# tmtlakmal/acme

Measured on AMD Instinct MI355X. Metric: learner transitions/sec (sample+step) at batch 512, 1/2/4/8 MI355X, higher is better.
Workload: dtype f32 (2xf16 split planes, 3 MFMA terms); 1 GPU; dqn_nature_cnn_prioritized_replay (BASELINE configs[1]); global_batch=512, batch_per_gpu=512, replay_slots=1000000, replay_slots_per_gpu=1000000, obs=uint8[84,84,4], num_actions=18, sampler=prioritized(alpha=0.6), IS beta=0.2, prefetch_size=4, parallelism=dp1

## Files before the change

acme_amd/csrc/conv.h:

```cpp
#pragma once

#include "gemm.h"

namespace acme {
namespace conv {

using gemm::f32x4;
using gemm::KCONTIG;
using gemm::RCONTIG;
using gemm::zero4;

template <int IH_, int IW_, int CI_, int OH_, int OW_, int CO_, int KH_, int KW_, int S_,
          int PT_, int PL_>
struct Geom {
  static constexpr int IH = IH_, IW = IW_, CI = CI_, OH = OH_, OW = OW_, CO = CO_;
  static constexpr int KH = KH_, KW = KW_, S = S_, PT = PT_, PL = PL_;
  static constexpr int K = KH * KW * CI;
  static constexpr int IPIX = IH * IW, OPIX = OH * OW;
  static_assert(CI % 4 == 0 && CO % 4 == 0, "channel counts must be multiples of 4");
};

struct InU8 {
  using T = uint8_t;
  __device__ static __forceinline__ float scale(uint32_t x) {
    const float xf = (float)x;
    const float c = 1.0f / 255.0f;
    const float q = xf * c;
    return __builtin_fmaf(__builtin_fmaf(-q, 255.0f, xf), c, q);
  }
  __device__ static __forceinline__ f32x4 load4(const uint8_t* p) {
    const uint32_t w = *reinterpret_cast<const uint32_t*>(p);
    return f32x4{scale(w & 0xff), scale((w >> 8) & 0xff), scale((w >> 16) & 0xff),
                 scale(w >> 24)};
  }
};
struct InF32 {
  using T = float;
  __device__ static __forceinline__ f32x4 load4(const float* p) {
    return *reinterpret_cast<const f32x4*>(p);
  }
};

template <class G, class In>
struct ConvFwd {
  static constexpr int A_MODE = KCONTIG, B_MODE = KCONTIG;
  int M, N, K, k_chunk;
  const typename In::T* x;
  const typename In::T* x2;
  int split_b;
  const float* w;
  const float* bias;
  float* y;
  struct ARow {
    const typename In::T* base;
    int ih0, iw0;
    bool ok;
  };
  struct BRow {
    int n;
  };
  __device__ ARow a_row(int m) const {
    ARow a;
    a.ok = m < M;
    const int mm = a.ok ? m : 0;
    const int b = mm / G::OPIX, rem = mm - b * G::OPIX;
    const int oh = rem / G::OW, ow = rem - oh * G::OW;
    a.base = b < split_b ? x + (size_t)b * G::IPIX * G::CI
                         : x2 + (size_t)(b - split_b) * G::IPIX * G::CI;
    a.ih0 = oh * G::S - G::PT;
    a.iw0 = ow * G::S - G::PL;
    return a;
  }
  __device__ f32x4 a_load(const ARow& a, int k) const {
    const int kh = k / (G::KW * G::CI), r = k - kh * (G::KW * G::CI);
    const int kw = r / G::CI, ci = r - kw * G::CI;
    const int ih = a.ih0 + kh, iw = a.iw0 + kw;
    if (!a.ok || (unsigned)ih >= (unsigned)G::IH || (unsigned)iw >= (unsigned)G::IW) return zero4();
    return In::load4(a.base + (ih * G::IW + iw) * G::CI + ci);
  }
  __device__ BRow b_row(int n) const { return BRow{n}; }
  __device__ f32x4 b_load(const BRow& b, int k) const {
    if (b.n >= N) return zero4();
    const float* p = w + (size_t)k * G::CO + b.n;
    return f32x4{p[0], p[G::CO], p[2 * G::CO], p[3 * G::CO]};
  }
  __device__ void store(int m, int n, float v, int) const {
    v += bias[n];
    y[(size_t)m * G::CO + n] = v > 0.f ? v : 0.f;
  }
};

template <class G, class In>
struct ConvWgrad {
  static constexpr int A_MODE = RCONTIG, B_MODE = RCONTIG;
  static constexpr bool kColSum = true;
  int M, N, K, k_chunk;
  const typename In::T* x;
  const float* dz;
  float* slab;
  struct ARow {
    int dh, dw, ci;
    bool ok;
  };
  struct BRow {
    int n;
  };
  __device__ ARow a_row(int i) const {
    ARow a;
    a.ok = i < M;
    const int ii = a.ok ? i : 0;
    const int kh = ii / (G::KW * G::CI), r = ii - kh * (G::KW * G::CI);
    const int kw = r / G::CI;
    a.ci = r - kw * G::CI;
    a.dh = kh - G::PT;
    a.dw = kw - G::PL;
    return a;
  }
  __device__ f32x4 a_load(const ARow& a, int m) const {
    if (!a.ok) return zero4();
    const int b = m / G::OPIX, rem = m - b * G::OPIX;
    const int oh = rem / G::OW, ow = rem - oh * G::OW;
    const int ih = oh * G::S + a.dh, iw = ow * G::S + a.dw;
    if ((unsigned)ih >= (unsigned)G::IH || (unsigned)iw >= (unsigned)G::IW) return zero4();
    return In::load4(x + ((size_t)b * G::IPIX + ih * G::IW + iw) * G::CI + a.ci);
  }
  __device__ BRow b_row(int n) const { return BRow{n}; }
  __device__ f32x4 b_load(const BRow& b, int m) const {
    if (b.n >= N) return zero4();
    return *reinterpret_cast<const f32x4*>(dz + (size_t)m * G::CO + b.n);
  }
  __device__ void store(int i, int n, float v, int split) const {
    slab[((size_t)split * (M + 1) + i) * N + n] = v;
  }
  __device__ void store_colsum(int n, float v, int split) const {
    slab[((size_t)split * (M + 1) + M) * N + n] = v;
  }
};

template <class G, int PH, int PW>
struct ConvDgradSub {
  static_assert(G::KH % G::S == 0 && G::KW % G::S == 0, "kernel must be a multiple of stride");
  static constexpr int A_MODE = KCONTIG, B_MODE = KCONTIG;
  static constexpr int S = G::S;
  static constexpr int RH = ((PH - G::PT) % S + S) % S;
  static constexpr int RW = ((PW - G::PL) % S + S) % S;
  static constexpr int NH = (G::IH - RH + S - 1) / S;
  static constexpr int NW = (G::IW - RW + S - 1) / S;
  static constexpr int JH = G::KH / S, JW = G::KW / S;
  static constexpr int KR = JH * JW * G::CO;
  int M, N, K, k_chunk;
  const float* dz;
  const float* w;
  const float* xprev;
  float* dx;
  struct ARow {
    const float* base;
    int oh0, ow0;
    bool ok;
  };
  struct BRow {
    int ci;
  };
  __device__ static void decode(int m, int& b, int& ih, int& iw) {
    b = m / (NH * NW);
    const int rem = m - b * (NH * NW);
    const int i = rem / NW, j = rem - i * NW;
    ih = RH + S * i;
    iw = RW + S * j;
  }
  __device__ ARow a_row(int m) const {
    ARow a;
    a.ok = m < M;
    int b, ih, iw;
    decode(a.ok ? m : 0, b, ih, iw);
    a.base = dz + (size_t)b * G::OPIX * G::CO;
    a.oh0 = (ih + G::PT - PH) / S;
    a.ow0 = (iw + G::PL - PW) / S;
    return a;
  }
  __device__ f32x4 a_load(const ARow& a, int k) const {
    const int jh = k / (JW * G::CO), r = k - jh * (JW * G::CO);
    const int jw = r / G::CO, co = r - jw * G::CO;
    const int oh = a.oh0 - jh, ow = a.ow0 - jw;
    if (!a.ok || (unsigned)oh >= (unsigned)G::OH || (unsigned)ow >= (unsigned)G::OW) return zero4();
    return *reinterpret_cast<const f32x4*>(a.base + (oh * G::OW + ow) * G::CO + co);
  }
  __device__ BRow b_row(int ci) const { return BRow{ci}; }
  __device__ f32x4 b_load(const BRow& b, int k) const {
    if (b.ci >= N) return zero4();
    const int jh = k / (JW * G::CO), r = k - jh * (JW * G::CO);
    const int jw = r / G::CO, co = r - jw * G::CO;
    const int kh = PH + S * jh, kw = PW + S * jw;
    return *reinterpret_cast<const f32x4*>(w + ((size_t)(kh * G::KW + kw) * G::CI + b.ci) * G::CO + co);
  }
  __device__ void store(int m, int ci, float v, int) const {
    int b, ih, iw;
    decode(m, b, ih, iw);
    const size_t idx = ((size_t)b * G::IPIX + ih * G::IW + iw) * G::CI + ci;
    dx[idx] = xprev[idx] > 0.f ? v : 0.f;
  }
};
template <class G>
struct ConvDgradSubZ {
  static_assert(G::KH % G::S == 0 && G::KW % G::S == 0, "kernel must be a multiple of stride");
  static constexpr int A_MODE = KCONTIG, B_MODE = KCONTIG;
  static constexpr bool kZClass = true;
  static constexpr int S = G::S;
  static constexpr int JH = G::KH / S, JW = G::KW / S;
  static constexpr int KR = JH * JW * G::CO;
  int M, N, K, k_chunk;
  int batch;
  const float* dz;
  const float* w;
  const float* xprev;
  float* dx;
  int ph = 0, pw = 0, rh = 0, rw = 0, nh = 1, nw = 1, mc = 0;
  __device__ ConvDgradSubZ for_z(int z) const {
    ConvDgradSubZ q = *this;
    q.ph = z / S;
    q.pw = z % S;
    q.rh = ((q.ph - G::PT) % S + S) % S;
    q.rw = ((q.pw - G::PL) % S + S) % S;
    q.nh = (G::IH - q.rh + S - 1) / S;
    q.nw = (G::IW - q.rw + S - 1) / S;
    q.mc = batch * q.nh * q.nw;
    return q;
  }
  static int max_rows(int batch) {
    int best = 0;
    for (int ph = 0; ph < S; ++ph)
      for (int pw = 0; pw < S; ++pw) {
        const int rh = ((ph - G::PT) % S + S) % S, rw = ((pw - G::PL) % S + S) % S;
        const int n = batch * ((G::IH - rh + S - 1) / S) * ((G::IW - rw + S - 1) / S);
        best = n > best ? n : best;
      }
    return best;
  }
  struct ARow {
    const float* base;
    int oh0, ow0;
    bool ok;
  };
  struct BRow {
    int ci;
  };
  __device__ void decode(int m, int& b, int& ih, int& iw) const {
    b = m / (nh * nw);
    const int rem = m - b * (nh * nw);
    const int i = rem / nw, j = rem - i * nw;
    ih = rh + S * i;
    iw = rw + S * j;
  }
  __device__ ARow a_row(int m) const {
    ARow a;
    a.ok = m < mc;
    int b, ih, iw;
    decode(a.ok ? m : 0, b, ih, iw);
    a.base = dz + (size_t)b * G::OPIX * G::CO;
    a.oh0 = (ih + G::PT - ph) / S;
    a.ow0 = (iw + G::PL - pw) / S;
    return a;
  }
  __device__ f32x4 a_load(const ARow& a, int k) const {
    const int jh = k / (JW * G::CO), r = k - jh * (JW * G::CO);
    const int jw = r / G::CO, co = r - jw * G::CO;
    const int oh = a.oh0 - jh, ow = a.ow0 - jw;
    if (!a.ok || (unsigned)oh >= (unsigned)G::OH || (unsigned)ow >= (unsigned)G::OW) return zero4();
    return *reinterpret_cast<const f32x4*>(a.base + (oh * G::OW + ow) * G::CO + co);
  }
  __device__ BRow b_row(int ci) const { return BRow{ci}; }
  __device__ f32x4 b_load(const BRow& b, int k) const {
    if (b.ci >= N) return zero4();
    const int jh = k / (JW * G::CO), r = k - jh * (JW * G::CO);
    const int jw = r / G::CO, co = r - jw * G::CO;
    const int kh = ph + S * jh, kw = pw + S * jw;
    return *reinterpret_cast<const f32x4*>(w + ((size_t)(kh * G::KW + kw) * G::CI + b.ci) * G::CO + co);
  }
  __device__ void store(int m, int ci, float v, int) const {
    if (m >= mc) return;
    int b, ih, iw;
    decode(m, b, ih, iw);
    const size_t idx = ((size_t)b * G::IPIX + ih * G::IW + iw) * G::CI + ci;
    dx[idx] = xprev[idx] > 0.f ? v : 0.f;
  }
};

template <class G>
struct ConvDgrad {
  static constexpr int A_MODE = KCONTIG, B_MODE = KCONTIG;
  int M, N, K, k_chunk;
  const float* dz;
  const float* w;
  const float* xprev;
  float* dx;
  struct ARow {
    const float* base;
    int th0, tw0;
    bool ok;
  };
  struct BRow {
    int ci;
  };
  __device__ ARow a_row(int m) const {
    ARow a;
    a.ok = m < M;
    const int mm = a.ok ? m : 0;
    const int b = mm / G::IPIX, rem = mm - b * G::IPIX;
    const int ih = rem / G::IW, iw = rem - ih * G::IW;
    a.base = dz + (size_t)b * G::OPIX * G::CO;
    a.th0 = ih + G::PT;
    a.tw0 = iw + G::PL;
    return a;
  }
  __device__ f32x4 a_load(const ARow& a, int k) const {
    const int kh = k / (G::KW * G::CO), r = k - kh * (G::KW * G::CO);
    const int kw = r / G::CO, co = r - kw * G::CO;
    const int th = a.th0 - kh, tw = a.tw0 - kw;
    if (!a.ok || th < 0 || tw < 0) return zero4();
    if (G::S > 1 && ((th % G::S) != 0 || (tw % G::S) != 0)) return zero4();
    const int oh = th / G::S, ow = tw / G::S;
    if (oh >= G::OH || ow >= G::OW) return zero4();
    return *reinterpret_cast<const f32x4*>(a.base + (oh * G::OW + ow) * G::CO + co);
  }
  __device__ BRow b_row(int ci) const { return BRow{ci}; }
  __device__ f32x4 b_load(const BRow& b, int k) const {
    if (b.ci >= N) return zero4();
    const int kh = k / (G::KW * G::CO), r = k - kh * (G::KW * G::CO);
    const int kw = r / G::CO, co = r - kw * G::CO;
    return *reinterpret_cast<const f32x4*>(w + ((size_t)(kh * G::KW + kw) * G::CI + b.ci) * G::CO + co);
  }
  __device__ void store(int m, int ci, float v, int) const {
    const size_t idx = (size_t)m * G::CI + ci;
    dx[idx] = xprev[idx] > 0.f ? v : 0.f;
  }
};

template <bool VEC>
__device__ __forceinline__ f32x4 load_row4(const float* p, int k, int lim) {
  if (VEC) return *reinterpret_cast<const f32x4*>(p + k);
  f32x4 r;
#pragma unroll
  for (int j = 0; j < 4; ++j) r[j] = (k + j < lim) ? p[k + j] : 0.f;
  return r;
}

enum Act { ACT_NONE = 0, ACT_RELU = 1, ACT_ELU = 2, ACT_TANH = 3 };

__device__ __forceinline__ float act_fwd(int act, float v) {
  if (act == ACT_RELU) return v > 0.f ? v : 0.f;
  if (act == ACT_ELU) return v < 0.f ? expm1f(v) : v;
  if (act == ACT_TANH) return tanhf(v);
  return v;
}
__device__ __forceinline__ float act_bwd(int act, float y, float g) {
  if (act == ACT_RELU) return y > 0.f ? g : 0.f;
  if (act == ACT_ELU) return y < 0.f ? g * (y + 1.f) : g;
  if (act == ACT_TANH) return g * (1.f - y * y);
  return g;
}

template <bool VEC, class In = InF32>
struct DenseFwd {
  static constexpr int A_MODE = KCONTIG, B_MODE = KCONTIG;
  int M, N, K, k_chunk;
  const typename In::T* x;
  const typename In::T* x2;
  int split_b;
  int ldx;
  const float* w;
  const float* bias;
  float* y;
  int act;
  float* slab = nullptr;
  struct ARow {
    const typename In::T* p;
  };
  struct BRow {
    int n;
  };
  __device__ ARow a_row(int m) const {
    if (m >= M) return ARow{nullptr};
    return ARow{m < split_b ? x + (size_t)m * ldx : x2 + (size_t)(m - split_b) * ldx};
  }
  __device__ f32x4 a_load(const ARow& a, int k) const {
    if (!a.p) return zero4();
    if constexpr (sizeof(typename In::T) == 1) {
      if (VEC) return In::load4(a.p + k);
      f32x4 r;
      for (int j = 0; j < 4; ++j) r[j] = (k + j < K) ? In::scale(a.p[k + j]) : 0.f;
      return r;
    } else {
      return load_row4<VEC>(reinterpret_cast<const float*>(a.p), k, K);
    }
  }
  __device__ BRow b_row(int n) const { return BRow{n}; }
  __device__ f32x4 b_load(const BRow& b, int k) const {
    if (b.n >= N || k >= K) return zero4();
    const float* p = w + (size_t)k * N + b.n;
    return f32x4{p[0], k + 1 < K ? p[N] : 0.f, k + 2 < K ? p[2 * N] : 0.f,
                 k + 3 < K ? p[3 * N] : 0.f};
  }
  __device__ void store(int m, int n, float v, int split) const {
    if (slab) {
      slab[((size_t)split * M + m) * N + n] = v;
      return;
    }
    v += bias[n];
    y[(size_t)m * N + n] = act_fwd(act, v);
  }
  static constexpr bool kPreStore = true;
  __device__ float pre(int, int n) const { return bias[n]; }
  __device__ float finish(float v, float b) const { return slab ? v : act_fwd(act, v + b); }
  __device__ void put(int m, int n, float v, int split) const {
    if (slab) slab[((size_t)split * M + m) * N + n] = v;
    else y[(size_t)m * N + n] = v;
  }
  static constexpr bool kStrided = sizeof(typename In::T) == 4;
  static constexpr bool kAVec = VEC, kBVec = false;
  __device__ gemm::StridedOp a_op() const {
    return {reinterpret_cast<const float*>(x), (uint32_t)(4u * M * ldx), 4u * ldx, 4u};
  }
  __device__ gemm::StridedOp b_op() const { return {w, (uint32_t)(4u * K * N), 4u, 4u * N}; }
};

template <bool VEC, class In = InF32>
struct DenseWgrad {
  static constexpr int A_MODE = KCONTIG, B_MODE = KCONTIG;
  static constexpr bool kColSum = true;
  int M, N, K, k_chunk;
  const typename In::T* x;
  int ldx;
  const float* dz;
  float* out;
  float* bias_out;
  struct ARow {
    int i;
  };
  struct BRow {
    int n;
  };
  __device__ ARow a_row(int i) const { return ARow{i}; }
  __device__ f32x4 a_load(const ARow& a, int m) const {
    if (a.i >= M || m >= K) return zero4();
    f32x4 r;
#pragma unroll
    for (int j = 0; j < 4; ++j) {
      if (m + j >= K) {
        r[j] = 0.f;
      } else if constexpr (sizeof(typename In::T) == 1) {
        r[j] = In::scale(reinterpret_cast<const uint8_t*>(x)[(size_t)(m + j) * ldx + a.i]);
      } else {
        r[j] = reinterpret_cast<const float*>(x)[(size_t)(m + j) * ldx + a.i];
      }
    }
    return r;
  }
  __device__ BRow b_row(int n) const { return BRow{n}; }
  __device__ f32x4 b_load(const BRow& b, int m) const {
    if (b.n >= N || m >= K) return zero4();
    const float* p = dz + (size_t)m * N + b.n;
    return f32x4{p[0], m + 1 < K ? p[N] : 0.f, m + 2 < K ? p[2 * N] : 0.f,
                 m + 3 < K ? p[3 * N] : 0.f};
  }
  __device__ void store(int i, int n, float v, int) const { out[(size_t)i * N + n] = v; }
  __device__ void store_colsum(int n, float v, int) const {
    if (bias_out) bias_out[n] = v;
  }
  static constexpr bool kStrided = sizeof(typename In::T) == 4;
  static constexpr bool kAVec = false, kBVec = false;
  __device__ gemm::StridedOp a_op() const {
    return {reinterpret_cast<const float*>(x), (uint32_t)(4u * K * ldx), 4u, 4u * ldx};
  }
  __device__ gemm::StridedOp b_op() const { return {dz, (uint32_t)(4u * K * N), 4u, 4u * N}; }
};

template <bool VEC>
struct DenseDgrad {
  static constexpr int A_MODE = KCONTIG, B_MODE = KCONTIG;
  int M, N, K, k_chunk;
  const float* dz;
  const float* w;
  const float* xprev;
  int ldx;
  float* dx;
  int act = ACT_RELU;
  struct ARow {
    const float* p;
  };
  struct BRow {
    const float* p;
  };
  __device__ ARow a_row(int m) const { return ARow{m < M ? dz + (size_t)m * K : nullptr}; }
  __device__ f32x4 a_load(const ARow& a, int k) const {
    if (!a.p) return zero4();
    return load_row4<VEC>(a.p, k, K);
  }
  __device__ BRow b_row(int n) const { return BRow{n < N ? w + (size_t)n * K : nullptr}; }
  __device__ f32x4 b_load(const BRow& b, int k) const {
    if (!b.p) return zero4();
    return load_row4<VEC>(b.p, k, K);
  }
  __device__ void store(int m, int n, float v, int) const {
    const size_t idx = (size_t)m * ldx + n;
    if (xprev) v = act_bwd(act, xprev[idx], v);
    dx[idx] = v;
  }
  static constexpr bool kPreStore = true;
  __device__ float pre(int m, int n) const {
    return (xprev ? xprev : static_cast<const float*>(dx))[(size_t)m * ldx + n];
  }
  __device__ float finish(float v, float xp) const { return xprev ? act_bwd(act, xp, v) : v; }
  __device__ void put(int m, int n, float v, int) const { dx[(size_t)m * ldx + n] = v; }
  static constexpr bool kStrided = true;
  static constexpr bool kAVec = VEC, kBVec = VEC;
  __device__ gemm::StridedOp a_op() const { return {dz, (uint32_t)(4u * M * K), 4u * K, 4u}; }
  __device__ gemm::StridedOp b_op() const { return {w, (uint32_t)(4u * N * K), 4u * K, 4u}; }
};

struct DuelHeadFwd {
  static constexpr int A_MODE = KCONTIG, B_MODE = RCONTIG;
  int M, N, K, k_chunk;
  int H, A;
  const float* h;
  const float* wv;
  const float* wa;
  float* slab;
  struct ARow {
    const float* p;
  };
  struct BRow {
    int n;
  };
  __device__ ARow a_row(int m) const { return ARow{m < M ? h + (size_t)m * K : nullptr}; }
  __device__ f32x4 a_load(const ARow& a, int k) const {
    if (!a.p) return zero4();
    return *reinterpret_cast<const f32x4*>(a.p + k);
  }
  __device__ BRow b_row(int n) const { return BRow{n}; }
  __device__ float wt(int n, int k) const {
    if (n < A) return k >= H ? wa[(size_t)(k - H) * A + n] : 0.f;
    if (n == A) return k < H ? wv[k] : 0.f;
    return 0.f;
  }
  __device__ f32x4 b_load(const BRow& b, int k) const {
    return f32x4{wt(b.n, k), wt(b.n + 1, k), wt(b.n + 2, k), wt(b.n + 3, k)};
  }
  __device__ void store(int m, int n, float v, int split) const {
    slab[((size_t)split * M + m) * N + n] = v;
  }
};

struct DuelHeadWgrad {
  static constexpr int A_MODE = RCONTIG, B_MODE = RCONTIG;
  static constexpr bool kColSum = true;
  int M, N, K, k_chunk;
  int A;
  const float* h;
  const float* g;
  const int32_t* act;
  float* slab;
  struct ARow {
    int i;
  };
  struct BRow {
    int n;
  };
  __device__ ARow a_row(int i) const { return ARow{i}; }
  __device__ f32x4 a_load(const ARow& a, int b) const {
    if (a.i >= M) return zero4();
    return *reinterpret_cast<const f32x4*>(h + (size_t)b * M + a.i);
  }
  __device__ BRow b_row(int n) const { return BRow{n}; }
  __device__ f32x4 b_load(const BRow& r, int b) const {
    const float gb = g[b];
    const int ab = act[b];
    const float inv_a = 1.f / (float)A;
    f32x4 out;
#pragma unroll
    for (int j = 0; j < 4; ++j) {
      const int n = r.n + j;
      out[j] = n < A ? gb * ((n == ab ? 1.f : 0.f) - inv_a) : (n == A ? gb : 0.f);
    }
    return out;
  }
  __device__ void store(int i, int n, float v, int split) const {
    slab[((size_t)split * (M + 1) + i) * N + n] = v;
  }
  __device__ void store_colsum(int n, float v, int split) const {
    slab[((size_t)split * (M + 1) + M) * N + n] = v;
  }
};

}
}
```

acme_amd/csrc/dqn.hip:

```cpp
#include <hip/hip_runtime.h>

#include <algorithm>
#include <cmath>
#include <cstring>
#include <string>
#include <vector>

#include "common.h"
#include "conv.h"
#include "rescale.h"
#include "conv_p3.h"
#include "gemm.h"
#include "gemm_p3.h"
#include "gemm_x6.h"
#include "kernels.h"
#include "launch.h"
#include "learner_common.h"
#include "plane_guard.h"
#include "profiler.h"
#include "rccl_dyn.h"
#include "torso.h"

using namespace acme;
using namespace acme::conv;
using acme::gemm::launch_gemm;

namespace {

using torso::G1;
constexpr int kFlat = torso::kFlat;
constexpr int kHidden = 512;
constexpr int kObsBytes = 84 * 84 * 4;

struct Layer {
  int in = 0, out = 0;
  int w = -1, b = -1;
  bool relu = true;
};

}

struct acme_dqn : PlaneGuard {
  acme_dqn_config cfg;
  std::vector<Tensor> tensors;
  int64_t flat = 0, logical = 0;
  float *params = nullptr, *target = nullptr, *grads = nullptr, *m = nullptr, *v = nullptr;
  int64_t num_steps = 0;
  int t_c1w = -1, t_c1b, t_c2w, t_c2b, t_c3w, t_c3b, t_fcw, t_fcb, t_vw, t_vb, t_aw, t_ab;
  std::vector<Layer> layers;
  std::vector<void*> allocs;
  float *x1 = nullptr, *x2 = nullptr, *x3 = nullptr, *hid = nullptr;
  float *t1 = nullptr, *t2 = nullptr, *t3 = nullptr, *thid = nullptr;
  std::vector<float*> mlp_act, mlp_tact, mlp_dz;
  float *q_on = nullptr, *q_tg = nullptr;
  float *dzh = nullptr, *dz3 = nullptr, *dz2 = nullptr, *dz1 = nullptr;
  float* slab = nullptr;
  int64_t slab_floats = 0;
  bool stamps_on = false;
  uint64_t* stamps = nullptr;
  float* g = nullptr;
  int32_t* a_cache = nullptr;
  float* loss_tmp = nullptr;
  float* td_tmp = nullptr;
  double* prio_tmp = nullptr;
  bool p3_capable = false;
  bool planes_stale = true;
  bool last_p3 = false;
  uint16_t *wpl = nullptr, *tpl = nullptr;
  bool calibrating = false;
  int64_t fwd_batch = 0;
  uint16_t* frames = nullptr;
  torso::Frames cur_frames{nullptr};
  hipStream_t side = nullptr;
  hipEvent_t ev[4] = {nullptr, nullptr, nullptr, nullptr};
  float* slab2 = nullptr;
  bool fused_step = false;
  acme_replay* upd_replay = nullptr;
  const uint64_t* upd_keys = nullptr;
  hipEvent_t upd_after = nullptr;
  const double* upd_prio = nullptr;
  int upd_n = 0;
  bool slabs_pending = false;
  torso::WgradSlab wslabs[3];
  float* side_slab = nullptr;
  float* tslab = nullptr;
  bool target_dirty = true;
  torso::Plane x1p{}, x2p{}, x3p{}, t1p{}, t2p{}, t3p{}, dzhp{}, dz3p{}, dz2p{}, dz1p{};
  LossArgs pending_la{};
  bool loss_pending = false;
  bool head_deferred = false;
  int head_splits = 0;
  int64_t loss_nparts = 0;
  hipEvent_t ev_dense = nullptr;
  hipEvent_t dense_ev = nullptr;
  bool dense_on_side = false;
  void* dp_comm = nullptr;
  int dp_world = 0;
  hipStream_t dp_stream = nullptr;
  hipEvent_t dp_ev[4] = {nullptr, nullptr, nullptr, nullptr};
  double* dp_gmin = nullptr;
  double* loss_part = nullptr;
  bool single_stream = false;
  bool single_role = false;
  bool frames_u8 = true;
  int64_t seq = 0;
  uint32_t* host_verdicts = nullptr;
  uint32_t verdict_seq = 0;
  bool sticky = false;
  bool dp_gate = false;
  int64_t dp_gate_index = -1;
  bool step_rescaled = false;
};

namespace {

enum {
  kScX1, kScX2, kScX3, kScT1, kScT2, kScT3, kScDzh, kScDz3, kScDz2, kScDz1,
  kScTransient,
  kScParams = kScTransient, kScTarget,
  kScCount
};
constexpr int64_t kParamAmaxPeriod = 8;
constexpr int kVerdictRing = 64;

int add_tensor(acme_dqn* l, const std::string& name, std::initializer_list<int64_t> shape) {
  const int t = acme::add_tensor<acme_dqn>(l, name, shape);
  l->logical += l->tensors[t].numel;
  return t;
}

inline torso::Plane WP(const acme_dqn* l, uint16_t* base, int t) {
  return torso::Plane{base + l->tensors[t].offset, l->flat,
                      l->scales + (base == l->tpl ? kScTarget : kScParams)};
}
int convert_frames(acme_dqn* l, const void* obs_a, const void* obs_b, int split, int rows,
                   hipStream_t st) {
  ACME_PROF("frames_f16", st, 0.0, 3.0 * (double)rows * kObsBytes);
  return launch_frames_f16(static_cast<const uint8_t*>(obs_a), static_cast<const uint8_t*>(obs_b),
                           split, rows, kObsBytes, l->frames, st);
}
bool use_p3(const acme_dqn* l) { return l->p3_capable && gemm::use_x6(); }
Gate step_gate(const acme_dqn* l) {
  Gate q;
  q.g = l->guard;
  q.par = (int)(l->seq & 1);
  if (l->dp_gate) q.dp = l->grads + l->dp_gate_index;
  return q;
}
hipStream_t side_stream(const acme_dqn* l) { return prof::enabled() ? nullptr : l->side; }

constexpr int kFcFwdSplits = 8;
constexpr int kHeadFwdSplits = 16;
constexpr int kHeadBwdSplits = 8;

int64_t slab_floats_needed(int B, int A) {
  return std::max<int64_t>({torso::wgrad_slab_floats(), (int64_t)kFcFwdSplits * 2 * B * 2 * kHidden,
                            (int64_t)kHeadFwdSplits * 2 * B * (A + 1),
                            (int64_t)kHeadBwdSplits * (2 * kHidden + 1) * (A + 1)});
}

int slab_reduce(const float* slab, int splits, int64_t count, float* out0, int64_t split_at,
                float* out1, const float* bias, int ncols, int relu, const char* name,
                hipStream_t st) {
  ACME_PROF(name, st, 0.0, 4.0 * (double)(splits + 1) * (double)count);
  return launch_slab_reduce(slab, splits, count, out0, split_at, out1, bias, ncols, relu, st);
}

int adam_range(acme_dqn* l, int64_t off, int64_t n, const Gate& gate, const AdamTail& tail,
               hipStream_t st) {
  const bool jax = l->cfg.semantics == ACME_SEMANTICS_JAX;
  const bool p3 = l->p3_capable;
  return launch_adam(l->params + off, l->grads + off, l->m + off, l->v + off, n,
                     l->cfg.learning_rate, l->cfg.adam_beta1, l->cfg.adam_beta2,
                     l->cfg.adam_epsilon, 0, p3 ? l->wpl + off : nullptr, l->flat, st, jax ? 1 : 0,
                     &l->guard->applied, p3 ? l->scales + kScParams : nullptr, gate, !p3, tail);
}

torso::Weights torso_weights(const acme_dqn* l, const float* prm) {
  return torso::Weights{P(l, prm, l->t_c1w), P(l, prm, l->t_c1b), P(l, prm, l->t_c2w),
                        P(l, prm, l->t_c2b), P(l, prm, l->t_c3w), P(l, prm, l->t_c3b)};
}

int head_forward(acme_dqn* l, const float* prm, int rows, const float* hid, float* q,
                 hipStream_t st) {
  const int A = l->cfg.num_actions;
  DuelHeadFwd p;
  p.M = rows; p.N = A + 1; p.K = 2 * kHidden; p.k_chunk = chunk_for(p.K, kHeadFwdSplits);
  p.H = kHidden; p.A = A; p.h = hid; p.wv = P(l, prm, l->t_vw); p.wa = P(l, prm, l->t_aw);
  p.slab = l->slab;
  ACME_GEMM("head_fwd", 64, 32, 2, 1, 16, 1, p, kHeadFwdSplits);
  ACME_PROF("head_fwd_finish", st, 0.0, 0.0);
  return launch_duel_head_finish(l->slab, kHeadFwdSplits, rows, A, P(l, prm, l->t_vb),
                                 P(l, prm, l->t_ab), q, st);
}

int nature_forward(acme_dqn* l, const float* prm, const void* obs_a, const void* obs_b,
                   int split, int rows, float* x1, float* x2, float* x3, float* hid,
                   float* q, hipStream_t st) {
  const bool u8 = l->cfg.obs_dtype == ACME_OBS_U8_SCALED;
  int rc0 = torso::forward(torso_weights(l, prm), u8, obs_a, obs_b, split, rows,
                           torso::Acts{x1, x2, x3}, st);
  if (rc0 != ACME_OK) return rc0;
  {
    DenseFwd<true> p;
    const int splits = kFcFwdSplits;
    p.M = rows; p.N = 2 * kHidden; p.K = kFlat; p.k_chunk = chunk_for(kFlat, splits);
    p.x = x3; p.x2 = x3; p.split_b = rows; p.ldx = kFlat;
    p.w = P(l, prm, l->t_fcw); p.bias = P(l, prm, l->t_fcb); p.y = hid; p.act = ACT_RELU;
    p.slab = l->slab;
    ACME_GEMM("fc_fwd", 128, 128, 2, 2, 32, 1, p, splits);
    const int64_t cnt = (int64_t)rows * 2 * kHidden;
    int rc = slab_reduce(l->slab, splits, cnt, hid, cnt, nullptr, P(l, prm, l->t_fcb),
                         2 * kHidden, 1, "fc_fwd_reduce", st);
    if (rc != ACME_OK) return rc;
  }
  return head_forward(l, prm, rows, hid, q, st);
}

int nature_forward_p3(acme_dqn* l, const float* prm, uint16_t* wpl, const torso::Frames& frames,
                      int rows, const torso::Plane& x1, const torso::Plane& x2,
                      const torso::Plane& x3, float* hid, float* q, hipStream_t st,
                      float* slab = nullptr, int keep_x1 = -1, bool defer_head = false) {
  if (!slab) slab = l->slab;
  torso::PWeights w{WP(l, wpl, l->t_c1w), WP(l, wpl, l->t_c2w), WP(l, wpl, l->t_c3w),
                    P(l, prm, l->t_c1b), P(l, prm, l->t_c2b), P(l, prm, l->t_c3b)};
  int rc = torso::forward_p3(w, frames, rows, torso::PActs{x1, x2, x3}, st, keep_x1);
  if (rc != ACME_OK) return rc;
  {
    P3DenseFwd p;
    const bool tall = rows > 512;
    const bool ttall = rows == 512 && !defer_head;
    const int splits = kFcFwdSplits;
    p.M = rows; p.N = 2 * kHidden; p.K = kFlat; p.k_chunk = chunk_for(kFlat, splits);
    p.a_src = SRC(x3, (int64_t)rows * kFlat); p.ldx = kFlat;
    p.b_src = SRC(WP(l, wpl, l->t_fcw), (int64_t)kFlat * 2 * kHidden); p.slab = slab;
    if (tall) p.stamps = l->stamps;
    if (ttall && l->single_role) ACME_P3_GEMM("fc_fwd_target", 256, 128, 2, 2, 32, p, splits);
    else if (ttall) ACME_P3WS_GEMM("fc_fwd_target", 256, 128, 2, 2, 32, p, splits);
    else if (tall && l->single_role) ACME_P3_GEMM("fc_fwd", 256, 128, 2, 2, 32, p, splits);
    else if (tall) ACME_P3WS_GEMM("fc_fwd", 256, 128, 2, 2, 32, p, splits);
    else if (l->single_role) ACME_P3_GEMM("fc_fwd", 128, 128, 2, 2, 32, p, splits);
    else ACME_P3WS_GEMM("fc_fwd", 128, 128, 2, 2, 32, p, splits);
    if (defer_head &&
        dqn_head_loss_dz_fusable(kHidden, l->cfg.num_actions, splits, P(l, prm, l->t_vw),
                                 P(l, prm, l->t_aw), P(l, prm, l->t_fcb))) {
      l->head_deferred = true;
      l->head_splits = splits;
      return ACME_OK;
    }
    ACME_PROF("fc_head_fwd", st, 0.0, 4.0 * (double)rows * 2 * kHidden * (splits + 1));
    return launch_fc_head_forward(slab, splits, rows, kHidden, P(l, prm, l->t_fcb),
                                  P(l, prm, l->t_vw), P(l, prm, l->t_vb), P(l, prm, l->t_aw),
                                  P(l, prm, l->t_ab), l->cfg.num_actions, hid, q, st);
  }
}

template <class In>
int mlp_layer(acme_dqn* l, const float* prm, const Layer& L, const void* a, const void* b,
              int split, int rows, float* y, hipStream_t st) {
  const bool vec = L.in % 4 == 0 && L.out % 4 == 0;
  if (vec) {
    DenseFwd<true, In> p;
    p.M = rows; p.N = L.out; p.K = L.in; p.k_chunk = L.in;
    p.x = static_cast<const typename In::T*>(a); p.x2 = static_cast<const typename In::T*>(b);
    p.split_b = split; p.ldx = L.in; p.w = P(l, prm, L.w); p.bias = P(l, prm, L.b); p.y = y;
    p.act = L.relu ? ACT_RELU : ACT_NONE;
    ACME_GEMM("mlp_fwd", 64, 64, 2, 2, 16, 1, p, 1);
  } else {
    DenseFwd<false, In> p;
    p.M = rows; p.N = L.out; p.K = L.in; p.k_chunk = L.in;
    p.x = static_cast<const typename In::T*>(a); p.x2 = static_cast<const typename In::T*>(b);
    p.split_b = split; p.ldx = L.in; p.w = P(l, prm, L.w); p.bias = P(l, prm, L.b); p.y = y;
    p.act = L.relu ? ACT_RELU : ACT_NONE;
    ACME_GEMM("mlp_fwd", 64, 64, 2, 2, 16, 1, p, 1);
  }
  return ACME_OK;
}

int mlp_forward(acme_dqn* l, const float* prm, const void* obs_a, const void* obs_b, int split,
                int rows, std::vector<float*>& act, float* q, hipStream_t st) {
  const int nl = (int)l->layers.size();
  for (int i = 0; i < nl; ++i) {
    const Layer& L = l->layers[i];
    float* y = i == nl - 1 ? q : act[i];
    int rc;
    if (i == 0) {
      rc = l->cfg.obs_dtype == ACME_OBS_U8_SCALED
               ? mlp_layer<InU8>(l, prm, L, obs_a, obs_b, split, rows, y, st)
               : mlp_layer<InF32>(l, prm, L, obs_a, obs_b, split, rows, y, st);
    } else {
      rc = mlp_layer<InF32>(l, prm, L, act[i - 1], act[i - 1], rows, rows, y, st);
    }
    if (rc != ACME_OK) return rc;
  }
  return ACME_OK;
}

RescaleJob step_rescale_job(acme_dqn* l, bool defer_r) {
  RescaleJob j;
  j.s = l->scales;
  j.nt = j.n = kScTransient;
  j.overflow = l->overflow;
  j.skip_lo = kScT1;
  j.skip_hi = kScT3 + 1;
  j.defer_r = defer_r ? 1 : 0;
  j.rg.g = l->guard;
  j.rg.mode = kRgStep;
  j.rg.gate = step_gate(l);
  j.rg.host_skipped = l->host_skipped;
  j.rg.host_verdicts = l->host_verdicts;
  j.rg.seq = l->verdict_seq++;
  j.rg.sticky = l->sticky ? 1 : 0;
  return j;
}

int priority_update_tail(void* ctx, hipStream_t st) {
  acme_dqn* l = static_cast<acme_dqn*>(ctx);
  acme_replay* r = l->upd_replay;
  if (!r || !l->upd_prio) return ACME_OK;
  l->upd_replay = nullptr;
  if (l->upd_after) ACME_HIP_TRY(hipStreamWaitEvent(st, l->upd_after, 0));
  const RescaleJob job = step_rescale_job(l, true);
  const int rc =
      replay_update_priorities_gated(r, l->upd_keys, l->upd_prio, l->upd_n, step_gate(l), st, &job);
  if (rc == ACME_OK) l->step_rescaled = true;
  return rc;
}

int nature_backward(acme_dqn* l, const void* o_tm1, int B, hipStream_t st_main,
                    bool join_dense) {
  hipStream_t st = st_main;
  const float* prm = l->params;
  float* gr = l->grads;
  const int A = l->cfg.num_actions;
  const bool p3 = use_p3(l);
  int rc;
  bool loss_sum = false;
  const LossArgs la = l->pending_la;
  if (p3 && l->loss_pending && l->head_deferred) {
    l->loss_pending = l->head_deferred = false;
    loss_sum = true;
    l->loss_nparts = B;
    ACME_PROF("head_loss_dz", st, 0.0, 4.0 * (double)2 * B * 2 * kHidden * (l->head_splits + 1));
    rc = launch_dqn_head_loss_dz(la, l->slab, l->head_splits, kHidden, P(l, prm, l->t_fcb),
                                 P(l, prm, l->t_vw), P(l, prm, l->t_vb), P(l, prm, l->t_aw),
                                 P(l, prm, l->t_ab), l->hid, l->dzhp.p, l->dzhp.stride,
                                 l->dzhp.sc, st);
    if (rc != ACME_OK) return rc;
  } else if (p3 && l->loss_pending) {
    l->loss_pending = false;
    loss_sum = la.loss_part != nullptr;
    l->loss_nparts = dqn_loss_head_dz_blocks(B, kHidden);
    ACME_PROF("loss_head_dz", st, 0.0, 0.0);
    rc = launch_dqn_loss_head_dz(la, l->hid, kHidden, P(l, prm, l->t_vw),
                                 P(l, prm, l->t_aw), l->dzhp.p, l->dzhp.stride, l->dzhp.sc, st);
    if (rc != ACME_OK) return rc;
  } else {
    ACME_PROF("head_dz", st, 0.0, 0.0);
    rc = p3 ? launch_head_dz_planes(l->hid, l->g, l->a_cache, B, kHidden, A, P(l, prm, l->t_vw),
                                    P(l, prm, l->t_aw), l->dzhp.p, l->dzhp.stride, l->dzhp.sc, st)
            : launch_duel_head_dz(l->hid, l->g, l->a_cache, B, kHidden, A, P(l, prm, l->t_vw),
                                  P(l, prm, l->t_aw), l->dzh, st);
    if (rc != ACME_OK) return rc;
  }
  const bool fork = p3 && side_stream(l);
  float* hslab = fork ? l->side_slab : l->slab;
  if (fork) {
    ACME_HIP_TRY(hipEventRecord(l->ev[2], st_main));
    ACME_HIP_TRY(hipStreamWaitEvent(l->side, l->ev[2], 0));
    st = l->side;
  }
  if (p3 && l->upd_replay && !l->calibrating) {
    l->upd_prio = la.prio;
    l->upd_n = B;
  }
  const bool sum_in_scatter = loss_sum;
  {
    DuelHeadWgrad p;
    p.M = 2 * kHidden; p.N = A + 1; p.K = B; p.k_chunk = chunk_for(B, kHeadBwdSplits);
    p.A = A; p.h = l->hid; p.g = l->g; p.act = l->a_cache; p.slab = hslab;
    ACME_GEMM("head_wgrad", 64, 32, 2, 1, 16, 1, p, kHeadBwdSplits);
    ACME_PROF("head_wgrad_scatter", st, 0.0, 0.0);
    rc = launch_duel_head_grad_scatter(
        hslab, kHeadBwdSplits, kHidden, A, Pm(l, gr, l->t_vw), Pm(l, gr, l->t_vb),
        Pm(l, gr, l->t_aw), Pm(l, gr, l->t_ab), st, sum_in_scatter ? la.loss_part : nullptr,
        l->loss_nparts, la.mean_over, la.loss);
    if (rc != ACME_OK) return rc;
  }
  if (p3) {
    {
      P3DenseWgrad p;
      p.M = kFlat; p.N = 2 * kHidden; p.K = B; p.k_chunk = B;
      p.a_src = SRC(l->x3p, (int64_t)B * kFlat); p.ldx = kFlat;
      p.b_src = SRC(l->dzhp, (int64_t)B * 2 * kHidden); p.out = Pm(l, gr, l->t_fcw);
      p.bias_out = Pm(l, gr, l->t_fcb);
      ACME_P3_GEMM("fc_wgrad", 128, 128, 2, 2, 16, p, 1);
    }
    if (fork) {
      ACME_HIP_TRY(hipEventRecord(l->ev[3], l->side));
      st = st_main;
    }
    {
      P3DenseDgrad p;
      p.M = B; p.N = kFlat; p.K = 2 * kHidden; p.k_chunk = p.K;
      p.a_src = SRC(l->dzhp, (int64_t)B * 2 * kHidden);
      p.b_src = SRC(WP(l, l->wpl, l->t_fcw), (int64_t)kFlat * 2 * kHidden); p.xprev = CP(l->x3p);
      p.ldx = kFlat; p.dx = PP(l->dz3p);
      if (l->single_role) ACME_P3G_GEMM("fc_dgrad", 128, 128, 2, 2, 32, 3, p, 1);
      else ACME_P3WS_GEMM("fc_dgrad", 128, 128, 2, 2, 32, p, 1);
    }
    if (fork && join_dense) ACME_HIP_TRY(hipStreamWaitEvent(st_main, l->ev[3], 0));
    l->dense_on_side = fork;
    return ACME_OK;
  }
  {
    DenseWgrad<true> p;
    p.M = kFlat; p.N = 2 * kHidden; p.K = B; p.k_chunk = B;
    p.x = l->x3; p.ldx = kFlat; p.dz = l->dzh; p.out = Pm(l, gr, l->t_fcw);
    p.bias_out = Pm(l, gr, l->t_fcb);
    ACME_GEMM("fc_wgrad", 128, 128, 2, 2, 16, 1, p, 1);
  }
  {
    DenseDgrad<true> p;
    p.M = B; p.N = kFlat; p.K = 2 * kHidden; p.k_chunk = p.K;
    p.dz = l->dzh; p.w = P(l, prm, l->t_fcw); p.xprev = l->x3; p.ldx = kFlat; p.dx = l->dz3;
    ACME_GEMM("fc_dgrad", 64, 128, 2, 2, 16, 1, p, 1);
  }
  return ACME_OK;
}

template <class In>
int mlp_wgrad(acme_dqn* l, const Layer& L, const void* x, const float* dz, int B, float* dw,
              float* db, hipStream_t st) {
  if (L.in % 4 == 0 && L.out % 4 == 0) {
    DenseWgrad<true, In> p;
    p.M = L.in; p.N = L.out; p.K = B; p.k_chunk = B;
    p.x = static_cast<const typename In::T*>(x); p.ldx = L.in; p.dz = dz; p.out = dw;
    p.bias_out = db;
    ACME_GEMM("mlp_wgrad", 64, 64, 2, 2, 16, 1, p, 1);
  } else {
    DenseWgrad<false, In> p;
    p.M = L.in; p.N = L.out; p.K = B; p.k_chunk = B;
    p.x = static_cast<const typename In::T*>(x); p.ldx = L.in; p.dz = dz; p.out = dw;
    p.bias_out = db;
    ACME_GEMM("mlp_wgrad", 64, 64, 2, 2, 16, 1, p, 1);
  }
  return ACME_OK;
}

int mlp_backward(acme_dqn* l, const void* o_tm1, int B, hipStream_t st) {
  const int nl = (int)l->layers.size();
  const float* prm = l->params;
  float* gr = l->grads;
  int rc = launch_onehot_dq(l->g, l->a_cache, B, l->cfg.num_actions, l->mlp_dz[nl - 1], st);
  if (rc != ACME_OK) return rc;
  for (int i = nl - 1; i >= 0; --i) {
    const Layer& L = l->layers[i];
    const float* dz = l->mlp_dz[i];
    if (i == 0) {
      rc = l->cfg.obs_dtype == ACME_OBS_U8_SCALED
               ? mlp_wgrad<InU8>(l, L, o_tm1, dz, B, Pm(l, gr, L.w), Pm(l, gr, L.b), st)
               : mlp_wgrad<InF32>(l, L, o_tm1, dz, B, Pm(l, gr, L.w), Pm(l, gr, L.b), st);
    } else {
      rc = mlp_wgrad<InF32>(l, L, l->mlp_act[i - 1], dz, B, Pm(l, gr, L.w), Pm(l, gr, L.b), st);
    }
    if (rc != ACME_OK) return rc;
    if (i > 0) {
      if (L.in % 4 == 0 && L.out % 4 == 0) {
        DenseDgrad<true> p;
        p.M = B; p.N = L.in; p.K = L.out; p.k_chunk = L.out;
        p.dz = dz; p.w = P(l, prm, L.w); p.xprev = l->mlp_act[i - 1]; p.ldx = L.in;
        p.dx = l->mlp_dz[i - 1];
        ACME_GEMM("mlp_dgrad", 64, 64, 2, 2, 16, 1, p, 1);
      } else {
        DenseDgrad<false> p;
        p.M = B; p.N = L.in; p.K = L.out; p.k_chunk = L.out;
        p.dz = dz; p.w = P(l, prm, L.w); p.xprev = l->mlp_act[i - 1]; p.ldx = L.in;
        p.dx = l->mlp_dz[i - 1];
        ACME_GEMM("mlp_dgrad", 64, 64, 2, 2, 16, 1, p, 1);
      }
    }
  }
  return ACME_OK;
}

int sync_planes(acme_dqn* l, hipStream_t st) {
  if (!l->p3_capable || !l->planes_stale) return ACME_OK;
  int rc = launch_split_planes(l->params, l->flat, l->wpl, l->flat, l->scales + kScParams, st,
                               l->overflow, 1);
  if (rc == ACME_OK)
    rc = launch_split_planes(l->target, l->flat, l->tpl, l->flat, l->scales + kScTarget, st,
                             l->overflow, 1);
  if (rc == ACME_OK) l->planes_stale = false;
  return rc;
}

int reset_scales(acme_dqn* l) {
  return scales_init(l, kScCount, [l](int i) {
    return i >= kScT1 && i <= kScT3 ? &l->guard->tt
           : i >= kScTransient     ? &l->guard->prm
                                   : &l->guard->on;
  });
}

}

extern "C" {

int acme_dqn_create(const acme_dqn_config* cfg, acme_dqn** out) {
  ACME_CHECK_ARG(cfg && out, "null argument");
  ACME_CHECK_ARG(cfg->num_actions >= 1 && cfg->num_actions <= 63, "num_actions must be in [1, 63]");
  ACME_CHECK_ARG(cfg->max_batch >= 1 && cfg->max_batch <= 65536, "max_batch must be in [1, 65536]");
  ACME_CHECK_ARG(cfg->network == ACME_NET_NATURE_DQN || cfg->network == ACME_NET_MLP,
                 "unknown network kind %d", cfg->network);
  ACME_CHECK_ARG(cfg->obs_dtype == ACME_OBS_U8_SCALED || cfg->obs_dtype == ACME_OBS_F32,
                 "unknown observation dtype %d", cfg->obs_dtype);
  ACME_CHECK_ARG(cfg->huber_loss_parameter >= 0.f, "quadratic_linear_boundary must be >= 0.");
  ACME_CHECK_ARG(cfg->target_update_period >= 1, "target_update_period must be >= 1");
  ACME_CHECK_ARG(cfg->semantics == ACME_SEMANTICS_TF || cfg->semantics == ACME_SEMANTICS_JAX,
                 "unknown learner semantics %d", cfg->semantics);
  acme_dqn* l = new acme_dqn();
  l->cfg = *cfg;
  l->single_stream = tune_variant("SIDE") == 1;
  l->single_role = tune_variant("WSN") == 1;
  l->stamps_on = tune_variant("STAMPS") == 1;
  const int A = cfg->num_actions;
  const int B = cfg->max_batch;
  int rc = ACME_OK;
  auto fail = [&](int code) {
    acme_dqn_destroy(l);
    return code;
  };
  if ((rc = guard_create(l)) != ACME_OK) return fail(rc);
  if (hipHostMalloc(reinterpret_cast<void**>(&l->host_verdicts), kVerdictRing * sizeof(uint32_t),
                    hipHostMallocCoherent | hipHostMallocMapped) != hipSuccess)
    return fail((set_error("step guard allocation failed"), ACME_ERR_HIP));
  for (int i = 0; i < kVerdictRing; ++i) l->host_verdicts[i] = 0xFFFFFFFFu;
  if (cfg->network == ACME_NET_NATURE_DQN) {
    l->t_c1w = add_tensor(l, "atari_torso/conv2_d/w", {8, 8, 4, 32});
    l->t_c1b = add_tensor(l, "atari_torso/conv2_d/b", {32});
    l->t_c2w = add_tensor(l, "atari_torso/conv2_d_1/w", {4, 4, 32, 64});
    l->t_c2b = add_tensor(l, "atari_torso/conv2_d_1/b", {64});
    l->t_c3w = add_tensor(l, "atari_torso/conv2_d_2/w", {3, 3, 64, 64});
    l->t_c3b = add_tensor(l, "atari_torso/conv2_d_2/b", {64});
    l->t_fcw = add_tensor(l, "duelling_q_network/hidden/w", {kFlat, 2 * kHidden});
    l->t_fcb = add_tensor(l, "duelling_q_network/hidden/b", {2 * kHidden});
    l->t_vw = add_tensor(l, "duelling_q_network/mlp/linear_1/w", {kHidden, 1});
    l->t_vb = add_tensor(l, "duelling_q_network/mlp/linear_1/b", {1});
    l->t_aw = add_tensor(l, "duelling_q_network/mlp_1/linear_1/w", {kHidden, A});
    l->t_ab = add_tensor(l, "duelling_q_network/mlp_1/linear_1/b", {A});
    const int R2 = 2 * B;
    if ((rc = dev_alloc(l, &l->x1, (int64_t)R2 * G1::OPIX * G1::CO)) ||
        (rc = dev_alloc(l, &l->x2, (int64_t)R2 * kFlat)) ||
        (rc = dev_alloc(l, &l->x3, (int64_t)R2 * kFlat)) ||
        (rc = dev_alloc(l, &l->hid, (int64_t)R2 * 2 * kHidden)) ||
        (rc = dev_alloc(l, &l->t1, (int64_t)B * G1::OPIX * G1::CO)) ||
        (rc = dev_alloc(l, &l->t2, (int64_t)B * kFlat)) ||
        (rc = dev_alloc(l, &l->t3, (int64_t)B * kFlat)) ||
        (rc = dev_alloc(l, &l->thid, (int64_t)B * 2 * kHidden)) ||
        (rc = dev_alloc(l, &l->dzh, (int64_t)B * 2 * kHidden)) ||
        (rc = dev_alloc(l, &l->dz3, (int64_t)B * kFlat)) ||
        (rc = dev_alloc(l, &l->dz2, (int64_t)B * kFlat)) ||
        (rc = dev_alloc(l, &l->dz1, (int64_t)B * G1::OPIX * G1::CO)))
      return fail(rc);
    l->slab_floats = slab_floats_needed(B, A);
    if (cfg->obs_dtype == ACME_OBS_U8_SCALED && (int64_t)R2 * kObsBytes * 2 < (int64_t)INT32_MAX) {
      l->p3_capable = true;
      const int64_t fl = l->flat;
      if ((rc = reset_scales(l)) ||
          (rc = dev_alloc(l, &l->wpl, gemm::kPlanes * fl)) ||
          (rc = dev_alloc(l, &l->tpl, gemm::kPlanes * fl)) ||
          (rc = dev_alloc(l, &l->frames, (int64_t)R2 * kObsBytes)) ||
          (rc = plane_alloc(l, &l->x1p, (int64_t)R2 * torso::kX1, kScX1)) ||
          (rc = plane_alloc(l, &l->x2p, (int64_t)R2 * kFlat, kScX2)) ||
          (rc = plane_alloc(l, &l->x3p, (int64_t)R2 * kFlat, kScX3)) ||
          (rc = plane_alloc(l, &l->t1p, (int64_t)B * torso::kX1, kScT1)) ||
          (rc = plane_alloc(l, &l->t2p, (int64_t)B * kFlat, kScT2)) ||
          (rc = plane_alloc(l, &l->t3p, (int64_t)B * kFlat, kScT3)) ||
          (rc = plane_alloc(l, &l->dzhp, (int64_t)B * 2 * kHidden, kScDzh)) ||
          (rc = dev_alloc(l, &l->loss_part,
                          std::max<int64_t>(B, dqn_loss_head_dz_blocks(B, kHidden)))) ||
          (rc = plane_alloc(l, &l->dz3p, (int64_t)B * kFlat, kScDz3)) ||
          (rc = plane_alloc(l, &l->dz2p, (int64_t)B * kFlat, kScDz2)) ||
          (rc = plane_alloc(l, &l->dz1p, (int64_t)B * torso::kX1, kScDz1)))
        return fail(rc);
      l->slab_floats = std::max(l->slab_floats, torso::wgrad_slab_floats_p3());
      if (!l->single_stream) {
        hipError_t e = hipStreamCreateWithFlags(&l->side, hipStreamNonBlocking);
        for (auto& ev : l->ev)
          if (e == hipSuccess) e = make_order_event(&ev);
        if (e != hipSuccess)
          return fail((set_error("side stream: %s", hipGetErrorString(e)), ACME_ERR_HIP));
      }
      if ((rc = dev_alloc(l, &l->side_slab, l->slab_floats)) ||
          (rc = dev_alloc(l, &l->tslab, l->slab_floats)) ||
          (rc = dev_alloc(l, &l->slab2, torso::wgrad_slab_floats_p3())))
        return fail(rc);
    }
  } else {
    ACME_CHECK_ARG(cfg->obs_dim >= 1, "obs_dim must be >= 1");
    ACME_CHECK_ARG(cfg->num_hidden >= 0 && cfg->num_hidden <= ACME_MAX_MLP_LAYERS,
                   "num_hidden must be in [0, %d]", ACME_MAX_MLP_LAYERS);
    int in = cfg->obs_dim;
    char name[64];
    for (int i = 0; i <= cfg->num_hidden; ++i) {
      Layer L;
      L.in = in;
      L.out = i < cfg->num_hidden ? cfg->hidden[i] : A;
      L.relu = i < cfg->num_hidden;
      if (L.out < 1) return fail((set_error("hidden sizes must be >= 1"), ACME_ERR_INVALID));
      snprintf(name, sizeof(name), "mlp/linear_%d/w", i);
      L.w = add_tensor(l, name, {L.in, L.out});
      snprintf(name, sizeof(name), "mlp/linear_%d/b", i);
      L.b = add_tensor(l, name, {L.out});
      l->layers.push_back(L);
      in = L.out;
    }
    for (size_t i = 0; i < l->layers.size(); ++i) {
      float *a = nullptr, *ta = nullptr, *dz = nullptr;
      const int w = l->layers[i].out;
      if ((rc = dev_alloc(l, &a, (int64_t)2 * B * w)) || (rc = dev_alloc(l, &ta, (int64_t)B * w)) ||
          (rc = dev_alloc(l, &dz, (int64_t)B * w)))
        return fail(rc);
      l->mlp_act.push_back(a);
      l->mlp_tact.push_back(ta);
      l->mlp_dz.push_back(dz);
    }
    l->slab_floats = 1;
  }
  if (make_order_event(&l->ev_dense) != hipSuccess)
    return fail((set_error("event creation failed"), ACME_ERR_HIP));
  if ((rc = dev_alloc(l, &l->q_on, (int64_t)2 * B * A)) ||
      (rc = dev_alloc(l, &l->q_tg, (int64_t)B * A)) ||
      (rc = dev_alloc(l, &l->slab, l->slab_floats)) ||
      (rc = dev_alloc(l, &l->g, (int64_t)B)) || (rc = dev_alloc(l, &l->a_cache, (int64_t)B)) ||
      (rc = dev_alloc(l, &l->loss_tmp, 4)) || (rc = dev_alloc(l, &l->td_tmp, (int64_t)B)) ||
      (rc = dev_alloc(l, &l->prio_tmp, (int64_t)B)) ||
      (l->stamps_on && (rc = dev_alloc(l, &l->stamps, (int64_t)5 * 4096 * 8))))
    return fail(rc);
  if (l->stamps_on) {
    for (int i = 0; i < 3; ++i) torso::g_stamps_conv[i] = l->stamps + (int64_t)(i + 1) * 4096 * 8;
    g_update_stamps = l->stamps + (int64_t)4 * 4096 * 8;
  }
  if (hipDeviceSynchronize() != hipSuccess)
    return fail((set_error("learner init failed"), ACME_ERR_HIP));
  *out = l;
  return ACME_OK;
}

int acme_dqn_destroy(acme_dqn* l) {
  if (!l) return ACME_OK;
  (void)hipDeviceSynchronize();
  if (l->stamps_on) {
    for (auto& p : torso::g_stamps_conv) p = nullptr;
    g_update_stamps = nullptr;
  }
  for (void* p : l->allocs) (void)hipFree(p);
  for (auto& e : l->ev)
    if (e) (void)hipEventDestroy(e);
  if (l->side) (void)hipStreamDestroy(l->side);
  if (l->ev_dense) (void)hipEventDestroy(l->ev_dense);
  for (auto& e : l->dp_ev)
    if (e) (void)hipEventDestroy(e);
  if (l->dp_stream) (void)hipStreamDestroy(l->dp_stream);
  guard_destroy(l);
  if (l->host_verdicts) (void)hipHostFree(l->host_verdicts);
  delete l;
  return ACME_OK;
}

int64_t acme_dqn_num_params(const acme_dqn* l) { return l ? l->logical : 0; }
int64_t acme_dqn_flat_size(const acme_dqn* l) { return l ? l->flat : 0; }
int32_t acme_dqn_num_tensors(const acme_dqn* l) { return l ? (int32_t)l->tensors.size() : 0; }

int acme_dqn_tensor_info(const acme_dqn* l, int32_t i, int64_t* offset, int64_t* numel,
                         int32_t* ndim, int64_t* shape4, const char** name) {
  return tensor_info(l, i, offset, numel, ndim, shape4, name);
}

int acme_dqn_bind(acme_dqn* l, float* params, float* target, float* grads, float* adam_m,
                  float* adam_v) {
  ACME_CHECK_ARG(l && params && target && grads && adam_m && adam_v, "null buffer");
  for (const float* p : {params, target, grads, adam_m, adam_v})
    ACME_CHECK_ARG(reinterpret_cast<uintptr_t>(p) % 16 == 0, "buffers must be 16-byte aligned");
  l->params = params;
  l->target = target;
  l->grads = grads;
  l->m = adam_m;
  l->v = adam_v;
  l->planes_stale = true;
  l->scales_ok = false;
  return ACME_OK;
}

int acme_dqn_params_changed(acme_dqn* l) {
  ACME_CHECK_ARG(l, "null learner");
  l->planes_stale = true;
  l->scales_ok = false;
  l->target_dirty = true;
  return ACME_OK;
}

int acme_dqn_scale_state(const acme_dqn* l, float* out, int32_t capacity, int32_t* count) {
  return scale_state(l, out, capacity, count);
}

int acme_dqn_set_scale_state(acme_dqn* l, const float* in, int32_t count) {
  const int rc = set_scale_state(l, in, count);
  if (rc == ACME_OK) l->target_dirty = true;
  return rc;
}

int acme_dqn_plane_overflow(acme_dqn* l, int32_t* overflow, int32_t reset) {
  return plane_overflow(l, overflow, reset);
}

int64_t acme_dqn_skipped_steps(const acme_dqn* l) { return skipped_steps(l); }

int acme_dqn_guard_state(acme_dqn* l, int64_t* out4) {
  ACME_CHECK_ARG(l && out4 && l->guard, "null argument");
  StepGuard g;
  if (int rc = read_guard(l, &g)) return rc;
  out4[0] = g.applied;
  out4[1] = g.skipped;
  out4[2] = g.last;
  out4[3] = g.qv;
  return ACME_OK;
}

int acme_dqn_verdict_timeouts(acme_dqn* l, int64_t* out) {
  ACME_CHECK_ARG(l && out, "null argument");
  *out = 0;
  if (!l->guard) return ACME_OK;
  StepGuard g;
  if (int rc = read_guard(l, &g)) return rc;
  *out = g.vtimeout;
  return ACME_OK;
}

int acme_dqn_set_reissue(acme_dqn* l, int32_t enable) {
  ACME_CHECK_ARG(l, "null learner");
  l->sticky = enable != 0 && l->p3_capable;
  return ACME_OK;
}

int64_t acme_dqn_verdicts_issued(const acme_dqn* l) { return l ? (int64_t)l->verdict_seq : 0; }

int acme_dqn_step_verdict(const acme_dqn* l, int64_t seq, int32_t* state) {
  ACME_CHECK_ARG(l && state && seq >= 0, "bad argument");
  *state = -1;
  if (!l->host_verdicts || seq >= (int64_t)l->verdict_seq) return ACME_OK;
  ACME_CHECK_ARG(seq + kVerdictRing >= (int64_t)l->verdict_seq,
                 "verdict %lld is older than the ring's %d", (long long)seq, kVerdictRing);
  const uint32_t v =
      __atomic_load_n(l->host_verdicts + (seq & (kVerdictRing - 1)), __ATOMIC_ACQUIRE);
  if ((v >> 1) == ((uint32_t)seq & 0x7fffffffu)) *state = (int32_t)(v & 1u);
  return ACME_OK;
}

int acme_dqn_set_applied_steps(acme_dqn* l, int64_t n) {
  ACME_CHECK_ARG(l && l->guard && n >= 0, "bad argument");
  return set_applied(l, n);
}

int acme_dqn_skip_word(const acme_dqn* l, const uint32_t** out) {
  ACME_CHECK_ARG(l && out, "null argument");
  *out = l->p3_capable ? &l->guard->last : nullptr;
  return ACME_OK;
}

int acme_dqn_set_data_parallel_gate(acme_dqn* l, int32_t enable) {
  ACME_CHECK_ARG(l, "null learner");
  if (enable && l->cfg.network == ACME_NET_NATURE_DQN && l->p3_capable) {
    const Tensor& t = l->tensors[l->t_c1b];
    ACME_CHECK_ARG(align64(t.offset + t.numel) > t.offset + t.numel, "no padding word for the gate");
    l->dp_gate_index = t.offset + t.numel;
    l->dp_gate = true;
  } else {
    l->dp_gate = false;
  }
  return ACME_OK;
}

int64_t acme_dqn_num_steps(const acme_dqn* l) { return l ? l->num_steps : 0; }
int acme_dqn_set_num_steps(acme_dqn* l, int64_t n) {
  ACME_CHECK_ARG(l && n >= 0, "bad argument");
  l->num_steps = n;
  return ACME_OK;
}

int acme_dqn_debug_buffer(const acme_dqn* l, const char* name, const float** out,
                          int64_t* count) {
  ACME_CHECK_ARG(l && name && out && count, "null argument");
  const int64_t B = l->cfg.max_batch;
  struct {
    const char* n;
    const float* p;
    int64_t c;
  } tab[] = {{"gemm_stamps", reinterpret_cast<const float*>(l->stamps), 2 * 5 * 4096 * 8},
             {"x1", l->x1, 2 * B * 441 * 32}, {"x2", l->x2, 2 * B * kFlat},
             {"x3", l->x3, 2 * B * kFlat},    {"hid", l->hid, 2 * B * 2 * kHidden},
             {"dzh", l->dzh, B * 2 * kHidden}, {"dz3", l->dz3, B * kFlat},
             {"dz2", l->dz2, B * kFlat},       {"dz1", l->dz1, B * 441 * 32},
             {"q_on", l->q_on, 2 * B * l->cfg.num_actions},
             {"q_tg", l->q_tg, B * l->cfg.num_actions}, {"g", l->g, B}};
  for (auto& e : tab)
    if (e.p && std::strcmp(e.n, name) == 0) {
      if (l->last_p3) {
        struct {
          const char* n;
          torso::Plane pl;
        } ptab[] = {{"x1", l->x1p},   {"x2", l->x2p},   {"x3", l->x3p},  {"dzh", l->dzhp},
                    {"dz3", l->dz3p}, {"dz2", l->dz2p}, {"dz1", l->dz1p}};
        for (auto& q : ptab)
          if (std::strcmp(q.n, name) == 0) {
            int rc = launch_join_planes(q.pl.p, q.pl.stride, e.c, const_cast<float*>(e.p),
                                        q.pl.sc, 0);
            if (rc != ACME_OK) return rc;
            ACME_HIP_TRY(hipDeviceSynchronize());
          }
      }
      *out = e.p;
      *count = e.c;
      return ACME_OK;
    }
  for (size_t i = 0; i < l->mlp_act.size(); ++i) {
    char nm[16];
    snprintf(nm, sizeof(nm), "act%zu", i);
    if (std::strcmp(nm, name) == 0) {
      *out = l->mlp_act[i];
      *count = 2 * B * l->layers[i].out;
      return ACME_OK;
    }
  }
  set_error("unknown debug buffer '%s'", name);
  return ACME_ERR_INVALID;
}

int acme_dqn_q_values(acme_dqn* l, const void* obs, int64_t batch, int32_t use_target,
                      float* q_out, void* stream) {
  ACME_CHECK_ARG(l && obs && q_out && l->params, "null argument or unbound learner");
  ACME_CHECK_ARG(batch >= 1 && batch <= l->cfg.max_batch, "batch must be in [1, max_batch]");
  hipStream_t st = as_stream(stream);
  const float* prm = use_target ? l->target : l->params;
  const int B = (int)batch;
  if (l->cfg.network == ACME_NET_NATURE_DQN && use_p3(l)) {
    l->target_dirty = true;
    int rc = sync_planes(l, st);
    if (rc == ACME_OK) rc = convert_frames(l, obs, obs, B, B, st);
    for (int pass = l->scales_ok ? 1 : 0; pass < 2 && rc == ACME_OK; ++pass) {
      rc = nature_forward_p3(l, prm, use_target ? l->tpl : l->wpl, torso::Frames{l->frames}, B,
                             l->t1p, l->t2p, l->t3p, l->thid, q_out, st);
      RescaleGuard rg;
      rg.g = l->guard;
      rg.mode = kRgQValues;
      if (rc == ACME_OK)
        rc = launch_plane_rescale(l->scales + kScT1, 3, 3, -1, -1, l->overflow, st, -1, -1, rg);
    }
    return rc;
  }
  if (l->cfg.network == ACME_NET_NATURE_DQN)
    return nature_forward(l, prm, obs, obs, B, B, l->t1, l->t2, l->t3, l->thid, q_out, st);
  return mlp_forward(l, prm, obs, obs, B, B, l->mlp_tact, q_out, st);
}

static int forward_backward_stage(acme_dqn* l, const acme_transition_batch* batch,
                                  const acme_dqn_outputs* out, int32_t stage, void* stream,
                                  bool join_dense);

int acme_dqn_forward_backward_stage(acme_dqn* l, const acme_transition_batch* batch,
                                    const acme_dqn_outputs* out, int32_t stage, void* stream) {
  return forward_backward_stage(l, batch, out, stage, stream, true);
}

static int loss_and_dense_backward(acme_dqn* l, const acme_transition_batch* batch,
                                   const acme_dqn_outputs* out, hipStream_t st, bool join_dense);

constexpr int kCalibrationPasses = 4;
static int calibrate_scales(acme_dqn* l, const acme_transition_batch* batch, hipStream_t st) {
  acme_transition_batch cb = *batch;
  cb.global_min_probability = nullptr;
  l->calibrating = true;
  int rc = ACME_OK;
  for (int pass = 0; pass < kCalibrationPasses && rc == ACME_OK; ++pass) {
    rc = forward_backward_stage(l, &cb, nullptr, 2, st, false);
    if (rc == ACME_OK) rc = forward_backward_stage(l, &cb, nullptr, 3, st, false);
    if (rc == ACME_OK) rc = forward_backward_stage(l, &cb, nullptr, 1, st, false);
    if (rc == ACME_OK)
      rc = launch_plane_rescale(l->scales, kScTransient, kScTransient, -1, -1, l->overflow, st);
  }
  l->calibrating = false;
  if (rc != ACME_OK) return rc;
  return calibration_done(l, st);
}

static int forward_backward_stage(acme_dqn* l, const acme_transition_batch* batch,
                                  const acme_dqn_outputs* out, int32_t stage, void* stream,
                                  bool join_dense) {
  ACME_CHECK_ARG(l && batch && l->params, "null argument or unbound learner");
  ACME_CHECK_ARG(stage >= 0 && stage <= 4, "stage must be 0, 1, 2, 3 or 4");
  ACME_CHECK_ARG(batch->o_tm1 && batch->a_tm1 && batch->r_t && batch->d_t && batch->o_t &&
                     batch->probabilities,
                 "transition batch has null fields");
  ACME_CHECK_ARG(batch->batch >= 1 && batch->batch <= l->cfg.max_batch,
                 "batch %lld outside [1, max_batch=%d]", (long long)batch->batch, l->cfg.max_batch);
  hipStream_t st = as_stream(stream);
  const int B = (int)batch->batch;
  const bool nature = l->cfg.network == ACME_NET_NATURE_DQN;
  if (stage == 1) {
    if (!nature) return ACME_OK;
    if (use_p3(l)) {
      torso::Grads g{Pm(l, l->grads, l->t_c1w), Pm(l, l->grads, l->t_c1b),
                     Pm(l, l->grads, l->t_c2w), Pm(l, l->grads, l->t_c2b),
                     Pm(l, l->grads, l->t_c3w), Pm(l, l->grads, l->t_c3b)};
      torso::PWeights w{WP(l, l->wpl, l->t_c1w), WP(l, l->wpl, l->t_c2w),
                        WP(l, l->wpl, l->t_c3w), P(l, l->params, l->t_c1b),
                        P(l, l->params, l->t_c2b), P(l, l->params, l->t_c3b)};
      torso::Side sd;
      sd.single_role = l->single_role;
      sd.conv1_single = true;
      if (side_stream(l)) {
        sd.side = l->side;
        sd.slab = l->side_slab;
        for (int i = 0; i < 3; ++i) sd.e[i] = l->ev[i];
      }
      l->slabs_pending = false;
      if (l->upd_replay && l->upd_prio && !l->calibrating) {
        sd.tail = priority_update_tail;
        sd.tail_ctx = l;
      }
      if (l->fused_step && !l->calibrating && l->slab2) {
        sd.slab = l->side_slab;
        sd.slab2 = l->slab2;
        sd.defer = l->wslabs;
        l->slabs_pending = true;
      }
      int rc = torso::backward_p3(w, g, l->cur_frames, B,
                                  torso::PActs{l->x1p, l->x2p, l->x3p}, l->dz3p, l->dz2p, l->dz1p,
                                  l->slab, st, sd);
      if (rc == ACME_OK && l->dp_gate && !l->calibrating) {
        Gate local = step_gate(l);
        local.dp = nullptr;
        rc = launch_gate_publish(local, l->grads + l->dp_gate_index, st, l->scales,
                                 kScTransient, kScT1, kScT3 + 1);
      }
      return rc;
    }
    torso::Grads g{Pm(l, l->grads, l->t_c1w), Pm(l, l->grads, l->t_c1b), Pm(l, l->grads, l->t_c2w),
                   Pm(l, l->grads, l->t_c2b), Pm(l, l->grads, l->t_c3w), Pm(l, l->grads, l->t_c3b)};
    return torso::backward(torso_weights(l, l->params), g,
                           l->cfg.obs_dtype == ACME_OBS_U8_SCALED, batch->o_tm1, B,
                           torso::Acts{l->x1, l->x2, l->x3}, l->dz3, l->dz2, l->dz1, l->slab, st);
  }
  const int A = l->cfg.num_actions;
  int rc;
  if (stage == 3 || stage == 4) {
    ACME_CHECK_ARG(l->fwd_batch == (int64_t)B, "stage %d needs the stage-2 forward of this batch",
                   stage);
    l->fwd_batch = 0;
    return loss_and_dense_backward(l, batch, out, st, join_dense && stage == 3);
  }
  l->last_p3 = nature && use_p3(l);
  if (l->last_p3) {
    const bool u8 = !batch->obs_f16 && l->frames_u8 &&
                    ((reinterpret_cast<uintptr_t>(batch->o_tm1) |
                      reinterpret_cast<uintptr_t>(batch->o_t)) & 15) == 0;
    const bool quiet =
        !l->planes_stale && l->scales_ok && (batch->obs_f16 || u8) && !l->calibrating;
    if ((rc = sync_planes(l, st)) != ACME_OK) return rc;
    if (!l->scales_ok && !l->calibrating && (rc = calibrate_scales(l, batch, st)) != ACME_OK)
      return rc;
    l->last_p3 = true;
    hipStream_t tst = st;
    hipStream_t side = side_stream(l);
    if (!batch->obs_f16 && !u8 &&
        (rc = convert_frames(l, batch->o_tm1, batch->o_t, B, 2 * B, st)) != ACME_OK)
      return rc;
    const torso::Frames fwd_frames =
        u8 ? torso::Frames{batch->o_tm1, true, batch->o_t, B}
           : torso::Frames{batch->obs_f16 ? static_cast<const void*>(batch->obs_f16)
                                          : static_cast<const void*>(l->frames)};
    l->cur_frames = fwd_frames;
    if (side) {
      if (quiet && batch->inputs_event && !l->target_dirty) {
        ACME_HIP_TRY(hipStreamWaitEvent(side, static_cast<hipEvent_t>(batch->inputs_event), 0));
      } else {
        ACME_HIP_TRY(hipEventRecord(l->ev[0], st));
        ACME_HIP_TRY(hipStreamWaitEvent(side, l->ev[0], 0));
      }
      l->target_dirty = l->calibrating;
      tst = side;
    } else {
      l->target_dirty = true;
    }
    const bool online_first = side != nullptr;
    l->head_deferred = false;
    if (online_first &&
        (rc = nature_forward_p3(l, l->params, l->wpl, fwd_frames, 2 * B, l->x1p, l->x2p, l->x3p,
                                l->hid, l->q_on, st, nullptr, B, true)) != ACME_OK)
      return rc;
    if ((rc = nature_forward_p3(l, l->target, l->tpl, fwd_frames.rows_from(B), B,
                                l->t1p, l->t2p, l->t3p, l->thid, l->q_tg, tst,
                                side ? l->tslab : l->slab, 0)) != ACME_OK)
      return rc;
    {
      RescaleGuard rg;
      rg.g = l->guard;
      rg.mode = kRgTarget;
      rg.gate = step_gate(l);
      if ((rc = launch_plane_rescale(l->scales + kScT1, 3, 3, -1, -1, l->overflow, tst, -1, -1,
                                     rg)))
        return rc;
    }
    if (side) ACME_HIP_TRY(hipEventRecord(l->ev[1], side));
    if (!online_first &&
        (rc = nature_forward_p3(l, l->params, l->wpl, fwd_frames, 2 * B, l->x1p, l->x2p, l->x3p,
                                l->hid, l->q_on, st, nullptr, B, true)) != ACME_OK)
      return rc;
    if (side) ACME_HIP_TRY(hipStreamWaitEvent(st, l->ev[1], 0));
  } else if (nature) {
    if ((rc = nature_forward(l, l->params, batch->o_tm1, batch->o_t, B, 2 * B, l->x1, l->x2, l->x3,
                             l->hid, l->q_on, st)) != ACME_OK)
      return rc;
    if ((rc = nature_forward(l, l->target, batch->o_t, batch->o_t, B, B, l->t1, l->t2, l->t3,
                             l->thid, l->q_tg, st)) != ACME_OK)
      return rc;
  } else {
    if ((rc = mlp_forward(l, l->params, batch->o_tm1, batch->o_t, B, 2 * B, l->mlp_act, l->q_on,
                          st)) != ACME_OK)
      return rc;
    if ((rc = mlp_forward(l, l->target, batch->o_t, batch->o_t, B, B, l->mlp_tact, l->q_tg, st)) !=
        ACME_OK)
      return rc;
  }
  if (stage == 2) {
    l->fwd_batch = B;
    return ACME_OK;
  }
  return loss_and_dense_backward(l, batch, out, st, join_dense);
}

static int loss_and_dense_backward(acme_dqn* l, const acme_transition_batch* batch,
                                   const acme_dqn_outputs* out, hipStream_t st, bool join_dense) {
  const int B = (int)batch->batch, A = l->cfg.num_actions;
  const bool nature = l->cfg.network == ACME_NET_NATURE_DQN;
  int rc;
  float* loss = out && out->loss ? out->loss : l->loss_tmp;
  float* td = out && out->td_error ? out->td_error : l->td_tmp;
  double* prio = out && out->priorities ? out->priorities : l->prio_tmp;
  LossArgs la;
  la.q_on = l->q_on;
  la.q_tg = l->q_tg;
  la.a = batch->a_tm1;
  la.r = batch->r_t;
  la.d = batch->d_t;
  la.probs = batch->probabilities;
  la.global_min_prob = batch->global_min_probability;
  la.B = B;
  la.A = A;
  la.mean_over = batch->mean_over > 0 ? (int)batch->mean_over : B;
  la.discount = l->cfg.discount;
  la.beta = l->cfg.importance_sampling_exponent;
  la.delta = l->cfg.huber_loss_parameter;
  la.max_abs_reward = l->cfg.max_abs_reward;
  la.jax = l->cfg.semantics == ACME_SEMANTICS_JAX;
  la.loss = loss;
  la.td = td;
  la.prio = prio;
  la.g = l->g;
  la.a_cache = l->a_cache;
  if (l->last_p3) {
    la.loss_part = l->loss_part;
    l->pending_la = la;
    l->loss_pending = true;
  } else {
    ACME_PROF("loss", st, 0.0, 0.0);
    if ((rc = launch_dqn_loss(la, st)) != ACME_OK) return rc;
  }
  l->dense_on_side = false;
  rc = nature ? nature_backward(l, batch->o_tm1, B, st, join_dense)
              : mlp_backward(l, batch->o_tm1, B, st);
  if (rc != ACME_OK) return rc;
  if (out && out->q_tm1)
    ACME_HIP_TRY(hipMemcpyAsync(out->q_tm1, l->q_on, (size_t)B * A * sizeof(float),
                                hipMemcpyDeviceToDevice, st));
  if (l->dense_on_side) {
    l->dense_ev = l->ev[3];
  } else {
    ACME_HIP_TRY(hipEventRecord(l->ev_dense, st));
    l->dense_ev = l->ev_dense;
  }
  return ACME_OK;
}

int acme_dqn_forward_backward(acme_dqn* l, const acme_transition_batch* batch,
                              const acme_dqn_outputs* out, void* stream) {
  int rc = forward_backward_stage(l, batch, out, 0, stream, false);
  if (rc != ACME_OK) return rc;
  return forward_backward_stage(l, batch, out, 1, stream, false);
}

int acme_dqn_grad_split(const acme_dqn* l, int64_t* split) {
  ACME_CHECK_ARG(l && split, "null argument");
  *split = l->cfg.network == ACME_NET_NATURE_DQN ? l->tensors[l->t_fcw].offset : 0;
  return ACME_OK;
}

static int apply_impl(acme_dqn* l, bool copy, hipStream_t st) {
  int rc = ACME_OK;
  Gate gate;
  AdamTail tail;
  if (l->p3_capable) {
    if (!l->step_rescaled) {
      ACME_PROF("plane_rescale", st, 0.0, 0.0);
      if ((rc = launch_rescale_job(step_rescale_job(l, false), st)) != ACME_OK) return rc;
    } else {
      tail.commit = l->scales;
      tail.ncommit = kScTransient;
      tail.skip_lo = kScT1;
      tail.skip_hi = kScT3 + 1;
    }
    l->step_rescaled = false;
    gate.g = l->guard;
    gate.use_last = 1;
    tail.clear = l->guard;
    tail.params = l->scales + kScParams;
    if (copy) tail.target = l->scales + kScTarget;
  }
  const double adam_bytes = 28.0 * (double)l->logical + (l->p3_capable ? 4.0 * (double)l->flat : 0.0);
  if (l->slabs_pending) {
    l->slabs_pending = false;
    double slab_bytes = 0.0;
    for (int k = 0; k < 3; ++k) {
      const double count4 = (double)((l->wslabs[k].wcount + l->wslabs[k].bcount) / 4);
      slab_bytes += 16.0 * count4 * (double)(l->wslabs[k].splits + 1);
    }
    ACME_PROF("adam", st, 0.0, adam_bytes + slab_bytes);
    const int ten[3][2] = {{l->t_c1w, l->t_c1b}, {l->t_c2w, l->t_c2b}, {l->t_c3w, l->t_c3b}};
    AdamSlabs a;
    for (int k = 0; k < 3; ++k) {
      const torso::WgradSlab& w = l->wslabs[k];
      const int64_t count4 = (w.wcount + w.bcount) / 4;
      for (int j = 0; j < 2; ++j) {
        const Tensor& t = l->tensors[ten[k][j]];
        a.seg[a.nseg++] = AdamSlabs::Seg{t.offset / 4, t.numel / 4, w.slab, w.splits, count4,
                                         j ? w.wcount / 4 : 0};
      }
    }
    a.dense_off4 = l->tensors[l->t_fcw].offset / 4;
    a.dense_n4 = (l->flat - l->tensors[l->t_fcw].offset) / 4;
    rc = launch_adam_slabs(l->params, l->grads, l->m, l->v, a, l->cfg.learning_rate,
                           l->cfg.adam_beta1, l->cfg.adam_beta2, l->cfg.adam_epsilon,
                           &l->guard->applied, l->wpl, l->flat, l->scales + kScParams,
                           l->cfg.semantics == ACME_SEMANTICS_JAX ? 1 : 0, gate, tail, st);
    if (rc != ACME_OK) return rc;
  } else {
    ACME_PROF("adam", st, 0.0, adam_bytes);
    if ((rc = adam_range(l, 0, l->flat, gate, tail, st)) != ACME_OK) return rc;
  }
  if (copy) {
    l->target_dirty = true;
    ACME_PROF("target_copy", st, 0.0, 8.0 * (double)l->logical);
    if (l->p3_capable) {
      if ((rc = launch_copy_gated(l->target, l->params, l->flat * sizeof(float), l->tpl, l->wpl,
                                  gemm::kPlanes * l->flat * sizeof(uint16_t), gate, st)))
        return rc;
    } else {
      ACME_HIP_TRY(hipMemcpyAsync(l->target, l->params, l->flat * sizeof(float),
                                  hipMemcpyDeviceToDevice, st));
    }
  }
  if (l->p3_capable && l->num_steps % kParamAmaxPeriod == 0) {
    {
      ACME_PROF("param_amax", st, 0.0, 4.0 * (double)l->flat);
      if ((rc = launch_param_amax(l->params, l->flat, l->scales + kScParams, st)) != ACME_OK)
        return rc;
    }
    ACME_PROF("param_rescale", st, 0.0, 0.0);
    rc = launch_plane_rescale(l->scales + kScParams, 0, 1, -1, -1, l->overflow, st);
  }
  return rc;
}

static bool copies_target(const acme_dqn* l) {
  const int64_t at = l->cfg.semantics == ACME_SEMANTICS_JAX ? l->num_steps + 1 : l->num_steps;
  return at % l->cfg.target_update_period == 0;
}

int acme_dqn_apply(acme_dqn* l, void* stream) {
  ACME_CHECK_ARG(l && l->params, "unbound learner");
  int rc = apply_impl(l, copies_target(l), as_stream(stream));
  if (rc != ACME_OK) return rc;
  l->num_steps += 1;
  l->seq += 1;
  return ACME_OK;
}

static int step_impl(acme_dqn* l, const acme_transition_batch* batch, const acme_dqn_outputs* out,
                     bool copy, hipStream_t st) {
  int rc = forward_backward_stage(l, batch, out, 0, st, false);
  l->fused_step = true;
  if (rc == ACME_OK) rc = forward_backward_stage(l, batch, out, 1, st, false);
  l->fused_step = false;
  if (rc == ACME_OK) rc = apply_impl(l, copy, st);
  return rc;
}

int acme_dqn_dense_grads_ready(acme_dqn* l, void* stream) {
  ACME_CHECK_ARG(l && l->dense_ev, "no stage 3 / 4 has run");
  ACME_HIP_TRY(hipStreamWaitEvent(as_stream(stream), l->dense_ev, 0));
  return ACME_OK;
}

int acme_dqn_dp_init(acme_dqn* l, void* nccl_comm, int32_t world_size) {
  ACME_CHECK_ARG(l && nccl_comm && world_size >= 1, "bad data-parallel arguments");
  if (!acme::rccl::api()) return ACME_ERR_HIP;
  if (!l->dp_stream) {
    ACME_HIP_TRY(hipStreamCreateWithFlags(&l->dp_stream, hipStreamNonBlocking));
    for (auto& e : l->dp_ev) ACME_HIP_TRY(make_order_event(&e));
    int rc = dev_alloc(l, &l->dp_gmin, 1);
    if (rc != ACME_OK) return rc;
  }
  l->dp_comm = nccl_comm;
  l->dp_world = world_size;
  return acme_dqn_set_data_parallel_gate(l, 1);
}

int acme_dqn_dp_step(acme_dqn* l, const acme_transition_batch* batch, const acme_dqn_outputs* out,
                     void* stream) {
  ACME_CHECK_ARG(l && batch && l->params, "null argument or unbound learner");
  ACME_CHECK_ARG(l->dp_comm, "acme_dqn_dp_init must be called first");
  const acme::rccl::Api* r = acme::rccl::api();
  if (!r) return ACME_ERR_HIP;
  hipStream_t st = as_stream(stream), cs = l->dp_stream;
  ncclComm_t comm = static_cast<ncclComm_t>(l->dp_comm);
  auto nccl = [&](ncclResult_t e, const char* what) {
    if (e == ncclSuccess) return ACME_OK;
    set_error("%s: %s", what, r->GetErrorString(e));
    return ACME_ERR_HIP;
  };
  int rc = acme_min_f64(batch->probabilities, batch->batch, l->dp_gmin, st);
  if (rc != ACME_OK) return rc;
  ACME_HIP_TRY(hipEventRecord(l->dp_ev[0], st));
  ACME_HIP_TRY(hipStreamWaitEvent(cs, l->dp_ev[0], 0));
  if ((rc = nccl(r->AllReduce(l->dp_gmin, l->dp_gmin, 1, ncclFloat64, ncclMin, comm, cs),
                 "all-reduce (min probability)")))
    return rc;
  ACME_HIP_TRY(hipEventRecord(l->dp_ev[1], cs));
  acme_transition_batch b = *batch;
  b.global_min_probability = l->dp_gmin;
  if ((rc = forward_backward_stage(l, &b, out, 2, st, false))) return rc;
  ACME_HIP_TRY(hipStreamWaitEvent(st, l->dp_ev[1], 0));
  if ((rc = forward_backward_stage(l, &b, out, 4, st, false))) return rc;
  int64_t split = 0;
  if ((rc = acme_dqn_grad_split(l, &split))) return rc;
  ACME_HIP_TRY(hipStreamWaitEvent(cs, l->dense_ev, 0));
  const ncclRedOp_t avg = static_cast<ncclRedOp_t>(ncclAvg);
  if ((rc = nccl(r->AllReduce(l->grads + split, l->grads + split, (size_t)(l->flat - split),
                              ncclFloat32, avg, comm, cs),
                 "all-reduce (dense gradients)")))
    return rc;
  if ((rc = forward_backward_stage(l, &b, out, 1, st, false))) return rc;
  if (split > 0) {
    ACME_HIP_TRY(hipEventRecord(l->dp_ev[2], st));
    ACME_HIP_TRY(hipStreamWaitEvent(cs, l->dp_ev[2], 0));
    if ((rc = nccl(r->AllReduce(l->grads, l->grads, (size_t)split, ncclFloat32, avg, comm, cs),
                   "all-reduce (torso gradients)")))
      return rc;
  }
  ACME_HIP_TRY(hipEventRecord(l->dp_ev[3], cs));
  ACME_HIP_TRY(hipStreamWaitEvent(st, l->dp_ev[3], 0));
  if ((rc = apply_impl(l, copies_target(l), st))) return rc;
  l->num_steps += 1;
  l->seq += 1;
  return ACME_OK;
}

int acme_dqn_step_update(acme_dqn* l, const acme_transition_batch* batch,
                         const acme_dqn_outputs* out, acme_replay* replay, const uint64_t* keys,
                         void* after_event, void* stream) {
  ACME_CHECK_ARG(l && batch && l->params, "null argument or unbound learner");
  ACME_CHECK_ARG(replay && keys, "null replay or keys");
  const bool inside = use_p3(l) && l->cfg.network == ACME_NET_NATURE_DQN && !l->calibrating;
  l->upd_replay = inside ? replay : nullptr;
  l->upd_keys = keys;
  l->upd_prio = nullptr;
  l->upd_after = static_cast<hipEvent_t>(after_event);
  int rc = step_impl(l, batch, out, copies_target(l), as_stream(stream));
  const bool pending = l->upd_replay != nullptr || !inside;
  l->upd_replay = nullptr;
  if (rc != ACME_OK) return rc;
  l->num_steps += 1;
  l->seq += 1;
  if (pending) {
    const double* prio = out && out->priorities ? out->priorities : l->prio_tmp;
    if (after_event)
      ACME_HIP_TRY(hipStreamWaitEvent(as_stream(stream), static_cast<hipEvent_t>(after_event), 0));
    Gate q;
    if (l->p3_capable) {
      q.g = l->guard;
      q.use_last = 1;
    }
    return replay_update_priorities_gated(replay, keys, prio, batch->batch, q,
                                          as_stream(stream));
  }
  return ACME_OK;
}

int acme_dqn_step(acme_dqn* l, const acme_transition_batch* batch, const acme_dqn_outputs* out,
                  void* stream) {
  ACME_CHECK_ARG(l && batch && l->params, "null argument or unbound learner");
  const int rc = step_impl(l, batch, out, copies_target(l), as_stream(stream));
  if (rc != ACME_OK) return rc;
  l->num_steps += 1;
  l->seq += 1;
  return ACME_OK;
}

}
```

acme_amd/csrc/gemm_p3c12.h:

```cpp
#pragma once

#include "conv_p3.h"
#include "gemm_p3i.h"

namespace acme {
namespace gemm {

template <class G1, class G2, bool U8 = false>
struct P3C1ToLds {
  using Base = conv::P3ConvFwd<G1, 1, U8>;
  using I2 = ImgGeom<G2, false>;
  static constexpr int A_MODE = Base::A_MODE, B_MODE = Base::B_MODE;
  static constexpr int A_PLANES = 1, B_PLANES = kPlanes;
  static constexpr bool kStore8 = true;
  static constexpr bool kAmax = true;
  int M, N, K, k_chunk;
  Base base;
  uint8_t* x1;
  int plane;
  int m0;
  bool hbm;
  __device__ PScale* amax_sc() const { return base.y.sc; }
  __device__ float store8(int m, int n, const conv::V8& acc, int) const {
    conv::V8 v;
    base.act8(n, acc, v);
    uint32_t h[4], l[4];
    const float mx = conv::split8(v, base.y.w(), h, l);
    const int pp = m - m0, oh = pp / G1::OW, ow = pp - oh * G1::OW;
    const int q = I2::pix(0, oh, ow);
    const int a = q * (2 * I2::C) + 16 * ((n / 8) ^ I2::swz(q));
    *reinterpret_cast<u32x4*>(x1 + a) = u32x4{h[0], h[1], h[2], h[3]};
    *reinterpret_cast<u32x4*>(x1 + plane + a) = u32x4{l[0], l[1], l[2], l[3]};
    if (hbm) {
      const int64_t e = (int64_t)m * G1::CO + n;
      *reinterpret_cast<uint4*>(base.y.p + e) = uint4{h[0], h[1], h[2], h[3]};
      *reinterpret_cast<uint4*>(base.y.p + base.y.stride + e) = uint4{l[0], l[1], l[2], l[3]};
    }
    return mx;
  }
};

template <class G1, class G2, bool U8 = false>
struct P3C12Cfg {
  using I1 = ImgGeomPairs<G1>;
  using I2 = ImgGeom<G2, false>;
  using P1 = conv::P3ConvFwd<G1, 1, U8>;
  using P2 = conv::P3ConvFwd<G2, kPlanes>;
  static constexpr int NP = kPlanes;
  using P1L = P3C1ToLds<G1, G2, U8>;
  static constexpr int NT = 512, BK = 32, KS = 2;
  using C1 = P3Core<512, 32, 8, 1, BK, P1L>;
  using C2 = P3Core<128, 64, 4, 2, BK, P2>;
  using PB1 = PlanP3<32, NT, RCONTIG, NP, BK>;
  using PB2 = PlanP3<64, NT, RCONTIG, NP, BK>;
  static constexpr int FRAME = I1::IMG + 16;
  static constexpr int RING1 = FRAME;
  static constexpr int X1 = RING1 + 2 * PB1::BYTES;
  static constexpr int PLANE2 = I2::IMG + 16;
  static constexpr int LDS = X1 + NP * PLANE2;
  static_assert(2 * PB2::BYTES <= I1::IMG && C1::EPI_BYTES <= I1::IMG && C2::EPI_BYTES <= I1::IMG,
                "conv2's ring and the epilogue staging reuse the frame image region");
  static_assert(G1::OPIX <= 512 && I2::OPIX <= 128 && P2::A_PLANES == NP, "geometry");
};

template <class G1, class G2, bool U8>
__global__ void __launch_bounds__(512) gemm_p3c12_kernel(const conv::P3ConvFwd<G1, 1, U8> p1,
                                                         const conv::P3ConvFwd<G2, kPlanes> p2,
                                                         int frames, int hbm_frames) {
  using Cfg = P3C12Cfg<G1, G2, U8>;
  using I1 = typename Cfg::I1;
  using I2 = typename Cfg::I2;
  using PB1 = typename Cfg::PB1;
  using PB2 = typename Cfg::PB2;
  using P1 = typename Cfg::P1;
  using P2 = typename Cfg::P2;
  constexpr int NT = Cfg::NT, BK = Cfg::BK, KS = Cfg::KS, NP = Cfg::NP;
  extern __shared__ __attribute__((aligned(16))) uint8_t smem[];
  const int tid = threadIdx.x, lane = tid & 63, wave = tid >> 6;
  const int f = blockIdx.x;
  uint8_t* x1 = smem + Cfg::X1;
  using S0 = std::integral_constant<int, 0>;
  using S1 = std::integral_constant<int, 1>;

  const bool own1 = PB1::owns(tid), own2 = PB2::owns(tid);
  const typename P1::BRow br1 = p1.b_row(own1 ? PB1::row_of(tid) : 0);
  const typename P2::BRow br2 = p2.b_row(own2 ? PB2::row_of(tid) : 0);
  __amdgpu_buffer_rsrc_t sb1[NP], sb2[NP];
#pragma unroll
  for (int pl = 0; pl < NP; ++pl) {
    sb1[pl] = plane_rsrc(p1.b_src, pl);
    sb2[pl] = plane_rsrc(p2.b_src, pl);
  }
  u32x4 r1[2][NP], r2[2][NP];
  auto fetch1 = [&](auto S, int k0) {
    constexpr int set = decltype(S)::value;
    const uint32_t off = own1 && k0 < p1.K ? p1.b_off(br1, k0, PB1::kk_of(tid)) : kOOB;
#pragma unroll
    for (int pl = 0; pl < NP; ++pl)
      r1[set][pl] = __builtin_bit_cast(u32x4, __builtin_amdgcn_raw_buffer_load_b128(sb1[pl], off, 0, 0));
  };
  auto fetch2 = [&](auto S, int k0) {
    constexpr int set = decltype(S)::value;
    const uint32_t off = own2 && k0 < p2.K ? p2.b_off(br2, k0, PB2::kk_of(tid)) : kOOB;
#pragma unroll
    for (int pl = 0; pl < NP; ++pl)
      r2[set][pl] = __builtin_bit_cast(u32x4, __builtin_amdgcn_raw_buffer_load_b128(sb2[pl], off, 0, 0));
  };
  auto stash1 = [&](auto S, int buf) {
    constexpr int set = decltype(S)::value;
    if (!own1) return;
    uint8_t* s = smem + Cfg::RING1 + buf * PB1::BYTES;
#pragma unroll
    for (int pl = 0; pl < NP; ++pl) *reinterpret_cast<u32x4*>(s + pl * PB1::PLANE + PB1::offset(tid)) = r1[set][pl];
  };
  auto stash2 = [&](auto S, int buf) {
    constexpr int set = decltype(S)::value;
    if (!own2) return;
    uint8_t* s = smem + buf * PB2::BYTES;
#pragma unroll
    for (int pl = 0; pl < NP; ++pl) *reinterpret_cast<u32x4*>(s + pl * PB2::PLANE + PB2::offset(tid)) = r2[set][pl];
  };
  fetch1(S0{}, 0);
  fetch1(S1{}, BK);
  fetch2(S0{}, 0);
  fetch2(S1{}, BK);

  if constexpr (AU8<P1>::value) {
    constexpr int U8U = I1::UNITS / 2;
    constexpr int PER = (U8U + NT - 1) / NT;
    const __amdgpu_buffer_rsrc_t sa = plane_rsrc(p1.a_src, 0);
    u32x4 v[PER];
#pragma unroll
    for (int j = 0; j < PER; ++j) {
      const int u = tid + j * NT;
      const uint32_t off = u < U8U ? (uint32_t)(((int64_t)f * U8U + u) * 16) : kOOB;
      v[j] = __builtin_bit_cast(u32x4, __builtin_amdgcn_raw_buffer_load_b128(sa, off, 0, 0));
    }
#pragma unroll
    for (int j = 0; j < PER; ++j) {
      const int u = tid + j * NT;
      if (u < U8U) {
        *reinterpret_cast<u32x4*>(smem + I1::fill(0, 2 * u)) = f16x8_of_bytes(v[j][0], v[j][1]);
        *reinterpret_cast<u32x4*>(smem + I1::fill(0, 2 * u + 1)) = f16x8_of_bytes(v[j][2], v[j][3]);
      }
    }
    if (tid == 0) *reinterpret_cast<u32x4*>(smem + Cfg::FRAME - 16) = zero_u4();
    if (tid < NP) *reinterpret_cast<u32x4*>(x1 + tid * Cfg::PLANE2 + Cfg::PLANE2 - 16) = zero_u4();
  } else {
    constexpr int PER = (I1::UNITS + NT - 1) / NT;
    const __amdgpu_buffer_rsrc_t sa = plane_rsrc(p1.a_src, 0);
    u32x4 v[PER];
#pragma unroll
    for (int j = 0; j < PER; ++j) {
      const int u = tid + j * NT;
      const uint32_t off = u < I1::UNITS ? (uint32_t)(((int64_t)f * I1::UNITS + u) * 16) : kOOB;
      v[j] = __builtin_bit_cast(u32x4, __builtin_amdgcn_raw_buffer_load_b128(sa, off, 0, 0));
    }
#pragma unroll
    for (int j = 0; j < PER; ++j) {
      const int u = tid + j * NT;
      if (u < I1::UNITS) *reinterpret_cast<u32x4*>(smem + I1::fill(0, u)) = v[j];
    }
    if (tid == 0) *reinterpret_cast<u32x4*>(smem + Cfg::FRAME - 16) = zero_u4();
    if (tid < NP) *reinterpret_cast<u32x4*>(x1 + tid * Cfg::PLANE2 + Cfg::PLANE2 - 16) = zero_u4();
  }
  stash1(S0{}, 0);
  __syncthreads();

  {
    typename I1::Lane ln[2];
#pragma unroll
    for (int i = 0; i < 2; ++i) {
      const int lr = wave * 64 + i * 32 + (lane & 31);
      ln[i] = I1::lane(0, lr, lr < G1::OPIX);
    }
    typename Cfg::C1::Acc acc;
    acc.zero();
    auto compute = [&](int k0, int buf) {
      const uint8_t* sb = smem + Cfg::RING1 + buf * PB1::BYTES;
      typename I1::Stage sg[2];
#pragma unroll
      for (int i = 0; i < 2; ++i) sg[i] = I1::stage(ln[i], k0);
#pragma unroll
      for (int s = 0; s < KS; ++s) {
        f16x8 fb[NP];
#pragma unroll
        for (int pl = 0; pl < NP; ++pl) fb[pl] = PB1::frag(sb, pl, 0, s, lane);
#pragma unroll
        for (int i = 0; i < 2; ++i) {
          const int u = I1::unit(sg[i], ln[i], k0, s, lane >> 5);
          const f16x8 fa[1] = {*reinterpret_cast<const f16x8*>(smem + (u >= 0 ? u : Cfg::FRAME - 16))};
          acc.terms(i, 0, fa, fb);
        }
      }
    };
    auto iter = [&](auto S, int kt) {
      constexpr int set = decltype(S)::value;
      using Other = std::integral_constant<int, set ^ 1>;
      stash1(Other{}, set ^ 1);
      fetch1(S, (kt + 2) * BK);
      compute(kt * BK, set);
      __syncthreads();
    };
    const int nk = p1.K / BK;
    for (int kt = 0; kt < nk; kt += 2) {
      iter(S0{}, kt);
      iter(S1{}, kt + 1);
    }
    typename Cfg::P1L q;
    q.M = (f + 1) * G1::OPIX < p1.M ? (f + 1) * G1::OPIX : p1.M;
    q.N = p1.N; q.K = p1.K; q.k_chunk = p1.k_chunk;
    q.base = p1; q.x1 = x1; q.plane = Cfg::PLANE2; q.m0 = f * G1::OPIX; q.hbm = f < hbm_frames;
    Cfg::C1::epilogue(q, smem, q.m0, 0, wave, wave, 0, lane, 0, acc, false);
  }

  stash2(S0{}, 0);
  __syncthreads();
  {
    const int wm = wave >> 1, wn = wave & 1;
    const int lr = wm * 32 + (lane & 31);
    const typename I2::Lane ln = I2::lane(0, lr, lr < I2::OPIX);
    typename Cfg::C2::Acc acc;
    acc.zero();
    auto compute = [&](int k0, int buf) {
      const uint8_t* sb = smem + buf * PB2::BYTES;
      const typename I2::Stage sg = I2::stage(ln, k0);
#pragma unroll
      for (int s = 0; s < KS; ++s) {
        f16x8 fb[NP];
#pragma unroll
        for (int pl = 0; pl < NP; ++pl) fb[pl] = PB2::frag(sb, pl, wn * 32, s, lane);
        const int u = I2::unit(sg, ln, k0, s, lane >> 5);
        const uint8_t* a = x1 + (u >= 0 ? u : Cfg::PLANE2 - 16);
        f16x8 fa[NP];
#pragma unroll
        for (int pl = 0; pl < NP; ++pl) fa[pl] = *reinterpret_cast<const f16x8*>(a + pl * Cfg::PLANE2);
        acc.terms(0, 0, fa, fb);
      }
    };
    auto iter = [&](auto S, int kt) {
      constexpr int set = decltype(S)::value;
      using Other = std::integral_constant<int, set ^ 1>;
      stash2(Other{}, set ^ 1);
      fetch2(S, (kt + 2) * BK);
      compute(kt * BK, set);
      __syncthreads();
    };
    const int nk = p2.K / BK;
    for (int kt = 0; kt < nk; kt += 2) {
      iter(S0{}, kt);
      iter(S1{}, kt + 1);
    }
    P2 q = p2;
    q.M = (f + 1) * I2::OPIX < p2.M ? (f + 1) * I2::OPIX : p2.M;
    Cfg::C2::epilogue(q, smem, f * I2::OPIX, 0, wave, wm, wn, lane, 0, acc, false);
  }
}

template <class G1, class G2, bool U8>
inline hipError_t launch_gemm_p3c12(const conv::P3ConvFwd<G1, 1, U8>& p1,
                                    const conv::P3ConvFwd<G2, kPlanes>& p2, int frames, int hbm_frames,
                                    hipStream_t st) {
  using Cfg = P3C12Cfg<G1, G2, U8>;
  static_assert(Cfg::LDS <= 160 * 1024, "LDS");
  static hipError_t attr = p3_set_lds(&gemm_p3c12_kernel<G1, G2, U8>, Cfg::LDS);
  if (attr != hipSuccess) return attr;
  if (frames < 1 || p1.M != frames * G1::OPIX || p2.M != frames * G2::OPIX || p1.N > 32 ||
      p2.N > 64 || (p1.K / Cfg::BK) % 2 != 0 || (p2.K / Cfg::BK) % 2 != 0)
    return hipErrorInvalidValue;
  hipLaunchKernelGGL((gemm_p3c12_kernel<G1, G2, U8>), dim3(frames), dim3(Cfg::NT), Cfg::LDS, st, p1, p2,
                     frames, hbm_frames);
  return hipGetLastError();
}

}
}
```

acme_amd/csrc/gemm_p3i.h:

```cpp
#pragma once

#include "gemm_p3.h"

namespace acme {
namespace gemm {

template <class G, bool DGRAD>
struct ImgGeom {
  static constexpr int H = DGRAD ? G::OH : G::IH, W = DGRAD ? G::OW : G::IW;
  static constexpr int C = DGRAD ? G::CO : G::CI;
  static constexpr int OH = DGRAD ? G::IH : G::OH, OW = DGRAD ? G::IW : G::OW;
  static constexpr int S = DGRAD ? 1 : G::S;
  static constexpr int KW = G::KW;
  static constexpr int OPIX = OH * OW, IPIX = H * W;
  static constexpr int CPX = C / 8;
  static constexpr int HALF = (W + 1) / 2;
  static constexpr int SWZ = CPX == 8 ? 1 : 2;
  static constexpr int UNITS = IPIX * CPX, IMG = IPIX * 2 * C;
  static_assert(!DGRAD || G::S == 1, "strided input gradients are not image-resident");
  static_assert(C == 32 || C == 64, "a 32-k stage must stay within one tap");
  static_assert(S == 1 || S == 2, "stride 1 or 2");
  __device__ static __forceinline__ int dh(int kh) { return DGRAD ? G::PT - kh : kh - G::PT; }
  __device__ static __forceinline__ int dw(int kw) { return DGRAD ? G::PL - kw : kw - G::PL; }
  __device__ static __forceinline__ int pix(int fr, int ih, int iw) {
    return (fr * H + ih) * W + (S == 1 ? iw : (iw & 1) * HALF + (iw >> 1));
  }
  __device__ static __forceinline__ int swz(int q) { return (q >> SWZ) & (CPX - 1); }
  __device__ static __forceinline__ int fill(int f, int u) {
    const int px = u / CPX, c = u - px * CPX;
    const int ih = px / W, iw = px - ih * W;
    const int q = pix(f, ih, iw);
    return q * (2 * C) + 16 * (c ^ swz(q));
  }
  struct Lane {
    int f, ih, iw;
    bool ok;
  };
  __device__ static __forceinline__ Lane lane(int f, int pp, bool ok) {
    const int oh = pp / OW, ow = pp - oh * OW;
    return Lane{f, oh * S, ow * S, ok};
  }
  struct Stage {
    int base, x;
  };
  __device__ static __forceinline__ Stage stage(const Lane& l, int k0) {
    const int tap = k0 / C;
    const int kh = tap / KW, kw = tap - kh * KW;
    const int ih = l.ih + dh(kh), iw = l.iw + dw(kw);
    const bool in = l.ok && (unsigned)ih < (unsigned)H && (unsigned)iw < (unsigned)W;
    const int q = pix(l.f, ih, iw);
    return Stage{in ? q * (2 * C) : -1, swz(q)};
  }
  __device__ static __forceinline__ int unit(const Stage& st, const Lane&, int k0, int s, int h) {
    const int c = ((k0 % C) >> 3) + 2 * s + h;
    return st.base >= 0 ? st.base + 16 * (c ^ st.x) : -1;
  }
};

template <class G>
struct ImgGeomPairs {
  static constexpr int UNIT = 16;
  static constexpr int H = G::IH, W = G::IW;
  static constexpr int OW = G::OW, OPIX = G::OPIX;
  static constexpr int PAIRS = W / 2, HALF = (PAIRS + 1) / 2;
  static constexpr int UNITS = H * PAIRS, IMG = UNITS * UNIT;
  static_assert(G::CI == 4 && G::KW * G::CI == 32, "4 channels, one kernel row per stage");
  static_assert(W % 2 == 0 && G::S % 2 == 0 && G::PL % 2 == 0, "pairs never straddle the border");
  __device__ static __forceinline__ int col(int pw) { return (pw & 1) * HALF + (pw >> 1); }
  __device__ static __forceinline__ int fill(int f, int u) {
    const int ih = u / PAIRS, pw = u - ih * PAIRS;
    return ((f * H + ih) * PAIRS + col(pw)) * UNIT;
  }
  struct Lane {
    int f, ih, iw;
    bool ok;
  };
  __device__ static __forceinline__ Lane lane(int f, int pp, bool ok) {
    const int oh = pp / OW, ow = pp - oh * OW;
    return Lane{f, oh * G::S - G::PT, ow * G::S - G::PL, ok};
  }
  struct Stage {
    int base;
  };
  __device__ static __forceinline__ Stage stage(const Lane& l, int k0) {
    const int ih = l.ih + k0 / 32;
    const bool in = l.ok && (unsigned)ih < (unsigned)H;
    return Stage{in ? (l.f * H + ih) * PAIRS * UNIT : -1};
  }
  __device__ static __forceinline__ int unit(const Stage& st, const Lane& l, int, int s, int h) {
    const int iw = l.iw + 4 * s + 2 * h;
    return st.base >= 0 && (unsigned)iw < (unsigned)W ? st.base + col(iw >> 1) * UNIT : -1;
  }
};


template <class GI, int FPB, int BN, int WM, int WN, int MT, class P>
struct P3ICfg {
  static constexpr int BK = 32, KS = 2;
  static constexpr int NW = WM * WN, NT = 64 * NW;
  static constexpr int TN = BN / WN, NTL = TN / 32;
  static constexpr int BM = WM * 32 * MT;
  static_assert(BM >= FPB * GI::OPIX, "the block's waves must cover its frames' rows");
  static_assert(TN % 32 == 0, "wave panel of whole 32-column MFMA tiles");
  using Core = P3Core<BM, BN, WM, WN, BK, P>;
  using PB = typename Core::PB;
  static constexpr int NPA = P::A_PLANES;
  static constexpr int PLANE = FPB * GI::IMG + 16;
  static constexpr int IMG = NPA * PLANE;
  static constexpr int STAGE_B = PB::BYTES;
  static constexpr int MAIN = IMG + 2 * STAGE_B;
  static constexpr int LDS = MAIN > Core::EPI_BYTES ? MAIN : Core::EPI_BYTES;
};

template <class GI, int FPB, int BN, int WM, int WN, int MT, class P>
__global__ void __launch_bounds__(64 * WM * WN) gemm_p3i_kernel(const P p_in, int frames) {
  using Cfg = P3ICfg<GI, FPB, BN, WM, WN, MT, P>;
  using C = typename Cfg::Core;
  using PB = typename Cfg::PB;
  constexpr int NT = Cfg::NT, NTL = Cfg::NTL, TN = Cfg::TN, BK = Cfg::BK, KS = Cfg::KS;
  constexpr int PLANE = Cfg::PLANE, NPA = Cfg::NPA;
  constexpr int NPB = kPlanes;
  static_assert(P::A_MODE == KCONTIG && (NPA == 1 || NPA == kPlanes) && P::B_PLANES == NPB,
                "k-contiguous A (one or two planes), two-plane B");
  extern __shared__ __attribute__((aligned(16))) uint8_t smem[];

  const int tid = threadIdx.x;
  const int lane = tid & 63, wave = tid >> 6;
  const int wm = wave / WN, wn = wave % WN;
  uint64_t st_rt0 = 0, st_t0 = 0, st_t1 = 0, st_t2 = 0;
  bool stamp = false;
  if constexpr (HasStamps<P>::value) {
    stamp = p_in.stamps != nullptr && tid == 0;
    if (stamp) {
      st_rt0 = __builtin_amdgcn_s_memrealtime();
      st_t0 = __builtin_amdgcn_s_memtime();
    }
  }
  const int f0 = blockIdx.x * FPB;
  const int nf = frames - f0 < FPB ? frames - f0 : FPB;
  const int rows = nf * GI::OPIX;
  const int m0 = f0 * GI::OPIX;
  P p = p_in;
  p.M = m0 + rows < p_in.M ? m0 + rows : p_in.M;
  const int nk = p.K / BK;

  typename P::BRow brow[PB::PER_THREAD];
#pragma unroll
  for (int i = 0; i < PB::PER_THREAD; ++i)
    brow[i] = p.b_row(PB::owns(tid + i * NT) ? PB::row_of(tid + i * NT) : 0);
  __amdgpu_buffer_rsrc_t srcB[NPB];
#pragma unroll
  for (int pl = 0; pl < NPB; ++pl) srcB[pl] = plane_rsrc(p.b_src, pl);
  constexpr int RS = 2;
  u32x4 rb[RS][PB::PER_THREAD][NPB];
  auto fetch_b = [&](auto S, int k0) {
    constexpr int set = decltype(S)::value;
#pragma unroll
    for (int i = 0; i < PB::PER_THREAD; ++i) {
      const int u = tid + i * NT;
      const int kk = PB::kk_of(u);
      const uint32_t off = (PB::owns(u) && k0 + kk < p.K) ? p.b_off(brow[i], k0, kk) : kOOB;
#pragma unroll
      for (int pl = 0; pl < NPB; ++pl)
        rb[set][i][pl] =
            __builtin_bit_cast(u32x4, __builtin_amdgcn_raw_buffer_load_b128(srcB[pl], off, 0, 0));
    }
  };
  auto stash_b = [&](auto S, int buf) {
    constexpr int set = decltype(S)::value;
    uint8_t* sb = smem + Cfg::IMG + buf * Cfg::STAGE_B;
#pragma unroll
    for (int i = 0; i < PB::PER_THREAD; ++i) {
      const int u = tid + i * NT;
      if (!PB::owns(u)) continue;
      const int off = PB::offset(u);
#pragma unroll
      for (int pl = 0; pl < NPB; ++pl)
        *reinterpret_cast<u32x4*>(sb + pl * PB::PLANE + off) = rb[set][i][pl];
    }
  };

  using S0 = std::integral_constant<int, 0>;
  using S1 = std::integral_constant<int, 1>;
  fetch_b(S0{}, 0);
  fetch_b(S1{}, BK);

  constexpr int UB = 16;
  using UT = u32x4;
  if constexpr (AU8<P>::value) {
    static_assert(FPB == 1 && NPA == 1 && GI::UNITS % 2 == 0, "uint8 frames: one per block");
    constexpr int U8U = GI::UNITS / 2;
    constexpr int PER = (U8U + NT - 1) / NT;
    const bool second = f0 >= p.a_split;
    const __amdgpu_buffer_rsrc_t sa = plane_rsrc(second ? p.a_src2 : p.a_src, 0);
    const int fl = second ? f0 - p.a_split : f0;
    u32x4 v[PER];
#pragma unroll
    for (int j = 0; j < PER; ++j) {
      const int u = tid + j * NT;
      const uint32_t off = u < U8U ? (uint32_t)(((int64_t)fl * U8U + u) * 16) : kOOB;
      v[j] = __builtin_bit_cast(u32x4, __builtin_amdgcn_raw_buffer_load_b128(sa, off, 0, 0));
    }
#pragma unroll
    for (int j = 0; j < PER; ++j) {
      const int u = tid + j * NT;
      if (U8U % NT == 0 || u < U8U) {
        *reinterpret_cast<u32x4*>(smem + GI::fill(0, 2 * u)) = f16x8_of_bytes(v[j][0], v[j][1]);
        *reinterpret_cast<u32x4*>(smem + GI::fill(0, 2 * u + 1)) = f16x8_of_bytes(v[j][2], v[j][3]);
      }
    }
    if (tid == 0) *reinterpret_cast<u32x4*>(smem + PLANE - 16) = zero_u4();
  } else {
    constexpr int UNITS = FPB * GI::UNITS;
    constexpr int PER = (UNITS + NT - 1) / NT;
    __amdgpu_buffer_rsrc_t srcA[NPA];
#pragma unroll
    for (int pl = 0; pl < NPA; ++pl) srcA[pl] = plane_rsrc(p.a_src, pl);
    UT v[PER][NPA];
#pragma unroll
    for (int j = 0; j < PER; ++j) {
      const int u = tid + j * NT;
      const int f = u / GI::UNITS;
      const bool ok = u < UNITS && f < nf;
      const uint32_t off = ok ? (uint32_t)(((int64_t)f0 * GI::UNITS + u) * UB) : kOOB;
#pragma unroll
      for (int pl = 0; pl < NPA; ++pl) {
        v[j][pl] = __builtin_bit_cast(UT, __builtin_amdgcn_raw_buffer_load_b128(srcA[pl], off, 0, 0));
      }
    }
#pragma unroll
    for (int j = 0; j < PER; ++j) {
      const int u = tid + j * NT;
      if (UNITS % NT == 0 || u < UNITS) {
        const int f = u / GI::UNITS;
        const int a = GI::fill(f, u - f * GI::UNITS);
#pragma unroll
        for (int pl = 0; pl < NPA; ++pl) *reinterpret_cast<UT*>(smem + pl * PLANE + a) = v[j][pl];
      }
    }
    if (tid < NPA) *reinterpret_cast<u32x4*>(smem + tid * PLANE + PLANE - 16) = zero_u4();
  }
  stash_b(S0{}, 0);

  typename GI::Lane ln[MT];
#pragma unroll
  for (int i = 0; i < MT; ++i) {
    const int lr = wm * 32 * MT + i * 32 + (lane & 31);
    const int f = lr / GI::OPIX;
    ln[i] = GI::lane(f, lr - f * GI::OPIX, lr < rows);
  }
  __syncthreads();
  if constexpr (HasStamps<P>::value)
    if (stamp) st_t1 = __builtin_amdgcn_s_memtime();

  typename C::Acc acc;
  acc.zero();
  typename EpiPre<P>::type pre{};
  if constexpr (EpiPre<P>::has) pre = p.pre(wn * TN + C::epi_col(lane));

  auto compute = [&](int k0, int buf) {
    const uint8_t* sb = smem + Cfg::IMG + buf * Cfg::STAGE_B;
    typename GI::Stage sg[MT];
#pragma unroll
    for (int i = 0; i < MT; ++i) sg[i] = GI::stage(ln[i], k0);
    f16x8 fb[KS][NTL][NPB], fa[KS][MT][NPA];
#pragma unroll
    for (int s = 0; s < KS; ++s) {
#pragma unroll
      for (int j = 0; j < NTL; ++j)
#pragma unroll
        for (int pl = 0; pl < NPB; ++pl) fb[s][j][pl] = PB::frag(sb, pl, wn * TN + j * 32, s, lane);
#pragma unroll
      for (int i = 0; i < MT; ++i) {
        const int u = GI::unit(sg[i], ln[i], k0, s, lane >> 5);
        const int a = u >= 0 ? u : PLANE - 16;
#pragma unroll
        for (int pl = 0; pl < NPA; ++pl)
          fa[s][i][pl] = *reinterpret_cast<const f16x8*>(smem + pl * PLANE + a);
      }
    }
    __builtin_amdgcn_sched_barrier(0);
#pragma unroll
    for (int s = 0; s < KS; ++s)
#pragma unroll
      for (int i = 0; i < MT; ++i)
#pragma unroll
        for (int j = 0; j < NTL; ++j) acc.terms(i, j, fa[s][i], fb[s][j]);
  };

  auto iter = [&](auto S, int kt) {
    constexpr int set = decltype(S)::value;
    using Next = std::integral_constant<int, (set + 1) % RS>;
    stash_b(Next{}, (kt + 1) & 1);
    fetch_b(S, (kt + RS) * BK);
    __builtin_amdgcn_sched_barrier(0);
    compute(kt * BK, kt & 1);
    __syncthreads();
  };
  int kt = 0;
  for (; kt + 1 < nk; kt += 2) {
    iter(S0{}, kt);
    iter(S1{}, kt + 1);
  }
  if (kt < nk) iter(S0{}, kt);

  if constexpr (HasStamps<P>::value)
    if (stamp) st_t2 = __builtin_amdgcn_s_memtime();
  C::epilogue(p, smem, m0, 0, wave, wm, wn, lane, 0, acc, false, &pre);
  if constexpr (HasStamps<P>::value) {
    if (stamp) {
      uint64_t* o = p_in.stamps + 8 * (int64_t)blockIdx.x;
      o[0] = st_rt0;
      o[1] = __builtin_amdgcn_s_memrealtime();
      o[2] = st_t0;
      o[3] = st_t1;
      o[4] = st_t2;
      o[5] = __builtin_amdgcn_s_memtime();
    }
  }
}

template <class GI, int FPB, int BN, int WM, int WN, int MT, class P>
inline hipError_t launch_gemm_p3i(const P& p, int frames, hipStream_t st) {
  using Cfg = P3ICfg<GI, FPB, BN, WM, WN, MT, P>;
  static_assert(Cfg::LDS <= 160 * 1024, "image + two B stages must fit the 160-KiB LDS");
  static hipError_t attr = p3_set_lds(&gemm_p3i_kernel<GI, FPB, BN, WM, WN, MT, P>, Cfg::LDS);
  if (attr != hipSuccess) return attr;
  if (p.N > BN || p.M != frames * GI::OPIX || p.K % Cfg::BK != 0) return hipErrorInvalidValue;
  const int blocks = (frames + FPB - 1) / FPB;
  hipLaunchKernelGGL((gemm_p3i_kernel<GI, FPB, BN, WM, WN, MT, P>), dim3(blocks), dim3(Cfg::NT),
                     Cfg::LDS, st, p, frames);
  return hipGetLastError();
}

}
}
```

acme_amd/csrc/gemm_p3s.h:

```cpp
#pragma once

#include "conv_p3.h"
#include "gemm_p3.h"

namespace acme {
namespace gemm {

template <class G, int FPB = 1>
struct P3SCfg {
  using P = conv::P3ConvDgradSubZ<G>;
  static constexpr int S = G::S, CLASSES = G::S * G::S;
  static constexpr int MT = 2, NW = 2 * CLASSES * FPB, NT = 64 * NW, BK = 32, KS = 2;
  static constexpr int BN = 32;
  static constexpr int H = G::OH, W = G::OW, C = G::CO;
  static constexpr int CPX = C / 8;
  static constexpr int FRAME = H * W * 2 * C;
  static constexpr int PLANE = FPB * FRAME + 16;
  static constexpr int NP = kPlanes;
  static constexpr int IMG = NP * PLANE;
  using PB = PlanP3<BN, 64 * 2 * CLASSES, KCONTIG, NP, BK>;
  static constexpr int STAGE_B = CLASSES * PB::BYTES;
  static constexpr int MAIN = IMG + 2 * STAGE_B;
  static constexpr int EPI = NW * 32 * (BN + 4) * 4;
  static constexpr int LDS = MAIN > EPI ? MAIN : EPI;
  using Core = P3Core<2 * 32 * MT, BN, 2, 1, BK, P>;
  static_assert(G::CI == BN && C == 64 && CPX == 8, "conv2 geometry (CI 32, CO 64)");
  static constexpr int BT = PB::UNITS * CLASSES;
  static_assert(BT == 64 * 2 * CLASSES, "one B unit per loader thread per plane");
  static_assert(P::KR % BK == 0 && (P::KR / BK) % 2 == 0, "whole, even stage count");
  __device__ static __forceinline__ int swz(int q) { return (q >> 1) & (CPX - 1); }
};

template <class G, int FPB>
__global__ void __launch_bounds__(64 * 2 * G::S * G::S * FPB) gemm_p3s_kernel(
    const conv::P3ConvDgradSubZ<G> p_in, int frames) {
  using Cfg = P3SCfg<G, FPB>;
  using PB = typename Cfg::PB;
  using C = typename Cfg::Core;
  using P = conv::P3ConvDgradSubZ<G>;
  constexpr int NT = Cfg::NT, BK = Cfg::BK, KS = Cfg::KS, MT = Cfg::MT, PLANE = Cfg::PLANE;
  constexpr int W = Cfg::W, H = Cfg::H, CPX = Cfg::CPX, NP = Cfg::NP;
  extern __shared__ __attribute__((aligned(16))) uint8_t smem[];

  const int tid = threadIdx.x, lane = tid & 63, wave = tid >> 6;
  const int fi = wave / (2 * Cfg::CLASSES);
  const int f = blockIdx.x * FPB + fi;
  const int z = (wave >> 1) % Cfg::CLASSES, half = wave & 1;
  const uint8_t* img = smem + fi * Cfg::FRAME;
  P pz = p_in.for_z(z);
  const int nhw = pz.nh * pz.nw;
  const int m0 = f * nhw;
  pz.M = m0 + nhw < pz.M ? m0 + nhw : pz.M;
  const int nk = P::KR / BK;

  const bool bload = tid < Cfg::BT;
  const int bz = bload ? tid / PB::UNITS : 0, bu = tid - bz * PB::UNITS;
  const P pb = p_in.for_z(bz);
  const typename P::BRow brow = pb.b_row(PB::row_of(bu));
  __amdgpu_buffer_rsrc_t srcB[NP];
#pragma unroll
  for (int pl = 0; pl < NP; ++pl) srcB[pl] = plane_rsrc(p_in.b_src, pl);
  u32x4 rb[2][NP];
  auto fetch_b = [&](auto S_, int k0) {
    constexpr int set = decltype(S_)::value;
    const uint32_t off = bload && k0 < P::KR ? pb.b_off(brow, k0, PB::kk_of(bu)) : kOOB;
#pragma unroll
    for (int pl = 0; pl < NP; ++pl)
      rb[set][pl] =
          __builtin_bit_cast(u32x4, __builtin_amdgcn_raw_buffer_load_b128(srcB[pl], off, 0, 0));
  };
  auto stash_b = [&](auto S_, int buf) {
    constexpr int set = decltype(S_)::value;
    uint8_t* sb = smem + Cfg::IMG + buf * Cfg::STAGE_B + bz * PB::BYTES;
    if (!bload) return;
#pragma unroll
    for (int pl = 0; pl < NP; ++pl)
      *reinterpret_cast<u32x4*>(sb + pl * PB::PLANE + PB::offset(bu)) = rb[set][pl];
  };
  using S0 = std::integral_constant<int, 0>;
  using S1 = std::integral_constant<int, 1>;
  fetch_b(S0{}, 0);
  fetch_b(S1{}, BK);

  {
    constexpr int UNITS = FPB * H * W * CPX;
    constexpr int PER = (UNITS + NT - 1) / NT;
    __amdgpu_buffer_rsrc_t srcA[NP];
#pragma unroll
    for (int pl = 0; pl < NP; ++pl) srcA[pl] = plane_rsrc(p_in.a_src, pl);
    u32x4 v[PER][NP];
#pragma unroll
    for (int j = 0; j < PER; ++j) {
      const int u = tid + j * NT;
      const bool ok = u < UNITS && blockIdx.x * FPB + u / (H * W * CPX) < frames;
      const uint32_t off = ok ? (uint32_t)(((int64_t)blockIdx.x * UNITS + u) * 16) : kOOB;
#pragma unroll
      for (int pl = 0; pl < NP; ++pl)
        v[j][pl] =
            __builtin_bit_cast(u32x4, __builtin_amdgcn_raw_buffer_load_b128(srcA[pl], off, 0, 0));
    }
#pragma unroll
    for (int j = 0; j < PER; ++j) {
      const int u = tid + j * NT;
      if (u < UNITS) {
        const int fu = u / (H * W * CPX), uu = u - fu * (H * W * CPX);
        const int q = uu / CPX, c = uu - q * CPX;
        const int a = fu * Cfg::FRAME + q * (2 * Cfg::C) + 16 * (c ^ Cfg::swz(q));
#pragma unroll
        for (int pl = 0; pl < NP; ++pl) *reinterpret_cast<u32x4*>(smem + pl * PLANE + a) = v[j][pl];
      }
    }
    if (tid < NP) *reinterpret_cast<u32x4*>(smem + tid * PLANE + PLANE - 16) = zero_u4();
  }
  stash_b(S0{}, 0);

  int oh0[MT], ow0[MT];
  bool rok[MT];
#pragma unroll
  for (int i = 0; i < MT; ++i) {
    const int lr = half * 32 * MT + i * 32 + (lane & 31);
    rok[i] = lr < nhw && f < frames;
    const int ii = rok[i] ? lr / pz.nw : 0, jj = rok[i] ? lr - ii * pz.nw : 0;
    oh0[i] = (pz.rh + Cfg::S * ii + G::PT - pz.ph) / Cfg::S;
    ow0[i] = (pz.rw + Cfg::S * jj + G::PL - pz.pw) / Cfg::S;
  }
  __syncthreads();

  typename C::Acc acc;
  acc.zero();

  auto compute = [&](int k0, int buf) {
    const uint8_t* sb = smem + Cfg::IMG + buf * Cfg::STAGE_B + z * PB::BYTES;
    constexpr int T = P::JW * Cfg::C;
    const int jh = k0 / T, jw = (k0 - jh * T) / Cfg::C;
    const int cb = (k0 % Cfg::C) >> 3;
    int qb[MT], qs[MT];
#pragma unroll
    for (int i = 0; i < MT; ++i) {
      const int oh = oh0[i] - jh, ow = ow0[i] - jw;
      const bool in = rok[i] && (unsigned)oh < (unsigned)H && (unsigned)ow < (unsigned)W;
      const int q = oh * W + ow;
      qb[i] = in ? q * (2 * Cfg::C) : -1;
      qs[i] = Cfg::swz(q);
    }
#pragma unroll
    for (int s = 0; s < KS; ++s) {
      f16x8 fb[NP];
#pragma unroll
      for (int pl = 0; pl < NP; ++pl) fb[pl] = PB::frag(sb, pl, 0, s, lane);
      const int c = cb + 2 * s + (lane >> 5);
#pragma unroll
      for (int i = 0; i < MT; ++i) {
        const uint8_t* a = qb[i] >= 0 ? img + qb[i] + 16 * (c ^ qs[i]) : smem + PLANE - 16;
        f16x8 fa[NP];
#pragma unroll
        for (int pl = 0; pl < NP; ++pl)
          fa[pl] = *reinterpret_cast<const f16x8*>(a + pl * PLANE);
        acc.terms(i, 0, fa, fb);
      }
    }
  };
  auto iter = [&](auto S_, int kt) {
    constexpr int set = decltype(S_)::value;
    using Other = std::integral_constant<int, set ^ 1>;
    stash_b(Other{}, set ^ 1);
    fetch_b(S_, (kt + 2) * BK);
    compute(kt * BK, set);
    __syncthreads();
  };
  for (int kt = 0; kt < nk; kt += 2) {
    iter(S0{}, kt);
    iter(S1{}, kt + 1);
  }

  C::epilogue(pz, smem, m0, 0, wave, half, 0, lane, 0, acc, false);
}

template <class G, int FPB = 1>
inline hipError_t launch_gemm_p3s(const conv::P3ConvDgradSubZ<G>& p, int frames, hipStream_t st) {
  using Cfg = P3SCfg<G, FPB>;
  static_assert(Cfg::LDS <= 160 * 1024, "dZ images + two four-class B stages must fit the LDS");
  static hipError_t attr = p3_set_lds(&gemm_p3s_kernel<G, FPB>, Cfg::LDS);
  if (attr != hipSuccess) return attr;
  if (p.N > Cfg::BN || p.batch != frames || frames < 1) return hipErrorInvalidValue;
  hipLaunchKernelGGL((gemm_p3s_kernel<G, FPB>), dim3((frames + FPB - 1) / FPB), dim3(Cfg::NT),
                     Cfg::LDS, st, p, frames);
  return hipGetLastError();
}

}
}
```

acme_amd/csrc/torso.h:

```cpp
#pragma once

#include <hip/hip_runtime.h>

#include <cstdint>

#include "conv.h"

namespace acme {
namespace gemm {
struct PScale;
}
namespace torso {

using G1 = conv::Geom<84, 84, 4, 21, 21, 32, 8, 8, 4, 2, 2>;
using G2 = conv::Geom<21, 21, 32, 11, 11, 64, 4, 4, 2, 1, 1>;
using G3 = conv::Geom<11, 11, 64, 11, 11, 64, 3, 3, 1, 1, 1>;
constexpr int kFlat = 11 * 11 * 64;
constexpr int kObsBytes = 84 * 84 * 4;
constexpr int kX1 = G1::OPIX * G1::CO;

struct Weights {
  const float *w1, *b1, *w2, *b2, *w3, *b3;
};
struct Grads {
  float *w1, *b1, *w2, *b2, *w3, *b3;
};
struct Acts {
  float *x1, *x2, *x3;
};

int64_t wgrad_slab_floats();

int forward(const Weights& w, bool u8, const void* obs_a, const void* obs_b, int split, int rows,
            const Acts& a, hipStream_t st);

int backward(const Weights& w, const Grads& g, bool u8, const void* obs, int rows, const Acts& a,
             const float* dz3, float* dz2, float* dz1, float* slab, hipStream_t st);

struct Plane {
  uint16_t* p;
  int64_t stride;
  gemm::PScale* sc;
};
struct PWeights {
  Plane w1, w2, w3;
  const float *b1, *b2, *b3;
};
extern uint64_t* g_stamps_conv[3];

struct PActs {
  Plane x1, x2, x3;
};
int64_t wgrad_slab_floats_p3();
struct Frames {
  const void* p;
  bool u8 = false;
  const void* p2 = nullptr;
  int split = 1 << 30;
  Frames rows_from(int r) const {
    if (!u8) return Frames{static_cast<const uint8_t*>(p) + (size_t)r * kObsBytes * 2};
    if (r >= split)
      return Frames{static_cast<const uint8_t*>(p2) + (size_t)(r - split) * kObsBytes, true};
    return Frames{static_cast<const uint8_t*>(p) + (size_t)r * kObsBytes, true, p2, split - r};
  }
};
int forward_p3(const PWeights& w, const Frames& frames, int rows, const PActs& a,
               hipStream_t st, int keep_x1 = -1);
struct WgradSlab {
  const float* slab = nullptr;
  int splits = 0;
  int64_t wcount = 0, bcount = 0;
};
struct Side {
  hipStream_t side = nullptr;
  float* slab = nullptr;
  hipEvent_t e[3] = {nullptr, nullptr, nullptr};
  float* slab2 = nullptr;
  WgradSlab* defer = nullptr;
  int (*tail)(void* ctx, hipStream_t st) = nullptr;
  void* tail_ctx = nullptr;
  bool single_role = false;
  bool conv1_single = false;
};
int backward_p3(const PWeights& w, const Grads& g, const Frames& frames, int rows,
                const PActs& a, const Plane& dz3, const Plane& dz2, const Plane& dz1, float* slab,
                hipStream_t st, const Side& side = Side());

}
}
```

acme_amd/csrc/torso.hip:

```cpp
#include "torso.h"

#include <algorithm>

#include "common.h"
#include "conv_p3.h"
#include "gemm.h"
#include "gemm_p3.h"
#include "gemm_p3i.h"
#include "gemm_p3s.h"
#include "gemm_p3c12.h"
#include "gemm_x6.h"
#include "kernels.h"
#include "launch.h"
#include "plane_guard.h"
#include "profiler.h"

namespace acme {
namespace torso {

using namespace acme::conv;
using acme::gemm::launch_gemm;

namespace {

constexpr int kConv1WgradSplits = 256, kConv2WgradSplits = 64, kConv3WgradSplits = 64;

template <class G, class In, int BM, int BN, int WM, int WN>
int conv_wgrad(const typename In::T* x, const float* dz, int rows, int splits, float* slab,
               float* dw, float* db, const char* name, const char* rname, hipStream_t st) {
  ConvWgrad<G, In> p;
  p.M = G::K; p.N = G::CO; p.K = rows * G::OPIX; p.k_chunk = chunk_for(p.K, splits);
  p.x = x; p.dz = dz; p.slab = slab;
  ACME_GEMM(name, BM, BN, WM, WN, 16, 1, p, splits);
  const int64_t count = (int64_t)(p.M + 1) * p.N;
  ACME_PROF(rname, st, 0.0, 4.0 * (double)(splits + 1) * (double)count);
  return launch_slab_reduce(slab, splits, count, dw, (int64_t)p.M * p.N, db, nullptr, 0, 0, st);
}

}

int64_t wgrad_slab_floats() {
  return std::max<int64_t>({(int64_t)kConv1WgradSplits * (G1::K + 1) * G1::CO,
                            (int64_t)kConv2WgradSplits * (G2::K + 1) * G2::CO,
                            (int64_t)kConv3WgradSplits * (G3::K + 1) * G3::CO});
}

int forward(const Weights& w, bool u8, const void* obs_a, const void* obs_b, int split, int rows,
            const Acts& a, hipStream_t st) {
  if (u8) {
    ConvFwd<G1, InU8> p;
    p.M = rows * G1::OPIX; p.N = G1::CO; p.K = G1::K; p.k_chunk = G1::K;
    p.x = static_cast<const uint8_t*>(obs_a); p.x2 = static_cast<const uint8_t*>(obs_b);
    p.split_b = split; p.w = w.w1; p.bias = w.b1; p.y = a.x1;
    ACME_GEMM("conv1_fwd", 128, 32, 4, 1, 16, 1, p, 1);
  } else {
    ConvFwd<G1, InF32> p;
    p.M = rows * G1::OPIX; p.N = G1::CO; p.K = G1::K; p.k_chunk = G1::K;
    p.x = static_cast<const float*>(obs_a); p.x2 = static_cast<const float*>(obs_b);
    p.split_b = split; p.w = w.w1; p.bias = w.b1; p.y = a.x1;
    ACME_GEMM("conv1_fwd", 128, 32, 4, 1, 16, 1, p, 1);
  }
  {
    ConvFwd<G2, InF32> p;
    p.M = rows * G2::OPIX; p.N = G2::CO; p.K = G2::K; p.k_chunk = G2::K;
    p.x = a.x1; p.x2 = a.x1; p.split_b = rows; p.w = w.w2; p.bias = w.b2; p.y = a.x2;
    ACME_GEMM("conv2_fwd", 128, 64, 2, 2, 16, 1, p, 1);
  }
  {
    ConvFwd<G3, InF32> p;
    p.M = rows * G3::OPIX; p.N = G3::CO; p.K = G3::K; p.k_chunk = G3::K;
    p.x = a.x2; p.x2 = a.x2; p.split_b = rows; p.w = w.w3; p.bias = w.b3; p.y = a.x3;
    ACME_GEMM("conv3_fwd", 128, 64, 2, 2, 16, 1, p, 1);
  }
  return ACME_OK;
}

int backward(const Weights& w, const Grads& g, bool u8, const void* obs, int rows, const Acts& a,
             const float* dz3, float* dz2, float* dz1, float* slab, hipStream_t st) {
  int rc;
  if ((rc = conv_wgrad<G3, InF32, 64, 64, 2, 2>(a.x2, dz3, rows, kConv3WgradSplits, slab, g.w3,
                                                g.b3, "conv3_wgrad", "conv3_wgrad_reduce", st)))
    return rc;
  {
    ConvDgrad<G3> p;
    p.M = rows * G3::IPIX; p.N = G3::CI; p.K = G3::KH * G3::KW * G3::CO; p.k_chunk = p.K;
    p.dz = dz3; p.w = w.w3; p.xprev = a.x2; p.dx = dz2;
    ACME_GEMM("conv3_dgrad", 128, 64, 2, 2, 16, 1, p, 1);
  }
  if ((rc = conv_wgrad<G2, InF32, 64, 64, 2, 2>(a.x1, dz2, rows, kConv2WgradSplits, slab, g.w2,
                                                g.b2, "conv2_wgrad", "conv2_wgrad_reduce", st)))
    return rc;
  {
    ConvDgradSubZ<G2> p;
    p.M = ConvDgradSubZ<G2>::max_rows(rows); p.N = G2::CI; p.K = ConvDgradSubZ<G2>::KR;
    p.k_chunk = p.K; p.batch = rows;
    p.dz = dz2; p.w = w.w2; p.xprev = a.x1; p.dx = dz1;
    ACME_GEMM_F("conv2_dgrad", 2.0 * rows * G2::IPIX * G2::CI * (double)p.K, 256, 32, 4, 1, 16,
                1, p, G2::S * G2::S);
  }
  if (u8)
    return conv_wgrad<G1, InU8, 128, 32, 4, 1>(static_cast<const uint8_t*>(obs), dz1, rows,
                                               kConv1WgradSplits, slab, g.w1, g.b1,
                                               "conv1_wgrad", "conv1_wgrad_reduce", st);
  return conv_wgrad<G1, InF32, 128, 32, 4, 1>(static_cast<const float*>(obs), dz1, rows,
                                              kConv1WgradSplits, slab, g.w1, g.b1, "conv1_wgrad",
                                              "conv1_wgrad_reduce", st);
}

namespace {

constexpr int kP3Conv1WgradSplits = 512, kP3Conv2WgradSplits = 128, kP3Conv3WgradSplits = 128;
constexpr int kP3MaxWgradSplits = 512;

using I1F = gemm::ImgGeomPairs<G1>;
using I2F = gemm::ImgGeom<G2, false>;
using I3F = gemm::ImgGeom<G3, false>;
using I3D = gemm::ImgGeom<G3, true>;
#define P3I_GEMM(name, GI, FPB, BN, WM, WN, MT, prob, frames)                                 \
  ACME_LAUNCH_GEMM(name, ACME_MNK_FLOPS(prob), gemm::p3_peak_tflops<decltype(prob)>(),        \
                   (gemm::launch_gemm_p3i<GI, FPB, BN, WM, WN, MT>(prob, frames, st)))

inline PlaneSrc frames_src(const Frames& f, int rows) {
  return PlaneSrc{static_cast<const uint16_t*>(f.p), 0,
                  (int32_t)((f.u8 ? 1 : 2) * (int64_t)rows * G1::IPIX * G1::CI)};
}

template <bool U8>
int conv1_fwd_p3(const PWeights& w, const Frames& frames, int rows, const Planes& y,
                 hipStream_t st, uint64_t* stamps = nullptr) {
  P3ConvFwd<G1, 1, U8> p;
  p.stamps = stamps;
  p.M = rows * G1::OPIX; p.N = G1::CO; p.K = G1::K; p.k_chunk = G1::K;
  const int n1 = U8 ? std::min(rows, frames.split) : rows;
  p.a_src = frames_src(frames, n1); p.b_src = SRC(w.w1, G1::K * G1::CO);
  if (U8 && n1 < rows) {
    p.a_src2 = frames_src(frames.rows_from(n1), rows - n1);
    p.a_split = n1;
  }
  p.bias = w.b1; p.y = y;
  P3I_GEMM("conv1_fwd", I1F, 1, 32, 7, 1, 2, p, rows);
  return ACME_OK;
}

template <bool U8>
int conv12_fwd_p3(const PWeights& w, const Frames& frames, int rows, int nsep, const PActs& a,
                  hipStream_t st) {
  const int nf = rows - nsep;
  const Frames fr = frames.rows_from(nsep);
  if (U8 && fr.split < nf)
    return (set_error("the fused conv1 -> conv2 forward reads its frames from one buffer"),
            ACME_ERR_INVALID);
  P3ConvFwd<G1, 1, U8> p1;
  p1.M = nf * G1::OPIX; p1.N = G1::CO; p1.K = G1::K; p1.k_chunk = G1::K;
  p1.a_src = frames_src(fr, nf); p1.b_src = SRC(w.w1, G1::K * G1::CO);
  p1.bias = w.b1;
  p1.y = Planes{a.x1.p + (int64_t)nsep * kX1, a.x1.stride, a.x1.sc};
  P3ConvFwd<G2, gemm::kPlanes> p2;
  p2.M = nf * G2::OPIX; p2.N = G2::CO; p2.K = G2::K; p2.k_chunk = G2::K;
  p2.a_src = SRC(a.x1, (int64_t)rows * kX1); p2.b_src = SRC(w.w2, G2::K * G2::CO);
  p2.bias = w.b2;
  p2.y = Planes{a.x2.p + (int64_t)nsep * kFlat, a.x2.stride, a.x2.sc};
  const double fl = 2.0 * p1.M * p1.N * (double)p1.K + 2.0 * p2.M * p2.N * (double)p2.K;
  ACME_PROF_PEAK("conv12_fwd", st, fl, 0.0, gemm::p3_peak_tflops<decltype(p2)>());
  hipError_t e = gemm::launch_gemm_p3c12(p1, p2, nf, 0, st);
  if (e != hipSuccess) return (set_error("gemm launch failed: %s", hipGetErrorString(e)), ACME_ERR_HIP);
  return ACME_OK;
}

template <bool U8>
int conv1_wgrad_p3(const Frames& frames, int rows, const Plane& dz1, float* slab, int splits,
                   bool single_role, P3ConvWgrad<G1, 1, U8>& p, hipStream_t st) {
  if (U8 && frames.split < rows)
    return (set_error("conv1's weight gradient reads its frames from one buffer"),
            ACME_ERR_INVALID);
  P3ConvWgrad<G1, 1, U8> q;
  q.M = G1::K; q.N = G1::CO; q.K = rows * G1::OPIX;
  q.k_chunk = chunk_for(q.K, splits);
  q.a_src = frames_src(frames, rows); q.b_src = SRC(dz1, (int64_t)rows * kX1);
  q.slab = slab;
  if (single_role) ACME_P3_GEMM("conv1_wgrad", 256, 32, 4, 1, 32, q, splits);
  else ACME_P3WS_GEMM("conv1_wgrad", 256, 32, 4, 1, 32, q, splits);
  p = q;
  return ACME_OK;
}

template <class P>
int p3_wgrad_reduce(const P& p, int splits, float* slab, float* dw, float* db, const char* rname,
                    hipStream_t st) {
  const int64_t count = (int64_t)(p.M + 1) * p.N;
  ACME_PROF(rname, st, 0.0, 4.0 * (double)(splits + 1) * (double)count);
  return launch_slab_reduce(slab, splits, count, dw, (int64_t)p.M * p.N, db, nullptr, 0, 0, st);
}

}

uint64_t* g_stamps_conv[3] = {nullptr, nullptr, nullptr};

int64_t wgrad_slab_floats_p3() {
  return std::max<int64_t>({(int64_t)kP3MaxWgradSplits * (G1::K + 1) * G1::CO,
                            (int64_t)kP3MaxWgradSplits * (G2::K + 1) * G2::CO,
                            (int64_t)kP3MaxWgradSplits * (G3::K + 1) * G3::CO});
}

int forward_p3(const PWeights& w, const Frames& frames, int rows, const PActs& a,
               hipStream_t st, int keep_x1) {
  const int nsep = keep_x1 == 0 ? 0 : rows;
  int rc;
  if (nsep < rows &&
      (rc = frames.u8 ? conv12_fwd_p3<true>(w, frames, rows, nsep, a, st)
                      : conv12_fwd_p3<false>(w, frames, rows, nsep, a, st)) != ACME_OK)
    return rc;
  if (nsep > 0 && (rc = frames.u8 ? conv1_fwd_p3<true>(w, frames, nsep, PP(a.x1), st, g_stamps_conv[0])
                                  : conv1_fwd_p3<false>(w, frames, nsep, PP(a.x1), st, g_stamps_conv[0])) != ACME_OK)
    return rc;
  if (nsep > 0) {
    P3ConvFwd<G2, gemm::kPlanes> p;
    p.M = nsep * G2::OPIX; p.N = G2::CO; p.K = G2::K; p.k_chunk = G2::K;
    p.a_src = SRC(a.x1, (int64_t)nsep * kX1); p.b_src = SRC(w.w2, G2::K * G2::CO);
    p.bias = w.b2; p.y = PP(a.x2);
    p.stamps = g_stamps_conv[1];
    P3I_GEMM("conv2_fwd", I2F, 2, 64, 8, 2, 1, p, nsep);
  }
  {
    P3ConvFwd<G3, gemm::kPlanes> p;
    p.M = rows * G3::OPIX; p.N = G3::CO; p.K = G3::K; p.k_chunk = G3::K;
    p.a_src = SRC(a.x2, (int64_t)rows * kFlat); p.b_src = SRC(w.w3, G3::K * G3::CO);
    p.bias = w.b3; p.y = PP(a.x3);
    if (keep_x1 != 0) p.stamps = g_stamps_conv[2];
    P3I_GEMM("conv3_fwd", I3F, 1, 64, 4, 2, 1, p, rows);
  }
  return ACME_OK;
}

int backward_p3(const PWeights& w, const Grads& g, const Frames& frames, int rows,
                const PActs& a, const Plane& dz3, const Plane& dz2, const Plane& dz1, float* slab,
                hipStream_t st_main, const Side& sd) {
  int rc;
  const bool fork = sd.side != nullptr;
  const bool defer = sd.defer != nullptr;
  if (defer && !(sd.slab && sd.slab2))
    return (set_error("deferred weight gradients need two side slabs"), ACME_ERR_INVALID);
  hipStream_t st = fork ? sd.side : st_main;
  float* wslab = fork || defer ? sd.slab : slab;
  {
    if (fork) {
      ACME_HIP_TRY(hipEventRecord(sd.e[0], st_main));
      ACME_HIP_TRY(hipStreamWaitEvent(sd.side, sd.e[0], 0));
    }
    P3ConvWgrad<G3, gemm::kPlanes> p;
    p.M = G3::K; p.N = G3::CO; p.K = rows * G3::OPIX;
    const int splits = kP3Conv3WgradSplits;
    p.k_chunk = chunk_for(p.K, splits);
    p.a_src = SRC(a.x2, (int64_t)rows * kFlat); p.b_src = SRC(dz3, (int64_t)rows * kFlat);
    p.slab = wslab;
    ACME_P3_GEMM("conv3_wgrad", 128, 64, 2, 2, 32, p, splits);
    if (defer) sd.defer[2] = WgradSlab{wslab, splits, (int64_t)p.M * p.N, p.N};
    else if ((rc = p3_wgrad_reduce(p, splits, wslab, g.w3, g.b3, "conv3_wgrad_reduce", st)))
      return rc;
  }
  st = st_main;
  {
    P3ConvDgrad<G3> p;
    p.M = rows * G3::IPIX; p.N = G3::CI; p.K = G3::KH * G3::KW * G3::CO; p.k_chunk = p.K;
    p.a_src = SRC(dz3, (int64_t)rows * kFlat); p.b_src = SRC(w.w3, G3::K * G3::CO);
    p.xprev = CP(a.x2); p.dx = PP(dz2);
    P3I_GEMM("conv3_dgrad", I3D, 2, 64, 8, 2, 1, p, rows);
  }
  if (fork) {
    ACME_HIP_TRY(hipEventRecord(sd.e[1], st_main));
    ACME_HIP_TRY(hipStreamWaitEvent(sd.side, sd.e[1], 0));
    st = sd.side;
  }
  {
    P3ConvWgrad<G2, gemm::kPlanes> p;
    p.M = G2::K; p.N = G2::CO; p.K = rows * G2::OPIX;
    const int splits = kP3Conv2WgradSplits;
    p.k_chunk = chunk_for(p.K, splits);
    p.a_src = SRC(a.x1, (int64_t)rows * kX1); p.b_src = SRC(dz2, (int64_t)rows * kFlat);
    float* slab2 = defer ? sd.slab2 : wslab;
    p.slab = slab2;
    ACME_P3_GEMM("conv2_wgrad", 128, 64, 2, 2, 32, p, splits);
    if (defer) sd.defer[1] = WgradSlab{slab2, splits, (int64_t)p.M * p.N, p.N};
    else if ((rc = p3_wgrad_reduce(p, splits, slab2, g.w2, g.b2, "conv2_wgrad_reduce", st)))
      return rc;
    if (fork) ACME_HIP_TRY(hipEventRecord(sd.e[2], sd.side));
  }
  st = st_main;
  {
    P3ConvDgradSubZ<G2> p;
    p.M = P3ConvDgradSubZ<G2>::max_rows(rows); p.N = G2::CI; p.K = P3ConvDgradSubZ<G2>::KR;
    p.k_chunk = p.K; p.batch = rows;
    p.a_src = SRC(dz2, (int64_t)rows * kFlat); p.b_src = SRC(w.w2, G2::K * G2::CO);
    p.xprev = CP(a.x1); p.dx = PP(dz1);
    const double fl = 2.0 * rows * G2::IPIX * G2::CI * (double)p.K;
    ACME_PROF_PEAK("conv2_dgrad", st, fl, 0.0, gemm::p3_peak_tflops<decltype(p)>());
    hipError_t e = gemm::launch_gemm_p3s<G2, 2>(p, rows, st);
    if (e != hipSuccess) return (set_error("gemm launch failed: %s", hipGetErrorString(e)), ACME_ERR_HIP);
  }
  {
    const int splits = kP3Conv1WgradSplits;
    int64_t wcount;
    int M1, N1;
    if (frames.u8) {
      P3ConvWgrad<G1, 1, true> p;
      if ((rc = conv1_wgrad_p3<true>(frames, rows, dz1, slab, splits, sd.conv1_single, p, st)))
        return rc;
      M1 = p.M, N1 = p.N;
      if (!defer && (rc = p3_wgrad_reduce(p, splits, slab, g.w1, g.b1, "conv1_wgrad_reduce", st)))
        return rc;
    } else {
      P3ConvWgrad<G1, 1> p;
      if ((rc = conv1_wgrad_p3<false>(frames, rows, dz1, slab, splits, sd.conv1_single, p, st)))
        return rc;
      M1 = p.M, N1 = p.N;
      if (!defer && (rc = p3_wgrad_reduce(p, splits, slab, g.w1, g.b1, "conv1_wgrad_reduce", st)))
        return rc;
    }
    wcount = (int64_t)M1 * N1;
    if (defer) sd.defer[0] = WgradSlab{slab, splits, wcount, N1};
  }
  if (sd.tail && (rc = sd.tail(sd.tail_ctx, st_main)) != ACME_OK) return rc;
  if (fork) ACME_HIP_TRY(hipStreamWaitEvent(st_main, sd.e[2], 0));
  return ACME_OK;
}

}
}
```

Measured before the change: 1.067 million transitions/s.

## Stage multiple 32-k groups per pipeline step in image-resident conv kernels

```diff
diff --git a/acme_amd/csrc/conv.h b/acme_amd/csrc/conv.h
--- a/acme_amd/csrc/conv.h
+++ b/acme_amd/csrc/conv.h
@@ -1,5 +1,6 @@
 #pragma once
 
+#include "conv_geom.h"
 #include "gemm.h"
 
 namespace acme {
@@ -9,16 +10,6 @@
 using gemm::KCONTIG;
 using gemm::RCONTIG;
 using gemm::zero4;
-
-template <int IH_, int IW_, int CI_, int OH_, int OW_, int CO_, int KH_, int KW_, int S_,
-          int PT_, int PL_>
-struct Geom {
-  static constexpr int IH = IH_, IW = IW_, CI = CI_, OH = OH_, OW = OW_, CO = CO_;
-  static constexpr int KH = KH_, KW = KW_, S = S_, PT = PT_, PL = PL_;
-  static constexpr int K = KH * KW * CI;
-  static constexpr int IPIX = IH * IW, OPIX = OH * OW;
-  static_assert(CI % 4 == 0 && CO % 4 == 0, "channel counts must be multiples of 4");
-};
 
 struct InU8 {
   using T = uint8_t;
diff --git a/acme_amd/csrc/conv_geom.h b/acme_amd/csrc/conv_geom.h
--- /dev/null
+++ b/acme_amd/csrc/conv_geom.h
@@ -0,0 +1,17 @@
+#pragma once
+
+namespace acme {
+namespace conv {
+
+template <int IH_, int IW_, int CI_, int OH_, int OW_, int CO_, int KH_, int KW_, int S_,
+          int PT_, int PL_>
+struct Geom {
+  static constexpr int IH = IH_, IW = IW_, CI = CI_, OH = OH_, OW = OW_, CO = CO_;
+  static constexpr int KH = KH_, KW = KW_, S = S_, PT = PT_, PL = PL_;
+  static constexpr int K = KH * KW * CI;
+  static constexpr int IPIX = IH * IW, OPIX = OH * OW;
+  static_assert(CI % 4 == 0 && CO % 4 == 0, "channel counts must be multiples of 4");
+};
+
+}
+}
diff --git a/acme_amd/csrc/dqn.hip b/acme_amd/csrc/dqn.hip
--- a/acme_amd/csrc/dqn.hip
+++ b/acme_amd/csrc/dqn.hip
@@ -102,6 +102,7 @@
   double* loss_part = nullptr;
   bool single_stream = false;
   bool single_role = false;
+  bool bk32 = false;
   bool frames_u8 = true;
   int64_t seq = 0;
   uint32_t* host_verdicts = nullptr;
@@ -224,7 +225,7 @@
   if (!slab) slab = l->slab;
   torso::PWeights w{WP(l, wpl, l->t_c1w), WP(l, wpl, l->t_c2w), WP(l, wpl, l->t_c3w),
                     P(l, prm, l->t_c1b), P(l, prm, l->t_c2b), P(l, prm, l->t_c3b)};
-  int rc = torso::forward_p3(w, frames, rows, torso::PActs{x1, x2, x3}, st, keep_x1);
+  int rc = torso::forward_p3(w, frames, rows, torso::PActs{x1, x2, x3}, st, keep_x1, l->bk32);
   if (rc != ACME_OK) return rc;
   {
     P3DenseFwd p;
@@ -523,6 +524,7 @@
   l->cfg = *cfg;
   l->single_stream = tune_variant("SIDE") == 1;
   l->single_role = tune_variant("WSN") == 1;
+  l->bk32 = tune_variant("BK32") == 1;
   l->stamps_on = tune_variant("STAMPS") == 1;
   const int A = cfg->num_actions;
   const int B = cfg->max_batch;
@@ -918,6 +920,7 @@
                         P(l, l->params, l->t_c2b), P(l, l->params, l->t_c3b)};
       torso::Side sd;
       sd.single_role = l->single_role;
+      sd.bk32 = l->bk32;
       sd.conv1_single = true;
       if (side_stream(l)) {
         sd.side = l->side;
diff --git a/acme_amd/csrc/gemm_p3c12.h b/acme_amd/csrc/gemm_p3c12.h
--- a/acme_amd/csrc/gemm_p3c12.h
+++ b/acme_amd/csrc/gemm_p3c12.h
@@ -27,8 +27,7 @@
     uint32_t h[4], l[4];
     const float mx = conv::split8(v, base.y.w(), h, l);
     const int pp = m - m0, oh = pp / G1::OW, ow = pp - oh * G1::OW;
-    const int q = I2::pix(0, oh, ow);
-    const int a = q * (2 * I2::C) + 16 * ((n / 8) ^ I2::swz(q));
+    const int a = I2::at(0, oh, ow, n / 8);
     *reinterpret_cast<u32x4*>(x1 + a) = u32x4{h[0], h[1], h[2], h[3]};
     *reinterpret_cast<u32x4*>(x1 + plane + a) = u32x4{l[0], l[1], l[2], l[3]};
     if (hbm) {
@@ -40,7 +39,7 @@
   }
 };
 
-template <class G1, class G2, bool U8 = false>
+template <class G1, class G2, bool U8 = false, int BK1_ = 32, int BK2_ = 32>
 struct P3C12Cfg {
   using I1 = ImgGeomPairs<G1>;
   using I2 = ImgGeom<G2, false>;
@@ -48,33 +47,42 @@
   using P2 = conv::P3ConvFwd<G2, kPlanes>;
   static constexpr int NP = kPlanes;
   using P1L = P3C1ToLds<G1, G2, U8>;
-  static constexpr int NT = 512, BK = 32, KS = 2;
-  using C1 = P3Core<512, 32, 8, 1, BK, P1L>;
-  using C2 = P3Core<128, 64, 4, 2, BK, P2>;
-  using PB1 = PlanP3<32, NT, RCONTIG, NP, BK>;
-  using PB2 = PlanP3<64, NT, RCONTIG, NP, BK>;
-  static constexpr int FRAME = I1::IMG + 16;
-  static constexpr int RING1 = FRAME;
-  static constexpr int X1 = RING1 + 2 * PB1::BYTES;
-  static constexpr int PLANE2 = I2::IMG + 16;
+  static constexpr int NT = 512, GK = 32, KS = 2;
+  static constexpr int BK1 = BK1_, BK2 = BK2_, NG1 = BK1 / GK, NG2 = BK2 / GK;
+  using C1 = P3Core<512, 32, 8, 1, GK, P1L>;
+  using C2 = P3Core<128, 64, 4, 2, GK, P2>;
+  using PB1 = PlanP3<32, NT, RCONTIG, NP, GK>;
+  using PB2 = PlanP3<64, NT, RCONTIG, NP, GK>;
+  static_assert(BK1 % GK == 0 && BK2 % GK == 0, "a stage is whole 32-k groups");
+  static_assert(NG1 * PB1::UNITS <= NT && NG2 * PB2::UNITS <= NT,
+                "one weight unit per thread per plane and stage");
+  static constexpr int ZERO1 = img_zero_base(I1::IMG);
+  static constexpr int FRAME = ZERO1 + kImgZeroBytes;
+  static constexpr int X1 = FRAME;
+  static constexpr int RING1 = X1;
+  static constexpr int ZERO2 = img_zero_base(I2::IMG);
+  static constexpr int PLANE2 = ZERO2 + kImgZeroBytes;
   static constexpr int LDS = X1 + NP * PLANE2;
-  static_assert(2 * PB2::BYTES <= I1::IMG && C1::EPI_BYTES <= I1::IMG && C2::EPI_BYTES <= I1::IMG,
+  static_assert(2 * NG1 * PB1::BYTES <= I2::IMG, "conv1's ring fits the first x1 plane's image");
+  static_assert(2 * NG2 * PB2::BYTES <= I1::IMG && C1::EPI_BYTES <= I1::IMG &&
+                    C2::EPI_BYTES <= I1::IMG,
                 "conv2's ring and the epilogue staging reuse the frame image region");
   static_assert(G1::OPIX <= 512 && I2::OPIX <= 128 && P2::A_PLANES == NP, "geometry");
 };
 
-template <class G1, class G2, bool U8>
+template <class G1, class G2, bool U8, int BK1_, int BK2_>
 __global__ void __launch_bounds__(512) gemm_p3c12_kernel(const conv::P3ConvFwd<G1, 1, U8> p1,
                                                          const conv::P3ConvFwd<G2, kPlanes> p2,
                                                          int frames, int hbm_frames) {
-  using Cfg = P3C12Cfg<G1, G2, U8>;
+  using Cfg = P3C12Cfg<G1, G2, U8, BK1_, BK2_>;
   using I1 = typename Cfg::I1;
   using I2 = typename Cfg::I2;
   using PB1 = typename Cfg::PB1;
   using PB2 = typename Cfg::PB2;
   using P1 = typename Cfg::P1;
   using P2 = typename Cfg::P2;
-  constexpr int NT = Cfg::NT, BK = Cfg::BK, KS = Cfg::KS, NP = Cfg::NP;
+  constexpr int NT = Cfg::NT, GK = Cfg::GK, KS = Cfg::KS, NP = Cfg::NP;
+  constexpr int BK1 = Cfg::BK1, BK2 = Cfg::BK2, NG1 = Cfg::NG1, NG2 = Cfg::NG2;
   extern __shared__ __attribute__((aligned(16))) uint8_t smem[];
   const int tid = threadIdx.x, lane = tid & 63, wave = tid >> 6;
   const int f = blockIdx.x;
@@ -82,9 +90,11 @@
   using S0 = std::integral_constant<int, 0>;
   using S1 = std::integral_constant<int, 1>;
 
-  const bool own1 = PB1::owns(tid), own2 = PB2::owns(tid);
-  const typename P1::BRow br1 = p1.b_row(own1 ? PB1::row_of(tid) : 0);
-  const typename P2::BRow br2 = p2.b_row(own2 ? PB2::row_of(tid) : 0);
+  const bool own1 = tid < NG1 * PB1::UNITS, own2 = tid < NG2 * PB2::UNITS;
+  const int g1 = tid / PB1::UNITS, u1 = tid % PB1::UNITS;
+  const int g2 = tid / PB2::UNITS, u2 = tid % PB2::UNITS;
+  const typename P1::BRow br1 = p1.b_row(own1 ? PB1::row_of(u1) : 0);
+  const typename P2::BRow br2 = p2.b_row(own2 ? PB2::row_of(u2) : 0);
   __amdgpu_buffer_rsrc_t sb1[NP], sb2[NP];
 #pragma unroll
   for (int pl = 0; pl < NP; ++pl) {
@@ -94,14 +104,16 @@
   u32x4 r1[2][NP], r2[2][NP];
   auto fetch1 = [&](auto S, int k0) {
     constexpr int set = decltype(S)::value;
-    const uint32_t off = own1 && k0 < p1.K ? p1.b_off(br1, k0, PB1::kk_of(tid)) : kOOB;
+    const uint32_t off =
+        own1 && k0 + g1 * GK < p1.K ? p1.b_off(br1, k0 + g1 * GK, PB1::kk_of(u1)) : kOOB;
 #pragma unroll
     for (int pl = 0; pl < NP; ++pl)
       r1[set][pl] = __builtin_bit_cast(u32x4, __builtin_amdgcn_raw_buffer_load_b128(sb1[pl], off, 0, 0));
   };
   auto fetch2 = [&](auto S, int k0) {
     constexpr int set = decltype(S)::value;
-    const uint32_t off = own2 && k0 < p2.K ? p2.b_off(br2, k0, PB2::kk_of(tid)) : kOOB;
+    const uint32_t off =
+        own2 && k0 + g2 * GK < p2.K ? p2.b_off(br2, k0 + g2 * GK, PB2::kk_of(u2)) : kOOB;
 #pragma unroll
     for (int pl = 0; pl < NP; ++pl)
       r2[set][pl] = __builtin_bit_cast(u32x4, __builtin_amdgcn_raw_buffer_load_b128(sb2[pl], off, 0, 0));
@@ -109,21 +121,21 @@
   auto stash1 = [&](auto S, int buf) {
     constexpr int set = decltype(S)::value;
     if (!own1) return;
-    uint8_t* s = smem + Cfg::RING1 + buf * PB1::BYTES;
-#pragma unroll
-    for (int pl = 0; pl < NP; ++pl) *reinterpret_cast<u32x4*>(s + pl * PB1::PLANE + PB1::offset(tid)) = r1[set][pl];
+    uint8_t* s = smem + Cfg::RING1 + (buf * NG1 + g1) * PB1::BYTES;
+#pragma unroll
+    for (int pl = 0; pl < NP; ++pl) *reinterpret_cast<u32x4*>(s + pl * PB1::PLANE + PB1::offset(u1)) = r1[set][pl];
   };
   auto stash2 = [&](auto S, int buf) {
     constexpr int set = decltype(S)::value;
     if (!own2) return;
-    uint8_t* s = smem + buf * PB2::BYTES;
-#pragma unroll
-    for (int pl = 0; pl < NP; ++pl) *reinterpret_cast<u32x4*>(s + pl * PB2::PLANE + PB2::offset(tid)) = r2[set][pl];
+    uint8_t* s = smem + (buf * NG2 + g2) * PB2::BYTES;
+#pragma unroll
+    for (int pl = 0; pl < NP; ++pl) *reinterpret_cast<u32x4*>(s + pl * PB2::PLANE + PB2::offset(u2)) = r2[set][pl];
   };
   fetch1(S0{}, 0);
-  fetch1(S1{}, BK);
+  fetch1(S1{}, BK1);
   fetch2(S0{}, 0);
-  fetch2(S1{}, BK);
+  fetch2(S1{}, BK2);
 
   if constexpr (AU8<P1>::value) {
     constexpr int U8U = I1::UNITS / 2;
@@ -144,8 +156,9 @@
         *reinterpret_cast<u32x4*>(smem + I1::fill(0, 2 * u + 1)) = f16x8_of_bytes(v[j][2], v[j][3]);
       }
     }
-    if (tid == 0) *reinterpret_cast<u32x4*>(smem + Cfg::FRAME - 16) = zero_u4();
-    if (tid < NP) *reinterpret_cast<u32x4*>(x1 + tid * Cfg::PLANE2 + Cfg::PLANE2 - 16) = zero_u4();
+    if (tid < 16) *reinterpret_cast<u32x4*>(smem + Cfg::ZERO1 + 16 * tid) = zero_u4();
+    else if (tid < 16 + 16 * NP)
+      *reinterpret_cast<u32x4*>(x1 + ((tid >> 4) - 1) * Cfg::PLANE2 + Cfg::ZERO2 + 16 * (tid & 15)) = zero_u4();
   } else {
     constexpr int PER = (I1::UNITS + NT - 1) / NT;
     const __amdgpu_buffer_rsrc_t sa = plane_rsrc(p1.a_src, 0);
@@ -161,8 +174,9 @@
       const int u = tid + j * NT;
       if (u < I1::UNITS) *reinterpret_cast<u32x4*>(smem + I1::fill(0, u)) = v[j];
     }
-    if (tid == 0) *reinterpret_cast<u32x4*>(smem + Cfg::FRAME - 16) = zero_u4();
-    if (tid < NP) *reinterpret_cast<u32x4*>(x1 + tid * Cfg::PLANE2 + Cfg::PLANE2 - 16) = zero_u4();
+    if (tid < 16) *reinterpret_cast<u32x4*>(smem + Cfg::ZERO1 + 16 * tid) = zero_u4();
+    else if (tid < 16 + 16 * NP)
+      *reinterpret_cast<u32x4*>(x1 + ((tid >> 4) - 1) * Cfg::PLANE2 + Cfg::ZERO2 + 16 * (tid & 15)) = zero_u4();
   }
   stash1(S0{}, 0);
   __syncthreads();
@@ -176,11 +190,10 @@
     }
     typename Cfg::C1::Acc acc;
     acc.zero();
-    auto compute = [&](int k0, int buf) {
-      const uint8_t* sb = smem + Cfg::RING1 + buf * PB1::BYTES;
+    auto group = [&](int k0, const uint8_t* sb) {
       typename I1::Stage sg[2];
 #pragma unroll
-      for (int i = 0; i < 2; ++i) sg[i] = I1::stage(ln[i], k0);
+      for (int i = 0; i < 2; ++i) sg[i] = I1::stage(ln[i], k0, Cfg::ZERO1);
 #pragma unroll
       for (int s = 0; s < KS; ++s) {
         f16x8 fb[NP];
@@ -189,20 +202,25 @@
 #pragma unroll
         for (int i = 0; i < 2; ++i) {
           const int u = I1::unit(sg[i], ln[i], k0, s, lane >> 5);
-          const f16x8 fa[1] = {*reinterpret_cast<const f16x8*>(smem + (u >= 0 ? u : Cfg::FRAME - 16))};
+          const f16x8 fa[1] = {*reinterpret_cast<const f16x8*>(smem + u)};
           acc.terms(i, 0, fa, fb);
         }
       }
+    };
+    auto compute = [&](int k0, int buf) {
+#pragma unroll
+      for (int g = 0; g < NG1; ++g)
+        group(k0 + g * GK, smem + Cfg::RING1 + (buf * NG1 + g) * PB1::BYTES);
     };
     auto iter = [&](auto S, int kt) {
       constexpr int set = decltype(S)::value;
       using Other = std::integral_constant<int, set ^ 1>;
       stash1(Other{}, set ^ 1);
-      fetch1(S, (kt + 2) * BK);
-      compute(kt * BK, set);
+      fetch1(S, (kt + 2) * BK1);
+      compute(kt * BK1, set);
       __syncthreads();
     };
-    const int nk = p1.K / BK;
+    const int nk = p1.K / BK1;
     for (int kt = 0; kt < nk; kt += 2) {
       iter(S0{}, kt);
       iter(S1{}, kt + 1);
@@ -222,31 +240,34 @@
     const typename I2::Lane ln = I2::lane(0, lr, lr < I2::OPIX);
     typename Cfg::C2::Acc acc;
     acc.zero();
-    auto compute = [&](int k0, int buf) {
-      const uint8_t* sb = smem + buf * PB2::BYTES;
-      const typename I2::Stage sg = I2::stage(ln, k0);
+    auto group = [&](int k0, const uint8_t* sb) {
+      const typename I2::Stage sg = I2::stage(ln, k0, Cfg::ZERO2);
 #pragma unroll
       for (int s = 0; s < KS; ++s) {
         f16x8 fb[NP];
 #pragma unroll
         for (int pl = 0; pl < NP; ++pl) fb[pl] = PB2::frag(sb, pl, wn * 32, s, lane);
         const int u = I2::unit(sg, ln, k0, s, lane >> 5);
-        const uint8_t* a = x1 + (u >= 0 ? u : Cfg::PLANE2 - 16);
+        const uint8_t* a = x1 + u;
         f16x8 fa[NP];
 #pragma unroll
         for (int pl = 0; pl < NP; ++pl) fa[pl] = *reinterpret_cast<const f16x8*>(a + pl * Cfg::PLANE2);
         acc.terms(0, 0, fa, fb);
       }
+    };
+    auto compute = [&](int k0, int buf) {
+#pragma unroll
+      for (int g = 0; g < NG2; ++g) group(k0 + g * GK, smem + (buf * NG2 + g) * PB2::BYTES);
     };
     auto iter = [&](auto S, int kt) {
       constexpr int set = decltype(S)::value;
       using Other = std::integral_constant<int, set ^ 1>;
       stash2(Other{}, set ^ 1);
-      fetch2(S, (kt + 2) * BK);
-      compute(kt * BK, set);
+      fetch2(S, (kt + 2) * BK2);
+      compute(kt * BK2, set);
       __syncthreads();
     };
-    const int nk = p2.K / BK;
+    const int nk = p2.K / BK2;
     for (int kt = 0; kt < nk; kt += 2) {
       iter(S0{}, kt);
       iter(S1{}, kt + 1);
@@ -257,18 +278,18 @@
   }
 }
 
-template <class G1, class G2, bool U8>
+template <int BK1_, int BK2_, class G1, class G2, bool U8>
 inline hipError_t launch_gemm_p3c12(const conv::P3ConvFwd<G1, 1, U8>& p1,
                                     const conv::P3ConvFwd<G2, kPlanes>& p2, int frames, int hbm_frames,
                                     hipStream_t st) {
-  using Cfg = P3C12Cfg<G1, G2, U8>;
+  using Cfg = P3C12Cfg<G1, G2, U8, BK1_, BK2_>;
   static_assert(Cfg::LDS <= 160 * 1024, "LDS");
-  static hipError_t attr = p3_set_lds(&gemm_p3c12_kernel<G1, G2, U8>, Cfg::LDS);
+  static hipError_t attr = p3_set_lds(&gemm_p3c12_kernel<G1, G2, U8, BK1_, BK2_>, Cfg::LDS);
   if (attr != hipSuccess) return attr;
   if (frames < 1 || p1.M != frames * G1::OPIX || p2.M != frames * G2::OPIX || p1.N > 32 ||
-      p2.N > 64 || (p1.K / Cfg::BK) % 2 != 0 || (p2.K / Cfg::BK) % 2 != 0)
+      p2.N > 64 || p1.K % (2 * Cfg::BK1) != 0 || p2.K % (2 * Cfg::BK2) != 0)
     return hipErrorInvalidValue;
-  hipLaunchKernelGGL((gemm_p3c12_kernel<G1, G2, U8>), dim3(frames), dim3(Cfg::NT), Cfg::LDS, st, p1, p2,
+  hipLaunchKernelGGL((gemm_p3c12_kernel<G1, G2, U8, BK1_, BK2_>), dim3(frames), dim3(Cfg::NT), Cfg::LDS, st, p1, p2,
                      frames, hbm_frames);
   return hipGetLastError();
 }
diff --git a/acme_amd/csrc/gemm_p3i.h b/acme_amd/csrc/gemm_p3i.h
--- a/acme_amd/csrc/gemm_p3i.h
+++ b/acme_amd/csrc/gemm_p3i.h
@@ -1,123 +1,42 @@
 #pragma once
 
 #include "gemm_p3.h"
+#include "gemm_p3i_geom.h"
 
 namespace acme {
 namespace gemm {
 
-template <class G, bool DGRAD>
-struct ImgGeom {
-  static constexpr int H = DGRAD ? G::OH : G::IH, W = DGRAD ? G::OW : G::IW;
-  static constexpr int C = DGRAD ? G::CO : G::CI;
-  static constexpr int OH = DGRAD ? G::IH : G::OH, OW = DGRAD ? G::IW : G::OW;
-  static constexpr int S = DGRAD ? 1 : G::S;
-  static constexpr int KW = G::KW;
-  static constexpr int OPIX = OH * OW, IPIX = H * W;
-  static constexpr int CPX = C / 8;
-  static constexpr int HALF = (W + 1) / 2;
-  static constexpr int SWZ = CPX == 8 ? 1 : 2;
-  static constexpr int UNITS = IPIX * CPX, IMG = IPIX * 2 * C;
-  static_assert(!DGRAD || G::S == 1, "strided input gradients are not image-resident");
-  static_assert(C == 32 || C == 64, "a 32-k stage must stay within one tap");
-  static_assert(S == 1 || S == 2, "stride 1 or 2");
-  __device__ static __forceinline__ int dh(int kh) { return DGRAD ? G::PT - kh : kh - G::PT; }
-  __device__ static __forceinline__ int dw(int kw) { return DGRAD ? G::PL - kw : kw - G::PL; }
-  __device__ static __forceinline__ int pix(int fr, int ih, int iw) {
-    return (fr * H + ih) * W + (S == 1 ? iw : (iw & 1) * HALF + (iw >> 1));
-  }
-  __device__ static __forceinline__ int swz(int q) { return (q >> SWZ) & (CPX - 1); }
-  __device__ static __forceinline__ int fill(int f, int u) {
-    const int px = u / CPX, c = u - px * CPX;
-    const int ih = px / W, iw = px - ih * W;
-    const int q = pix(f, ih, iw);
-    return q * (2 * C) + 16 * (c ^ swz(q));
-  }
-  struct Lane {
-    int f, ih, iw;
-    bool ok;
-  };
-  __device__ static __forceinline__ Lane lane(int f, int pp, bool ok) {
-    const int oh = pp / OW, ow = pp - oh * OW;
-    return Lane{f, oh * S, ow * S, ok};
-  }
-  struct Stage {
-    int base, x;
-  };
-  __device__ static __forceinline__ Stage stage(const Lane& l, int k0) {
-    const int tap = k0 / C;
-    const int kh = tap / KW, kw = tap - kh * KW;
-    const int ih = l.ih + dh(kh), iw = l.iw + dw(kw);
-    const bool in = l.ok && (unsigned)ih < (unsigned)H && (unsigned)iw < (unsigned)W;
-    const int q = pix(l.f, ih, iw);
-    return Stage{in ? q * (2 * C) : -1, swz(q)};
-  }
-  __device__ static __forceinline__ int unit(const Stage& st, const Lane&, int k0, int s, int h) {
-    const int c = ((k0 % C) >> 3) + 2 * s + h;
-    return st.base >= 0 ? st.base + 16 * (c ^ st.x) : -1;
-  }
-};
-
-template <class G>
-struct ImgGeomPairs {
-  static constexpr int UNIT = 16;
-  static constexpr int H = G::IH, W = G::IW;
-  static constexpr int OW = G::OW, OPIX = G::OPIX;
-  static constexpr int PAIRS = W / 2, HALF = (PAIRS + 1) / 2;
-  static constexpr int UNITS = H * PAIRS, IMG = UNITS * UNIT;
-  static_assert(G::CI == 4 && G::KW * G::CI == 32, "4 channels, one kernel row per stage");
-  static_assert(W % 2 == 0 && G::S % 2 == 0 && G::PL % 2 == 0, "pairs never straddle the border");
-  __device__ static __forceinline__ int col(int pw) { return (pw & 1) * HALF + (pw >> 1); }
-  __device__ static __forceinline__ int fill(int f, int u) {
-    const int ih = u / PAIRS, pw = u - ih * PAIRS;
-    return ((f * H + ih) * PAIRS + col(pw)) * UNIT;
-  }
-  struct Lane {
-    int f, ih, iw;
-    bool ok;
-  };
-  __device__ static __forceinline__ Lane lane(int f, int pp, bool ok) {
-    const int oh = pp / OW, ow = pp - oh * OW;
-    return Lane{f, oh * G::S - G::PT, ow * G::S - G::PL, ok};
-  }
-  struct Stage {
-    int base;
-  };
-  __device__ static __forceinline__ Stage stage(const Lane& l, int k0) {
-    const int ih = l.ih + k0 / 32;
-    const bool in = l.ok && (unsigned)ih < (unsigned)H;
-    return Stage{in ? (l.f * H + ih) * PAIRS * UNIT : -1};
-  }
-  __device__ static __forceinline__ int unit(const Stage& st, const Lane& l, int, int s, int h) {
-    const int iw = l.iw + 4 * s + 2 * h;
-    return st.base >= 0 && (unsigned)iw < (unsigned)W ? st.base + col(iw >> 1) * UNIT : -1;
-  }
-};
-
-
-template <class GI, int FPB, int BN, int WM, int WN, int MT, class P>
+template <class GI, int FPB, int BN, int WM, int WN, int MT, int BK_, class P>
 struct P3ICfg {
-  static constexpr int BK = 32, KS = 2;
+  static constexpr int BK = BK_;
+  static constexpr int GK = 32, KS = 2;
+  static constexpr int NG = BK / GK;
+  static_assert(BK % GK == 0 && NG >= 1, "a stage is whole 32-k groups");
   static constexpr int NW = WM * WN, NT = 64 * NW;
   static constexpr int TN = BN / WN, NTL = TN / 32;
   static constexpr int BM = WM * 32 * MT;
   static_assert(BM >= FPB * GI::OPIX, "the block's waves must cover its frames' rows");
   static_assert(TN % 32 == 0, "wave panel of whole 32-column MFMA tiles");
-  using Core = P3Core<BM, BN, WM, WN, BK, P>;
+  using Core = P3Core<BM, BN, WM, WN, GK, P>;
   using PB = typename Core::PB;
   static constexpr int NPA = P::A_PLANES;
-  static constexpr int PLANE = FPB * GI::IMG + 16;
+  static constexpr int ZERO = img_zero_base(FPB * GI::IMG);
+  static constexpr int PLANE = ZERO + kImgZeroBytes;
   static constexpr int IMG = NPA * PLANE;
-  static constexpr int STAGE_B = PB::BYTES;
+  static constexpr int STAGE_B = NG * PB::BYTES;
+  static constexpr int B_UNITS = NG * PB::UNITS;
+  static constexpr int B_PER = (B_UNITS + NT - 1) / NT;
   static constexpr int MAIN = IMG + 2 * STAGE_B;
   static constexpr int LDS = MAIN > Core::EPI_BYTES ? MAIN : Core::EPI_BYTES;
 };
 
-template <class GI, int FPB, int BN, int WM, int WN, int MT, class P>
+template <class GI, int FPB, int BN, int WM, int WN, int MT, int BK_, class P>
 __global__ void __launch_bounds__(64 * WM * WN) gemm_p3i_kernel(const P p_in, int frames) {
-  using Cfg = P3ICfg<GI, FPB, BN, WM, WN, MT, P>;
+  using Cfg = P3ICfg<GI, FPB, BN, WM, WN, MT, BK_, P>;
   using C = typename Cfg::Core;
   using PB = typename Cfg::PB;
   constexpr int NT = Cfg::NT, NTL = Cfg::NTL, TN = Cfg::TN, BK = Cfg::BK, KS = Cfg::KS;
+  constexpr int GK = Cfg::GK, NG = Cfg::NG, B_PER = Cfg::B_PER, B_UNITS = Cfg::B_UNITS;
   constexpr int PLANE = Cfg::PLANE, NPA = Cfg::NPA;
   constexpr int NPB = kPlanes;
   static_assert(P::A_MODE == KCONTIG && (NPA == 1 || NPA == kPlanes) && P::B_PLANES == NPB,
@@ -142,24 +61,28 @@
   const int m0 = f0 * GI::OPIX;
   P p = p_in;
   p.M = m0 + rows < p_in.M ? m0 + rows : p_in.M;
-  const int nk = p.K / BK;
-
-  typename P::BRow brow[PB::PER_THREAD];
-#pragma unroll
-  for (int i = 0; i < PB::PER_THREAD; ++i)
-    brow[i] = p.b_row(PB::owns(tid + i * NT) ? PB::row_of(tid + i * NT) : 0);
+  const int nk = (p.K + BK - 1) / BK;
+
+  typename P::BRow brow[B_PER];
+#pragma unroll
+  for (int i = 0; i < B_PER; ++i) {
+    const int u = tid + i * NT;
+    brow[i] = p.b_row(u < B_UNITS ? PB::row_of(u % PB::UNITS) : 0);
+  }
   __amdgpu_buffer_rsrc_t srcB[NPB];
 #pragma unroll
   for (int pl = 0; pl < NPB; ++pl) srcB[pl] = plane_rsrc(p.b_src, pl);
   constexpr int RS = 2;
-  u32x4 rb[RS][PB::PER_THREAD][NPB];
+  u32x4 rb[RS][B_PER][NPB];
   auto fetch_b = [&](auto S, int k0) {
     constexpr int set = decltype(S)::value;
 #pragma unroll
-    for (int i = 0; i < PB::PER_THREAD; ++i) {
+    for (int i = 0; i < B_PER; ++i) {
       const int u = tid + i * NT;
-      const int kk = PB::kk_of(u);
-      const uint32_t off = (PB::owns(u) && k0 + kk < p.K) ? p.b_off(brow[i], k0, kk) : kOOB;
+      const int g = u / PB::UNITS, kk = PB::kk_of(u % PB::UNITS);
+      const int kg = k0 + g * GK;
+      const uint32_t off =
+          ((B_UNITS % NT == 0 || u < B_UNITS) && kg + kk < p.K) ? p.b_off(brow[i], kg, kk) : kOOB;
 #pragma unroll
       for (int pl = 0; pl < NPB; ++pl)
         rb[set][i][pl] =
@@ -170,10 +93,10 @@
     constexpr int set = decltype(S)::value;
     uint8_t* sb = smem + Cfg::IMG + buf * Cfg::STAGE_B;
 #pragma unroll
-    for (int i = 0; i < PB::PER_THREAD; ++i) {
+    for (int i = 0; i < B_PER; ++i) {
       const int u = tid + i * NT;
-      if (!PB::owns(u)) continue;
-      const int off = PB::offset(u);
+      if (B_UNITS % NT != 0 && u >= B_UNITS) continue;
+      const int off = (u / PB::UNITS) * PB::BYTES + PB::offset(u % PB::UNITS);
 #pragma unroll
       for (int pl = 0; pl < NPB; ++pl)
         *reinterpret_cast<u32x4*>(sb + pl * PB::PLANE + off) = rb[set][i][pl];
@@ -209,7 +132,7 @@
         *reinterpret_cast<u32x4*>(smem + GI::fill(0, 2 * u + 1)) = f16x8_of_bytes(v[j][2], v[j][3]);
       }
     }
-    if (tid == 0) *reinterpret_cast<u32x4*>(smem + PLANE - 16) = zero_u4();
+    if (tid < 16) *reinterpret_cast<u32x4*>(smem + Cfg::ZERO + 16 * tid) = zero_u4();
   } else {
     constexpr int UNITS = FPB * GI::UNITS;
     constexpr int PER = (UNITS + NT - 1) / NT;
@@ -238,7 +161,8 @@
         for (int pl = 0; pl < NPA; ++pl) *reinterpret_cast<UT*>(smem + pl * PLANE + a) = v[j][pl];
       }
     }
-    if (tid < NPA) *reinterpret_cast<u32x4*>(smem + tid * PLANE + PLANE - 16) = zero_u4();
+    if (tid < 16 * NPA)
+      *reinterpret_cast<u32x4*>(smem + (tid >> 4) * PLANE + Cfg::ZERO + 16 * (tid & 15)) = zero_u4();
   }
   stash_b(S0{}, 0);
 
@@ -258,34 +182,43 @@
   typename EpiPre<P>::type pre{};
   if constexpr (EpiPre<P>::has) pre = p.pre(wn * TN + C::epi_col(lane));
 
+  auto group = [&](int k0, const uint8_t* sb) {
+    typename GI::Stage sg[MT];
+#pragma unroll
+    for (int i = 0; i < MT; ++i) sg[i] = GI::stage(ln[i], k0, Cfg::ZERO);
+    f16x8 fb[KS][NTL][NPB], fa[KS][MT][NPA];
+#pragma unroll
+    for (int s = 0; s < KS; ++s) {
+#pragma unroll
+      for (int j = 0; j < NTL; ++j)
+#pragma unroll
+        for (int pl = 0; pl < NPB; ++pl) fb[s][j][pl] = PB::frag(sb, pl, wn * TN + j * 32, s, lane);
+#pragma unroll
+      for (int i = 0; i < MT; ++i) {
+        const int a = GI::unit(sg[i], ln[i], k0, s, lane >> 5);
+#pragma unroll
+        for (int pl = 0; pl < NPA; ++pl)
+          fa[s][i][pl] = *reinterpret_cast<const f16x8*>(smem + pl * PLANE + a);
+      }
+    }
+    __builtin_amdgcn_sched_barrier(0);
+#pragma unroll
+    for (int s = 0; s < KS; ++s)
+#pragma unroll
+      for (int i = 0; i < MT; ++i)
+#pragma unroll
+        for (int j = 0; j < NTL; ++j) acc.terms(i, j, fa[s][i], fb[s][j]);
+  };
   auto compute = [&](int k0, int buf) {
     const uint8_t* sb = smem + Cfg::IMG + buf * Cfg::STAGE_B;
-    typename GI::Stage sg[MT];
-#pragma unroll
-    for (int i = 0; i < MT; ++i) sg[i] = GI::stage(ln[i], k0);
-    f16x8 fb[KS][NTL][NPB], fa[KS][MT][NPA];
-#pragma unroll
-    for (int s = 0; s < KS; ++s) {
-#pragma unroll
-      for (int j = 0; j < NTL; ++j)
-#pragma unroll
-        for (int pl = 0; pl < NPB; ++pl) fb[s][j][pl] = PB::frag(sb, pl, wn * TN + j * 32, s, lane);
-#pragma unroll
-      for (int i = 0; i < MT; ++i) {
-        const int u = GI::unit(sg[i], ln[i], k0, s, lane >> 5);
-        const int a = u >= 0 ? u : PLANE - 16;
-#pragma unroll
-        for (int pl = 0; pl < NPA; ++pl)
-          fa[s][i][pl] = *reinterpret_cast<const f16x8*>(smem + pl * PLANE + a);
-      }
-    }
-    __builtin_amdgcn_sched_barrier(0);
-#pragma unroll
-    for (int s = 0; s < KS; ++s)
-#pragma unroll
-      for (int i = 0; i < MT; ++i)
-#pragma unroll
-        for (int j = 0; j < NTL; ++j) acc.terms(i, j, fa[s][i], fb[s][j]);
+#pragma unroll
+    for (int g = 0; g < NG; ++g) {
+      if (g > 0) {
+        if (k0 + g * GK >= p.K) break;
+        __builtin_amdgcn_sched_barrier(0);
+      }
+      group(k0 + g * GK, sb + g * PB::BYTES);
+    }
   };
 
   auto iter = [&](auto S, int kt) {
@@ -320,15 +253,15 @@
   }
 }
 
-template <class GI, int FPB, int BN, int WM, int WN, int MT, class P>
+template <class GI, int FPB, int BN, int WM, int WN, int MT, int BK_, class P>
 inline hipError_t launch_gemm_p3i(const P& p, int frames, hipStream_t st) {
-  using Cfg = P3ICfg<GI, FPB, BN, WM, WN, MT, P>;
+  using Cfg = P3ICfg<GI, FPB, BN, WM, WN, MT, BK_, P>;
   static_assert(Cfg::LDS <= 160 * 1024, "image + two B stages must fit the 160-KiB LDS");
-  static hipError_t attr = p3_set_lds(&gemm_p3i_kernel<GI, FPB, BN, WM, WN, MT, P>, Cfg::LDS);
+  static hipError_t attr = p3_set_lds(&gemm_p3i_kernel<GI, FPB, BN, WM, WN, MT, BK_, P>, Cfg::LDS);
   if (attr != hipSuccess) return attr;
-  if (p.N > BN || p.M != frames * GI::OPIX || p.K % Cfg::BK != 0) return hipErrorInvalidValue;
+  if (p.N > BN || p.M != frames * GI::OPIX || p.K % Cfg::GK != 0) return hipErrorInvalidValue;
   const int blocks = (frames + FPB - 1) / FPB;
-  hipLaunchKernelGGL((gemm_p3i_kernel<GI, FPB, BN, WM, WN, MT, P>), dim3(blocks), dim3(Cfg::NT),
+  hipLaunchKernelGGL((gemm_p3i_kernel<GI, FPB, BN, WM, WN, MT, BK_, P>), dim3(blocks), dim3(Cfg::NT),
                      Cfg::LDS, st, p, frames);
   return hipGetLastError();
 }
diff --git a/acme_amd/csrc/gemm_p3i_geom.h b/acme_amd/csrc/gemm_p3i_geom.h
--- /dev/null
+++ b/acme_amd/csrc/gemm_p3i_geom.h
@@ -0,0 +1,181 @@
+#pragma once
+
+#include "conv_geom.h"
+
+#if defined(__HIPCC__)
+#define ACME_GEOM_FN __host__ __device__ static __forceinline__
+#else
+#define ACME_GEOM_FN static inline
+#endif
+
+namespace acme {
+namespace gemm {
+
+constexpr int kImgZeroBytes = 256;
+
+constexpr int img_zero_base(int bytes) { return (bytes + 255) & ~255; }
+
+constexpr int img_pitch(int n, int opix) { return n + (((opix - n) % 16) + 16) % 16; }
+
+template <class G, bool DGRAD>
+struct ImgGeom {
+  static constexpr int H = DGRAD ? G::OH : G::IH, W = DGRAD ? G::OW : G::IW;
+  static constexpr int C = DGRAD ? G::CO : G::CI;
+  static constexpr int OH = DGRAD ? G::IH : G::OH, OW = DGRAD ? G::IW : G::OW;
+  static constexpr int S = DGRAD ? 1 : G::S;
+  static constexpr int KW = G::KW;
+  static constexpr int OPIX = OH * OW, IPIX = H * W;
+  static constexpr int CPX = C / 8;
+  static constexpr int SWZ = CPX == 8 ? 1 : 2;
+  static constexpr int CH = (H + S - 1) / S, CW = (W + S - 1) / S;
+  static constexpr int FPITCH = img_pitch(S * S * CH * CW, OPIX);
+  static constexpr int UNITS = IPIX * CPX, IMG = FPITCH * 2 * C;
+  static_assert(!DGRAD || G::S == 1, "strided input gradients are not image-resident");
+  static_assert(C == 32 || C == 64, "a 32-k group must stay within one tap");
+  static_assert(S == 1 || S == 2, "stride 1 or 2");
+  static_assert(CW == OW, "class pitch = output pitch: a tap's positions are row + constant");
+  ACME_GEOM_FN int dh(int kh) { return DGRAD ? G::PT - kh : kh - G::PT; }
+  ACME_GEOM_FN int dw(int kw) { return DGRAD ? G::PL - kw : kw - G::PL; }
+  ACME_GEOM_FN int pix(int fr, int ih, int iw) {
+    if constexpr (S == 1) return fr * FPITCH + ih * CW + iw;
+    else return fr * FPITCH + ((ih & 1) * 2 + (iw & 1)) * (CH * CW) + (ih >> 1) * CW + (iw >> 1);
+  }
+  ACME_GEOM_FN int swz(int q) { return (q >> SWZ) & (CPX - 1); }
+  ACME_GEOM_FN int at(int fr, int ih, int iw, int c) {
+    const int q = pix(fr, ih, iw);
+    return q * (2 * C) + 16 * (c ^ swz(q));
+  }
+  ACME_GEOM_FN int fill(int f, int u) {
+    const int px = u / CPX, c = u - px * CPX;
+    const int ih = px / W, iw = px - ih * W;
+    return at(f, ih, iw, c);
+  }
+  struct Lane {
+    int f, ih, iw;
+    bool ok;
+  };
+  ACME_GEOM_FN Lane lane(int f, int pp, bool ok) {
+    const int oh = pp / OW, ow = pp - oh * OW;
+    return Lane{f, oh * S, ow * S, ok};
+  }
+  struct Stage {
+    int base, x;
+  };
+  ACME_GEOM_FN Stage stage(const Lane& l, int k0, int zero) {
+    const int tap = k0 / C;
+    const int kh = tap / KW, kw = tap - kh * KW;
+    const int ih = l.ih + dh(kh), iw = l.iw + dw(kw);
+    const bool in = l.ok && (unsigned)ih < (unsigned)H && (unsigned)iw < (unsigned)W;
+    const int q = pix(l.f, ih, iw);
+    const int b = q * (2 * C);
+    return Stage{in ? b : zero + (b & 255), swz(q)};
+  }
+  ACME_GEOM_FN int unit(const Stage& st, const Lane&, int k0, int s, int h) {
+    const int c = ((k0 % C) >> 3) + 2 * s + h;
+    return st.base + 16 * (c ^ st.x);
+  }
+};
+
+template <class G>
+struct ImgGeomPairs {
+  static constexpr int UNIT = 16;
+  static constexpr int H = G::IH, W = G::IW;
+  static constexpr int OW = G::OW, OPIX = G::OPIX;
+  static constexpr int PAIRS = W / 2;
+  static constexpr int SR = G::S, SC = G::S / 2;
+  static constexpr int CH = (H + SR - 1) / SR, CW = (PAIRS + SC - 1) / SC;
+  static constexpr int FPITCH = img_pitch(SR * SC * CH * CW, OPIX);
+  static constexpr int UNITS = H * PAIRS, IMG = FPITCH * UNIT;
+  static_assert(G::CI == 4 && G::KW * G::CI == 32, "4 channels, one kernel row per group");
+  static_assert(W % 2 == 0 && G::S % 2 == 0 && G::PL % 2 == 0, "pairs never straddle the border");
+  static_assert((SR & (SR - 1)) == 0 && (SC & (SC - 1)) == 0, "power-of-two classes");
+  static_assert(CW == OW, "class pitch = output pitch: a tap's positions are row + constant");
+  ACME_GEOM_FN int row_pos(int fr, int ih) {
+    const int cr = ih & (SR - 1);
+    return fr * FPITCH + cr * SC * (CH * CW) + (ih - cr) / SR * CW;
+  }
+  ACME_GEOM_FN int pos(int rp, int pw) {
+    const int cc = pw & (SC - 1);
+    return rp + cc * (CH * CW) + (pw - cc) / SC;
+  }
+  ACME_GEOM_FN int fill(int f, int u) {
+    const int ih = u / PAIRS, pw = u - ih * PAIRS;
+    return pos(row_pos(f, ih), pw) * UNIT;
+  }
+  struct Lane {
+    int f, ih, iw;
+    bool ok;
+  };
+  ACME_GEOM_FN Lane lane(int f, int pp, bool ok) {
+    const int oh = pp / OW, ow = pp - oh * OW;
+    return Lane{f, oh * G::S - G::PT, ow * G::S - G::PL, ok};
+  }
+  struct Stage {
+    int rp;
+    bool in;
+    int zero;
+  };
+  ACME_GEOM_FN Stage stage(const Lane& l, int k0, int zero) {
+    const int ih = l.ih + k0 / 32;
+    return Stage{row_pos(l.f, ih), l.ok && (unsigned)ih < (unsigned)H, zero};
+  }
+  ACME_GEOM_FN int unit(const Stage& st, const Lane& l, int, int s, int h) {
+    const int iw = l.iw + 4 * s + 2 * h;
+    const int q = pos(st.rp, (iw - (iw & 1)) / 2);
+    const int a = q * UNIT;
+    return st.in && (unsigned)iw < (unsigned)W ? a : st.zero + (a & 255);
+  }
+};
+
+template <class G>
+struct ImgGeomSub {
+  static constexpr int S = G::S, CLASSES = S * S;
+  static constexpr int H = G::OH, W = G::OW, C = G::CO;
+  static constexpr int JW = G::KW / S, KR = (G::KH / S) * JW * C;
+  static constexpr int CPX = C / 8;
+  static constexpr int SWZ = CPX == 8 ? 1 : 2;
+  static constexpr int UNITS = H * W * CPX, IMG = H * W * 2 * C;
+  static_assert(C == 32 || C == 64, "a 32-k group must stay within one tap");
+  struct Cls {
+    int ph, pw, rh, rw, nh, nw;
+  };
+  ACME_GEOM_FN Cls cls(int z) {
+    const int ph = z / S, pw = z % S;
+    const int rh = ((ph - G::PT) % S + S) % S, rw = ((pw - G::PL) % S + S) % S;
+    return Cls{ph, pw, rh, rw, (G::IH - rh + S - 1) / S, (G::IW - rw + S - 1) / S};
+  }
+  ACME_GEOM_FN int swz(int q) { return (q >> SWZ) & (CPX - 1); }
+  ACME_GEOM_FN int fill(int f, int u) {
+    const int q = u / CPX, c = u - q * CPX;
+    return f * IMG + q * (2 * C) + 16 * (c ^ swz(q));
+  }
+  struct Lane {
+    int f, oh0, ow0;
+    bool ok;
+  };
+  ACME_GEOM_FN Lane lane(int f, int z, int lr, bool ok) {
+    const Cls k = cls(z);
+    const bool in = ok && lr < k.nh * k.nw;
+    const int i = in ? lr / k.nw : 0, j = in ? lr - i * k.nw : 0;
+    return Lane{f, (k.rh + S * i + G::PT - k.ph) / S, (k.rw + S * j + G::PL - k.pw) / S, in};
+  }
+  struct Stage {
+    int base, x;
+  };
+  ACME_GEOM_FN Stage stage(const Lane& l, int k0, int zero) {
+    constexpr int T = JW * C;
+    const int jh = k0 / T, jw = (k0 - jh * T) / C;
+    const int oh = l.oh0 - jh, ow = l.ow0 - jw;
+    const bool in = l.ok && (unsigned)oh < (unsigned)H && (unsigned)ow < (unsigned)W;
+    const int q = oh * W + ow;
+    const int b = l.f * IMG + q * (2 * C);
+    return in ? Stage{b, swz(q)} : Stage{zero, 0};
+  }
+  ACME_GEOM_FN int unit(const Stage& st, const Lane&, int k0, int s, int h) {
+    const int c = ((k0 % C) >> 3) + 2 * s + h;
+    return st.base + 16 * (c ^ st.x);
+  }
+};
+
+}
+}
diff --git a/acme_amd/csrc/gemm_p3s.h b/acme_amd/csrc/gemm_p3s.h
--- a/acme_amd/csrc/gemm_p3s.h
+++ b/acme_amd/csrc/gemm_p3s.h
@@ -2,59 +2,66 @@
 
 #include "conv_p3.h"
 #include "gemm_p3.h"
+#include "gemm_p3i_geom.h"
 
 namespace acme {
 namespace gemm {
 
-template <class G, int FPB = 1>
+
+template <class G, int FPB = 1, int BK_ = 32>
 struct P3SCfg {
   using P = conv::P3ConvDgradSubZ<G>;
   static constexpr int S = G::S, CLASSES = G::S * G::S;
-  static constexpr int MT = 2, NW = 2 * CLASSES * FPB, NT = 64 * NW, BK = 32, KS = 2;
+  static constexpr int MT = 2, NW = 2 * CLASSES * FPB, NT = 64 * NW, GK = 32, KS = 2;
+  static constexpr int BK = BK_, NG = BK / GK;
   static constexpr int BN = 32;
-  static constexpr int H = G::OH, W = G::OW, C = G::CO;
-  static constexpr int CPX = C / 8;
-  static constexpr int FRAME = H * W * 2 * C;
-  static constexpr int PLANE = FPB * FRAME + 16;
+  using GI = ImgGeomSub<G>;
+  static constexpr int C = GI::C, CPX = GI::CPX;
+  static constexpr int FRAME = GI::IMG;
+  static constexpr int ZERO = img_zero_base(FPB * FRAME);
+  static constexpr int PLANE = ZERO + kImgZeroBytes;
   static constexpr int NP = kPlanes;
   static constexpr int IMG = NP * PLANE;
-  using PB = PlanP3<BN, 64 * 2 * CLASSES, KCONTIG, NP, BK>;
-  static constexpr int STAGE_B = CLASSES * PB::BYTES;
+  using PB = PlanP3<BN, 64 * 2 * CLASSES, KCONTIG, NP, GK>;
+  static constexpr int GROUP_B = CLASSES * PB::BYTES;
+  static constexpr int STAGE_B = NG * GROUP_B;
   static constexpr int MAIN = IMG + 2 * STAGE_B;
   static constexpr int EPI = NW * 32 * (BN + 4) * 4;
   static constexpr int LDS = MAIN > EPI ? MAIN : EPI;
-  using Core = P3Core<2 * 32 * MT, BN, 2, 1, BK, P>;
+  using Core = P3Core<2 * 32 * MT, BN, 2, 1, GK, P>;
   static_assert(G::CI == BN && C == 64 && CPX == 8, "conv2 geometry (CI 32, CO 64)");
   static constexpr int BT = PB::UNITS * CLASSES;
   static_assert(BT == 64 * 2 * CLASSES, "one B unit per loader thread per plane");
+  static_assert(BK % GK == 0 && NG * BT <= NT, "one B unit per loader thread per plane and stage");
   static_assert(P::KR % BK == 0 && (P::KR / BK) % 2 == 0, "whole, even stage count");
-  __device__ static __forceinline__ int swz(int q) { return (q >> 1) & (CPX - 1); }
 };
 
-template <class G, int FPB>
+template <class G, int FPB, int BK_>
 __global__ void __launch_bounds__(64 * 2 * G::S * G::S * FPB) gemm_p3s_kernel(
     const conv::P3ConvDgradSubZ<G> p_in, int frames) {
-  using Cfg = P3SCfg<G, FPB>;
+  using Cfg = P3SCfg<G, FPB, BK_>;
   using PB = typename Cfg::PB;
   using C = typename Cfg::Core;
   using P = conv::P3ConvDgradSubZ<G>;
-  constexpr int NT = Cfg::NT, BK = Cfg::BK, KS = Cfg::KS, MT = Cfg::MT, PLANE = Cfg::PLANE;
-  constexpr int W = Cfg::W, H = Cfg::H, CPX = Cfg::CPX, NP = Cfg::NP;
+  constexpr int NT = Cfg::NT, BK = Cfg::BK, GK = Cfg::GK, NG = Cfg::NG, KS = Cfg::KS, MT = Cfg::MT;
+  constexpr int PLANE = Cfg::PLANE;
+  constexpr int NP = Cfg::NP;
+  using GI = typename Cfg::GI;
   extern __shared__ __attribute__((aligned(16))) uint8_t smem[];
 
   const int tid = threadIdx.x, lane = tid & 63, wave = tid >> 6;
   const int fi = wave / (2 * Cfg::CLASSES);
   const int f = blockIdx.x * FPB + fi;
   const int z = (wave >> 1) % Cfg::CLASSES, half = wave & 1;
-  const uint8_t* img = smem + fi * Cfg::FRAME;
   P pz = p_in.for_z(z);
   const int nhw = pz.nh * pz.nw;
   const int m0 = f * nhw;
   pz.M = m0 + nhw < pz.M ? m0 + nhw : pz.M;
   const int nk = P::KR / BK;
 
-  const bool bload = tid < Cfg::BT;
-  const int bz = bload ? tid / PB::UNITS : 0, bu = tid - bz * PB::UNITS;
+  const bool bload = tid < NG * Cfg::BT;
+  const int bg = bload ? tid / Cfg::BT : 0, bt = tid - bg * Cfg::BT;
+  const int bz = bload ? bt / PB::UNITS : 0, bu = bt - bz * PB::UNITS;
   const P pb = p_in.for_z(bz);
   const typename P::BRow brow = pb.b_row(PB::row_of(bu));
   __amdgpu_buffer_rsrc_t srcB[NP];
@@ -63,7 +70,8 @@
   u32x4 rb[2][NP];
   auto fetch_b = [&](auto S_, int k0) {
     constexpr int set = decltype(S_)::value;
-    const uint32_t off = bload && k0 < P::KR ? pb.b_off(brow, k0, PB::kk_of(bu)) : kOOB;
+    const uint32_t off =
+        bload && k0 + bg * GK < P::KR ? pb.b_off(brow, k0 + bg * GK, PB::kk_of(bu)) : kOOB;
 #pragma unroll
     for (int pl = 0; pl < NP; ++pl)
       rb[set][pl] =
@@ -71,7 +79,7 @@
   };
   auto stash_b = [&](auto S_, int buf) {
     constexpr int set = decltype(S_)::value;
-    uint8_t* sb = smem + Cfg::IMG + buf * Cfg::STAGE_B + bz * PB::BYTES;
+    uint8_t* sb = smem + Cfg::IMG + buf * Cfg::STAGE_B + bg * Cfg::GROUP_B + bz * PB::BYTES;
     if (!bload) return;
 #pragma unroll
     for (int pl = 0; pl < NP; ++pl)
@@ -83,7 +91,7 @@
   fetch_b(S1{}, BK);
 
   {
-    constexpr int UNITS = FPB * H * W * CPX;
+    constexpr int UNITS = FPB * GI::UNITS;
     constexpr int PER = (UNITS + NT - 1) / NT;
     __amdgpu_buffer_rsrc_t srcA[NP];
 #pragma unroll
@@ -92,7 +100,7 @@
 #pragma unroll
     for (int j = 0; j < PER; ++j) {
       const int u = tid + j * NT;
-      const bool ok = u < UNITS && blockIdx.x * FPB + u / (H * W * CPX) < frames;
+      const bool ok = u < UNITS && blockIdx.x * FPB + u / GI::UNITS < frames;
       const uint32_t off = ok ? (uint32_t)(((int64_t)blockIdx.x * UNITS + u) * 16) : kOOB;
 #pragma unroll
       for (int pl = 0; pl < NP; ++pl)
@@ -103,55 +111,38 @@
     for (int j = 0; j < PER; ++j) {
       const int u = tid + j * NT;
       if (u < UNITS) {
-        const int fu = u / (H * W * CPX), uu = u - fu * (H * W * CPX);
-        const int q = uu / CPX, c = uu - q * CPX;
-        const int a = fu * Cfg::FRAME + q * (2 * Cfg::C) + 16 * (c ^ Cfg::swz(q));
+        const int fu = u / GI::UNITS;
+        const int a = GI::fill(fu, u - fu * GI::UNITS);
 #pragma unroll
         for (int pl = 0; pl < NP; ++pl) *reinterpret_cast<u32x4*>(smem + pl * PLANE + a) = v[j][pl];
       }
     }
-    if (tid < NP) *reinterpret_cast<u32x4*>(smem + tid * PLANE + PLANE - 16) = zero_u4();
+    if (tid < 16 * NP)
+      *reinterpret_cast<u32x4*>(smem + (tid >> 4) * PLANE + Cfg::ZERO + 16 * (tid & 15)) = zero_u4();
   }
   stash_b(S0{}, 0);
 
-  int oh0[MT], ow0[MT];
-  bool rok[MT];
+  typename GI::Lane ln[MT];
 #pragma unroll
-  for (int i = 0; i < MT; ++i) {
-    const int lr = half * 32 * MT + i * 32 + (lane & 31);
-    rok[i] = lr < nhw && f < frames;
-    const int ii = rok[i] ? lr / pz.nw : 0, jj = rok[i] ? lr - ii * pz.nw : 0;
-    oh0[i] = (pz.rh + Cfg::S * ii + G::PT - pz.ph) / Cfg::S;
-    ow0[i] = (pz.rw + Cfg::S * jj + G::PL - pz.pw) / Cfg::S;
-  }
+  for (int i = 0; i < MT; ++i)
+    ln[i] = GI::lane(fi, z, half * 32 * MT + i * 32 + (lane & 31), f < frames);
   __syncthreads();
 
   typename C::Acc acc;
   acc.zero();
 
-  auto compute = [&](int k0, int buf) {
-    const uint8_t* sb = smem + Cfg::IMG + buf * Cfg::STAGE_B + z * PB::BYTES;
-    constexpr int T = P::JW * Cfg::C;
-    const int jh = k0 / T, jw = (k0 - jh * T) / Cfg::C;
-    const int cb = (k0 % Cfg::C) >> 3;
-    int qb[MT], qs[MT];
+  auto group = [&](int k0, const uint8_t* sb) {
+    typename GI::Stage sg[MT];
 #pragma unroll
-    for (int i = 0; i < MT; ++i) {
-      const int oh = oh0[i] - jh, ow = ow0[i] - jw;
-      const bool in = rok[i] && (unsigned)oh < (unsigned)H && (unsigned)ow < (unsigned)W;
-      const int q = oh * W + ow;
-      qb[i] = in ? q * (2 * Cfg::C) : -1;
-      qs[i] = Cfg::swz(q);
-    }
+    for (int i = 0; i < MT; ++i) sg[i] = GI::stage(ln[i], k0, Cfg::ZERO);
 #pragma unroll
     for (int s = 0; s < KS; ++s) {
       f16x8 fb[NP];
 #pragma unroll
       for (int pl = 0; pl < NP; ++pl) fb[pl] = PB::frag(sb, pl, 0, s, lane);
-      const int c = cb + 2 * s + (lane >> 5);
 #pragma unroll
       for (int i = 0; i < MT; ++i) {
-        const uint8_t* a = qb[i] >= 0 ? img + qb[i] + 16 * (c ^ qs[i]) : smem + PLANE - 16;
+        const uint8_t* a = smem + GI::unit(sg[i], ln[i], k0, s, lane >> 5);
         f16x8 fa[NP];
 #pragma unroll
         for (int pl = 0; pl < NP; ++pl)
@@ -159,6 +150,11 @@
         acc.terms(i, 0, fa, fb);
       }
     }
+  };
+  auto compute = [&](int k0, int buf) {
+#pragma unroll
+    for (int g = 0; g < NG; ++g)
+      group(k0 + g * GK, smem + Cfg::IMG + buf * Cfg::STAGE_B + g * Cfg::GROUP_B + z * PB::BYTES);
   };
   auto iter = [&](auto S_, int kt) {
     constexpr int set = decltype(S_)::value;
@@ -176,14 +172,14 @@
   C::epilogue(pz, smem, m0, 0, wave, half, 0, lane, 0, acc, false);
 }
 
-template <class G, int FPB = 1>
+template <class G, int FPB = 1, int BK_ = 32>
 inline hipError_t launch_gemm_p3s(const conv::P3ConvDgradSubZ<G>& p, int frames, hipStream_t st) {
-  using Cfg = P3SCfg<G, FPB>;
+  using Cfg = P3SCfg<G, FPB, BK_>;
   static_assert(Cfg::LDS <= 160 * 1024, "dZ images + two four-class B stages must fit the LDS");
-  static hipError_t attr = p3_set_lds(&gemm_p3s_kernel<G, FPB>, Cfg::LDS);
+  static hipError_t attr = p3_set_lds(&gemm_p3s_kernel<G, FPB, BK_>, Cfg::LDS);
   if (attr != hipSuccess) return attr;
   if (p.N > Cfg::BN || p.batch != frames || frames < 1) return hipErrorInvalidValue;
-  hipLaunchKernelGGL((gemm_p3s_kernel<G, FPB>), dim3((frames + FPB - 1) / FPB), dim3(Cfg::NT),
+  hipLaunchKernelGGL((gemm_p3s_kernel<G, FPB, BK_>), dim3((frames + FPB - 1) / FPB), dim3(Cfg::NT),
                      Cfg::LDS, st, p, frames);
   return hipGetLastError();
 }
diff --git a/acme_amd/csrc/torso.h b/acme_amd/csrc/torso.h
--- a/acme_amd/csrc/torso.h
+++ b/acme_amd/csrc/torso.h
@@ -65,7 +65,7 @@
   }
 };
 int forward_p3(const PWeights& w, const Frames& frames, int rows, const PActs& a,
-               hipStream_t st, int keep_x1 = -1);
+               hipStream_t st, int keep_x1 = -1, bool bk32 = false);
 struct WgradSlab {
   const float* slab = nullptr;
   int splits = 0;
@@ -81,6 +81,7 @@
   void* tail_ctx = nullptr;
   bool single_role = false;
   bool conv1_single = false;
+  bool bk32 = false;
 };
 int backward_p3(const PWeights& w, const Grads& g, const Frames& frames, int rows,
                 const PActs& a, const Plane& dz3, const Plane& dz2, const Plane& dz1, float* slab,
diff --git a/acme_amd/csrc/torso.hip b/acme_amd/csrc/torso.hip
--- a/acme_amd/csrc/torso.hip
+++ b/acme_amd/csrc/torso.hip
@@ -116,9 +116,18 @@
 using I2F = gemm::ImgGeom<G2, false>;
 using I3F = gemm::ImgGeom<G3, false>;
 using I3D = gemm::ImgGeom<G3, true>;
-#define P3I_GEMM(name, GI, FPB, BN, WM, WN, MT, prob, frames)                                 \
+#define P3I_GEMM(name, GI, FPB, BN, WM, WN, MT, BK, prob, frames)                             \
   ACME_LAUNCH_GEMM(name, ACME_MNK_FLOPS(prob), gemm::p3_peak_tflops<decltype(prob)>(),        \
-                   (gemm::launch_gemm_p3i<GI, FPB, BN, WM, WN, MT>(prob, frames, st)))
+                   (gemm::launch_gemm_p3i<GI, FPB, BN, WM, WN, MT, BK>(prob, frames, st)))
+#define P3I_GEMM_BK(name, GI, FPB, BN, WM, WN, MT, BK, bk32, prob, frames) \
+  do {                                                                     \
+    if (bk32) P3I_GEMM(name, GI, FPB, BN, WM, WN, MT, 32, prob, frames);   \
+    else P3I_GEMM(name, GI, FPB, BN, WM, WN, MT, BK, prob, frames);        \
+  } while (0)
+
+constexpr int kBkConv1 = 64, kBkConv2 = 64, kBkConv3 = 32;
+constexpr int kBkConv3Dgrad = 128, kBkConv2Dgrad = 32;
+constexpr int kBkFused1 = 32, kBkFused2 = 64;
 
 inline PlaneSrc frames_src(const Frames& f, int rows) {
   return PlaneSrc{static_cast<const uint16_t*>(f.p), 0,
@@ -127,7 +136,7 @@
 
 template <bool U8>
 int conv1_fwd_p3(const PWeights& w, const Frames& frames, int rows, const Planes& y,
-                 hipStream_t st, uint64_t* stamps = nullptr) {
+                 hipStream_t st, bool bk32, uint64_t* stamps = nullptr) {
   P3ConvFwd<G1, 1, U8> p;
   p.stamps = stamps;
   p.M = rows * G1::OPIX; p.N = G1::CO; p.K = G1::K; p.k_chunk = G1::K;
@@ -138,13 +147,13 @@
     p.a_split = n1;
   }
   p.bias = w.b1; p.y = y;
-  P3I_GEMM("conv1_fwd", I1F, 1, 32, 7, 1, 2, p, rows);
+  P3I_GEMM_BK("conv1_fwd", I1F, 1, 32, 7, 1, 2, kBkConv1, bk32, p, rows);
   return ACME_OK;
 }
 
 template <bool U8>
 int conv12_fwd_p3(const PWeights& w, const Frames& frames, int rows, int nsep, const PActs& a,
-                  hipStream_t st) {
+                  hipStream_t st, bool bk32) {
   const int nf = rows - nsep;
   const Frames fr = frames.rows_from(nsep);
   if (U8 && fr.split < nf)
@@ -162,7 +171,8 @@
   p2.y = Planes{a.x2.p + (int64_t)nsep * kFlat, a.x2.stride, a.x2.sc};
   const double fl = 2.0 * p1.M * p1.N * (double)p1.K + 2.0 * p2.M * p2.N * (double)p2.K;
   ACME_PROF_PEAK("conv12_fwd", st, fl, 0.0, gemm::p3_peak_tflops<decltype(p2)>());
-  hipError_t e = gemm::launch_gemm_p3c12(p1, p2, nf, 0, st);
+  hipError_t e = bk32 ? gemm::launch_gemm_p3c12<32, 32>(p1, p2, nf, 0, st)
+                      : gemm::launch_gemm_p3c12<kBkFused1, kBkFused2>(p1, p2, nf, 0, st);
   if (e != hipSuccess) return (set_error("gemm launch failed: %s", hipGetErrorString(e)), ACME_ERR_HIP);
   return ACME_OK;
 }
@@ -203,15 +213,15 @@
 }
 
 int forward_p3(const PWeights& w, const Frames& frames, int rows, const PActs& a,
-               hipStream_t st, int keep_x1) {
+               hipStream_t st, int keep_x1, bool bk32) {
   const int nsep = keep_x1 == 0 ? 0 : rows;
   int rc;
   if (nsep < rows &&
-      (rc = frames.u8 ? conv12_fwd_p3<true>(w, frames, rows, nsep, a, st)
-                      : conv12_fwd_p3<false>(w, frames, rows, nsep, a, st)) != ACME_OK)
+      (rc = frames.u8 ? conv12_fwd_p3<true>(w, frames, rows, nsep, a, st, bk32)
+                      : conv12_fwd_p3<false>(w, frames, rows, nsep, a, st, bk32)) != ACME_OK)
     return rc;
-  if (nsep > 0 && (rc = frames.u8 ? conv1_fwd_p3<true>(w, frames, nsep, PP(a.x1), st, g_stamps_conv[0])
-                                  : conv1_fwd_p3<false>(w, frames, nsep, PP(a.x1), st, g_stamps_conv[0])) != ACME_OK)
+  if (nsep > 0 && (rc = frames.u8 ? conv1_fwd_p3<true>(w, frames, nsep, PP(a.x1), st, bk32, g_stamps_conv[0])
+                                  : conv1_fwd_p3<false>(w, frames, nsep, PP(a.x1), st, bk32, g_stamps_conv[0])) != ACME_OK)
     return rc;
   if (nsep > 0) {
     P3ConvFwd<G2, gemm::kPlanes> p;
@@ -219,7 +229,7 @@
     p.a_src = SRC(a.x1, (int64_t)nsep * kX1); p.b_src = SRC(w.w2, G2::K * G2::CO);
     p.bias = w.b2; p.y = PP(a.x2);
     p.stamps = g_stamps_conv[1];
-    P3I_GEMM("conv2_fwd", I2F, 2, 64, 8, 2, 1, p, nsep);
+    P3I_GEMM_BK("conv2_fwd", I2F, 2, 64, 8, 2, 1, kBkConv2, bk32, p, nsep);
   }
   {
     P3ConvFwd<G3, gemm::kPlanes> p;
@@ -227,7 +237,7 @@
     p.a_src = SRC(a.x2, (int64_t)rows * kFlat); p.b_src = SRC(w.w3, G3::K * G3::CO);
     p.bias = w.b3; p.y = PP(a.x3);
     if (keep_x1 != 0) p.stamps = g_stamps_conv[2];
-    P3I_GEMM("conv3_fwd", I3F, 1, 64, 4, 2, 1, p, rows);
+    P3I_GEMM_BK("conv3_fwd", I3F, 1, 64, 4, 2, 1, kBkConv3, bk32, p, rows);
   }
   return ACME_OK;
 }
@@ -264,7 +274,7 @@
     p.M = rows * G3::IPIX; p.N = G3::CI; p.K = G3::KH * G3::KW * G3::CO; p.k_chunk = p.K;
     p.a_src = SRC(dz3, (int64_t)rows * kFlat); p.b_src = SRC(w.w3, G3::K * G3::CO);
     p.xprev = CP(a.x2); p.dx = PP(dz2);
-    P3I_GEMM("conv3_dgrad", I3D, 2, 64, 8, 2, 1, p, rows);
+    P3I_GEMM_BK("conv3_dgrad", I3D, 2, 64, 8, 2, 1, kBkConv3Dgrad, sd.bk32, p, rows);
   }
   if (fork) {
     ACME_HIP_TRY(hipEventRecord(sd.e[1], st_main));
@@ -294,7 +304,8 @@
     p.xprev = CP(a.x1); p.dx = PP(dz1);
     const double fl = 2.0 * rows * G2::IPIX * G2::CI * (double)p.K;
     ACME_PROF_PEAK("conv2_dgrad", st, fl, 0.0, gemm::p3_peak_tflops<decltype(p)>());
-    hipError_t e = gemm::launch_gemm_p3s<G2, 2>(p, rows, st);
+    hipError_t e = sd.bk32 ? gemm::launch_gemm_p3s<G2, 2, 32>(p, rows, st)
+                           : gemm::launch_gemm_p3s<G2, 2, kBkConv2Dgrad>(p, rows, st);
     if (e != hipSuccess) return (set_error("gemm launch failed: %s", hipGetErrorString(e)), ACME_ERR_HIP);
   }
   {
```

Measured after the change: 1.082 million transitions/s (median of 6 runs). 1.5% higher.
